# rkansal47/MPGAN

Hardware: AMD Instinct MI355X
Metric: jets/sec (G+D step) MPGAN gluon N=30 bs=256 @1/2/4/8 MI355X (higher is better)
Workload: dtype split-16-bit MFMA, fp32 accumulate, fp32 in/out: f16 hi/lo x3 terms (forward), f16 x2 / x1 terms in per-sender dithered units (edge backward: data / weight gradients), bf16 hi/lo x3 (node network gradients); 1 GPU; MPGAN gluon-like jets (--jets g: lr_disc 3e-05, lr_gen 1e-05), N=30 particles, B=256 per GPU, one train_D+train_G iteration (LSGAN, RMSprop, D dropout 0.5); jets=g, loss=ls, fwd_two_term=False, global_batch=256, particles=30, multiplicity=gluon, parallelism=dp1, hip_graphs=True, graph_collectives=False

## Files before the change

include/mpgan_amd.h:

```cpp
#ifndef MPGAN_AMD_H
#define MPGAN_AMD_H
#include <stdint.h>
#ifdef __cplusplus
extern "C" {
#endif

typedef struct MpgGemm {
    const float* A;
    const float* A2;
    int lda, lda2, K1;
    const float* B;
    int ldb;
    float* C;
    int ldc;
    int M, N, K;
    long long split_stride;
    const float* bias;
    float out_scale;
    int act;
    float alpha;
    const uint64_t* seed;
    uint32_t drop_tag, drop_thr; float drop_scale;
    const float* gateH;
    int ldh, gate_act;
    uint32_t gate_tag, gate_thr; float gate_scale;
    const float* resid;
    int ldr;
    int accumulate;
    int f16;
    int ones_col;
} MpgGemm;

int mpg_gemm(const MpgGemm* g, int ak, int bk, int splitk, void* stream);

int mpg_splitk_reduce(const float* part, int S, int N, int K, int has_bias, float* out, int ldo, float* bias,
                      void* stream);

#define MPG_GROUP_MAX 16
typedef struct MpgReduceJob {
    const float* part; int S, N, K, has_bias; float* out; int ldo; float* bias;
    int accumulate;
} MpgReduceJob;
int mpg_gemm_wgrad_group(const MpgGemm* g, const int* splitk, int n, void* stream);
int mpg_splitk_reduce_group(const MpgReduceJob* jobs, int n, void* stream);

int mpg_gate(const float* in, int ldi, const float* H, int ldh, float* out, int ldo, int M, int N,
             int gate_act, float alpha, const uint64_t* seed, uint32_t tag, uint32_t thr, float scale,
             void* stream);

int mpg_slab_sums(const float* A, int slabsA, uint64_t strideA, const float* B, int slabsB, uint64_t strideB,
                  float* out, int M, int cols, void* stream);

int mpg_dropout_mask(float* out, uint64_t rows, int F, const uint64_t* seed, uint32_t tag, uint32_t thr,
                     void* stream);

int mpg_pack_weights(const float* W, int ldw, int rows, int cols, int transpose, float scale, int f16,
                     void* img, void* stream);

#define MPG_PACK_MAX_JOBS 24
typedef struct MpgPackJob {
    const float* W; int ldw, rows, cols, transpose; float scale; int f16; void* img;
    int row_split, split_cols;
    int* status;
} MpgPackJob;
int mpg_pack_many(const MpgPackJob* jobs, int njobs, void* stream);

typedef struct MpgChainLayer {
    const void* Wimg; const float* bias; int nbias;
    int K, N, act;
    uint32_t drop_tag, drop_thr; float drop_scale;
    const float* gateH; int ldh, gate_act;
    uint32_t gate_tag, gate_thr; float gate_scale;
    const float* resid; int ldr;
    float* out; int ldo;
    float wscale;
} MpgChainLayer;
typedef struct MpgChain {
    const float* A; int lda, K1;
    const float* A2; int lda2;
    int a_slabs; uint64_t a_slab_stride;
    uint32_t in_tag, in_thr; float in_scale;
    float* in_out; int ld_in_out;
    int M, nlayers; float alpha; const uint64_t* seed; int f16;
    float ascale;
    MpgChainLayer L[3];
} MpgChain;
int mpg_chain(const MpgChain* p, void* stream);

typedef struct MpgEdgeFwd {
    const float* a; const float* c;
    int ld_ac;
    const float* mask;
    const void* W2img; const void* W3img;
    const float* b2; const float* b3;
    float* agg;
    int B, N, SC;
    float alpha, agg_scale;
    const uint64_t* seed; uint32_t tag_base, thr; float dscale;
    int skip_masked;
    int f16;
    unsigned int* sign3;
    const unsigned int* nbr;
    void* stageE2;
    const float* es; const float* wq;
    const int* order;
    unsigned int* tickets;
    int two_term;
} MpgEdgeFwd;
#define MPG_EDGE_SCALARS 2
int mpg_edge_fwd(const MpgEdgeFwd* p, void* stream);

#define MPG_FN_NA (-100)
int mpg_edge_fwd_fn(const MpgEdgeFwd* p, const MpgChain* c, const MpgChain* c2, void* stream);

int mpg_knn_sets(const float* x, int ldx, const float* mask, int B, int N, int F, int k, int self_loops,
                 unsigned int* nbr, void* stream);

typedef struct MpgEdgeBwd {
    const float* a; const float* c; int ld_ac; const float* mask;
    const float* dagg; int ld_dagg;
    const unsigned int* sign3;
    const void* W2img; const void* W3Timg; const void* W2Timg;
    const float* b2;
    float* da; float* dc;
    const void* stageE2;
    void* stageZ2;
    int B, N, SC;
    float alpha, agg_scale;
    const uint64_t* seed; uint32_t tag_base, thr; float dscale;
    int f16;
    const unsigned int* nbr;
    int* gexp;
    const float* es; const float* wq;
    float* des;
    float* daq;
    const int* order;
} MpgEdgeBwd;
int mpg_edge_bwd(const MpgEdgeBwd* p, void* stream);

int mpg_edge_bwd_fn(const MpgEdgeBwd* p, const MpgChain* cdx, const MpgChain* cnx, void* stream);

typedef struct MpgEdgeDw {
    const float* a; const float* c; int ld_ac; const float* mask;
    const float* dagg; int ld_dagg;
    const unsigned int* sign3;
    const void* stageE2; const void* stageZ2;
    float* part; int nwg;
    float* dW3; float* dW2; float* db3; float* db2;
    int accumulate;
    int B, N;
    float alpha, agg_scale;
    const uint64_t* seed; uint32_t tag_base, thr; float dscale;
    int f16;
    const unsigned int* nbr;
    const int* gexp;
    const float* es; const float* wq;
    int defer_reduce;
} MpgEdgeDw;
int mpg_edge_dw(const MpgEdgeDw* p, void* stream);
int mpg_splitk_reduce_group_dw(const MpgReduceJob* jobs, int n, const MpgEdgeDw* p, void* stream);

typedef struct MpgAttn {
    const float* q; const float* k; const float* v; int ldq, ldk, ldv;
    const float* ignore;
    float* o; int ldo;
    float* P;
    const float* d_o;
    float* dq; float* dk; float* dv; int lddq, lddk, lddv;
    int B, L, S, H, d;
} MpgAttn;
int mpg_attn_fwd(const MpgAttn* p, void* stream);
int mpg_attn_bwd(const MpgAttn* p, void* stream);

int mpg_rank_mask(const float* x, int ld_jet, int ld_part, const float* labels, int ld_lab, int B, int N,
                  float* mask, float* ignore, void* stream);

int mpg_jet_order(const float* mask, int B, int N, int* order, void* stream);

int mpg_gen_tail_fwd(const float* y, int ldy, const float* mask, float* out, int ldo, int V, int F, int act, void* stream);
int mpg_gen_tail_bwd(const float* dout, int ldd, const float* out, int ldo, float* dy, int ldy, int V, int F, int act,
                     void* stream);

typedef struct MpgDiscHead {
    const float* y; int ldy;
    const float* mask;
    const float* w; const float* bias;
    int B, N, F;
    int mean;
    int sigmoid;
    const uint64_t* seed; uint32_t tag, thr; float dscale;
    float* out;
    float* pooled; float* aux;
    int loss, gen_step, n_real; float inv_count;
    const float* gout;
    float* terms; float* loss_out;
    float* dy; int ld_dy;
    float* dw; float* db; int accumulate;
} MpgDiscHead;
int mpg_disc_head_fwd(const MpgDiscHead* p, void* stream);
int mpg_disc_head_bwd(const MpgDiscHead* p, void* stream);
int mpg_disc_head_loss(const MpgDiscHead* p, void* stream);

typedef struct MpgBridge {
    const float* x; int ldx;
    const float* W1; const float* b1;
    int act1;
    float* feat; int ldf;
    int M, row0, K, F, E;
    const float* W2; const float* b2;
    int act2; float alpha;
    const uint64_t* seed; uint32_t tag, thr; float dscale;
    float* e; int lde;
} MpgBridge;
typedef struct MpgBridgeBwd {
    const float* ge; int ldge;
    const float* e; int lde;
    const float* feat; int ldf;
    const float* gfeat; int ldgf;
    const float* W1; const float* W2;
    int M, row0, K, F, E, act1, act2; float alpha;
    const uint64_t* seed; uint32_t tag, thr; float dscale;
    float* g2; int ldg2;
    float* g1; int ldg1;
    float* dx; int lddx;
} MpgBridgeBwd;
int mpg_bridge_fwd(const MpgBridge* p, void* stream);
int mpg_bridge_bwd(const MpgBridgeBwd* p, void* stream);

typedef struct MpgMab {
    const float* x; int ldx;
    const float* y; int ldy;
    const float* ignore;
    const void* Win; const float* bin;
    const void* Wo; const float* bo;
    const void* Wf; const float* bf;
    int B, L, S, E, H;
    float alpha; int ff_act;
    const uint64_t* seed; uint32_t tag; uint32_t thr_mab; float sc_mab; uint32_t thr_ff; float sc_ff;
    float wscale, ascale;
    float* out; int ldo;
    float* save_o; float* save_z;
    const void* WinT; const void* WoT; const void* WfT;
    const float* dout; int lddout;
    float* dx; int lddx; float* dy; int lddy;
    float* dq; int lddq; float* dk; float* dv; int lddkv;
    float* dza; float* du;
    const float* ln1_w; const float* ln1_b; const float* ln2_w; const float* ln2_b; float ln_eps;
    float* save_za;
    float* dn1; float* gn1; float* dn2; float* gn2;
} MpgMab;
int mpg_mab_fwd(const MpgMab* p, void* stream);
int mpg_mab_bwd(const MpgMab* p, void* stream);
#define MPG_MAB_CHAIN_MAX 4
typedef struct MpgMabChain { MpgMab blk[MPG_MAB_CHAIN_MAX]; int n; } MpgMabChain;
int mpg_mab_chain_fwd(const MpgMabChain* c, void* stream);

int mpg_layernorm_fwd(const float* x, int ldx, const float* w, const float* b, float* y, int ldy, float* stats, int M,
                      int E, float eps, void* stream);
int mpg_layernorm_bwd(const float* g, int ldg, const float* x, int ldx, const float* w, const float* stats, float* dx,
                      int lddx, float* part, int nwaves, float* dw, float* db, int accumulate, int M, int E, void* stream);

int mpg_batchnorm_stats(const float* x, int ldx, int M, int F, float* part, int nchunk, float* mean, float* var, void* stream);
int mpg_batchnorm_apply(const float* x, int ldx, const float* mean, const float* var, const float* w, const float* b, float eps,
                        float* y, int ldy, int M, int F, void* stream);
int mpg_batchnorm_bwd(const float* g, int ldg, const float* x, int ldx, const float* mean, const float* var, const float* w, float eps,
                      float* part, int nchunk, float* sums, float* dx, int lddx, float* dw, float* db, int accumulate, int M, int F,
                      void* stream);

int mpg_rmsprop(float* p, float* g, float* v, uint64_t n, float lr, float alpha, float eps, float gscale, int zero_grad,
                uint64_t* counter, uint64_t counter_add, void* stream);
int mpg_adam(float* p, float* g, float* m, float* v, float* step, uint64_t n, float lr, float beta1,
             float beta2, float eps, float weight_decay, float gscale, int zero_grad, uint64_t* counter, uint64_t counter_add,
             void* stream);
int mpg_adadelta(float* p, float* g, float* v, float* u, uint64_t n, float lr, float rho, float eps,
                 float gscale, int zero_grad, uint64_t* counter, uint64_t counter_add, void* stream);

#define MPG_JET_OBS_MAX_N 160
#define MPG_JET_OBS_EFP 1
#define MPG_JET_OBS_NORMED 2
int mpg_jet_obs(const float* jets, int ld_jet, int ld_part, int n, int N, int flags, float* kin, float* efp, void* stream);

#define MPG_JET_EFPS_D4_PRIMES 21
int mpg_jet_efps_d4(const float* jets, int ld_jet, int ld_part, int n, int N, int flags, float* efp, void* stream);

int mpg_jet_emd(const float* a, int ld_jet_a, const float* b, int ld_jet_b, int ld_part, int na, int nb, int N, float R,
                float* out, int* status, void* stream);
int mpg_jet_emd_host(const float* a, int ld_jet_a, const float* b, int ld_jet_b, int ld_part, int na, int nb, int N, float R,
                     double* out, int* status, int threads);
int mpg_jet_emd_host_iters(const float* a, int ld_jet_a, const float* b, int ld_jet_b, int ld_part, int na, int nb, int N, float R,
                           double* out, int* status, int* iters, int threads);

int mpg_normal(float* out, uint64_t n, const uint64_t* seed, uint32_t tag, float mean, float std, void* stream);
int mpg_normal_rank_mask(float* out, int B, int N, int L, const uint64_t* seed, uint32_t tag, float mean, float std,
                         const float* labels, int ld_lab, float* mask, float* ignore, void* stream);

#define MPG_AUG_R90 1
#define MPG_AUG_FLIP 2
#define MPG_AUG_TRANSLATE 4
#define MPG_AUG_SCALE 8
int mpg_augment(const float* x, float* y, uint64_t jet_stride, int ld, int F, int B, int N, const uint64_t* seed, uint32_t tag,
                const float* p, int flags, float translate_ratio, float scale_sd, float* params, void* stream);
int mpg_augment_bwd(const float* dy, float* dx, uint64_t jet_stride, int ld, int F, int B, int N, const float* params,
                    void* stream);

#define MPG_SHUFFLE_TAG 0x53000000
int mpg_shuffle_index_host(uint64_t key, uint64_t pos0, int64_t count, int64_t n, int32_t* out);

int mpg_batch_feed(const float* particles, const float* labels_in, int64_t n, int N, uint64_t key, uint64_t* cursor,
                   uint32_t* ticket, int B, uint64_t stride, float* data, float* labels, float* dcat, float* x3, float* mask2,
                   float* ign2, float* labels2, void* stream);

#ifdef __cplusplus
}
#endif
#endif
```

mpgan_amd/_lib.py:

```python
from __future__ import annotations

import ctypes as C
import glob
import os
import subprocess

_HERE = os.path.dirname(os.path.abspath(__file__))
CSRC = os.path.join(_HERE, "csrc")
LIBDIR = os.environ.get("MPG_LIBDIR") or os.path.join(_HERE, "lib")
LIBPATH = os.path.join(LIBDIR, "libmpgan_amd.so")
INCLUDE = os.path.join(os.path.dirname(_HERE), "include")

_u64p = C.POINTER(C.c_uint64)
_fp = C.c_void_p


class MpgGemm(C.Structure):
    _fields_ = [
        ("A", _fp), ("A2", _fp), ("lda", C.c_int), ("lda2", C.c_int), ("K1", C.c_int),
        ("B", _fp), ("ldb", C.c_int),
        ("C", _fp), ("ldc", C.c_int),
        ("M", C.c_int), ("N", C.c_int), ("K", C.c_int),
        ("split_stride", C.c_longlong),
        ("bias", _fp), ("out_scale", C.c_float), ("act", C.c_int), ("alpha", C.c_float),
        ("seed", _fp),
        ("drop_tag", C.c_uint32), ("drop_thr", C.c_uint32), ("drop_scale", C.c_float),
        ("gateH", _fp), ("ldh", C.c_int), ("gate_act", C.c_int),
        ("gate_tag", C.c_uint32), ("gate_thr", C.c_uint32), ("gate_scale", C.c_float),
        ("resid", _fp), ("ldr", C.c_int),
        ("accumulate", C.c_int), ("f16", C.c_int), ("ones_col", C.c_int),
    ]


class MpgEdgeFwd(C.Structure):
    _fields_ = [
        ("a", _fp), ("c", _fp), ("ld_ac", C.c_int), ("mask", _fp),
        ("W2img", _fp), ("W3img", _fp), ("b2", _fp), ("b3", _fp),
        ("agg", _fp),
        ("B", C.c_int), ("N", C.c_int), ("SC", C.c_int),
        ("alpha", C.c_float), ("agg_scale", C.c_float),
        ("seed", _fp), ("tag_base", C.c_uint32), ("thr", C.c_uint32), ("dscale", C.c_float),
        ("skip_masked", C.c_int), ("f16", C.c_int),
        ("sign3", _fp), ("nbr", _fp), ("stageE2", _fp),
        ("es", _fp), ("wq", _fp), ("order", _fp), ("tickets", _fp),
        ("two_term", C.c_int),
    ]


class MpgEdgeBwd(C.Structure):
    _fields_ = [
        ("a", _fp), ("c", _fp), ("ld_ac", C.c_int), ("mask", _fp),
        ("dagg", _fp), ("ld_dagg", C.c_int),
        ("sign3", _fp),
        ("W2img", _fp), ("W3Timg", _fp), ("W2Timg", _fp),
        ("b2", _fp),
        ("da", _fp), ("dc", _fp),
        ("stageE2", _fp), ("stageZ2", _fp),
        ("B", C.c_int), ("N", C.c_int), ("SC", C.c_int),
        ("alpha", C.c_float), ("agg_scale", C.c_float),
        ("seed", _fp), ("tag_base", C.c_uint32), ("thr", C.c_uint32), ("dscale", C.c_float),
        ("f16", C.c_int), ("nbr", _fp), ("gexp", _fp),
        ("es", _fp), ("wq", _fp), ("des", _fp), ("daq", _fp), ("order", _fp),
    ]


class MpgEdgeDw(C.Structure):
    _fields_ = [
        ("a", _fp), ("c", _fp), ("ld_ac", C.c_int), ("mask", _fp),
        ("dagg", _fp), ("ld_dagg", C.c_int),
        ("sign3", _fp), ("stageE2", _fp), ("stageZ2", _fp),
        ("part", _fp), ("nwg", C.c_int),
        ("dW3", _fp), ("dW2", _fp), ("db3", _fp), ("db2", _fp), ("accumulate", C.c_int),
        ("B", C.c_int), ("N", C.c_int),
        ("alpha", C.c_float), ("agg_scale", C.c_float),
        ("seed", _fp), ("tag_base", C.c_uint32), ("thr", C.c_uint32), ("dscale", C.c_float),
        ("f16", C.c_int), ("nbr", _fp), ("gexp", _fp),
        ("es", _fp), ("wq", _fp), ("defer_reduce", C.c_int),
    ]


class MpgReduceJob(C.Structure):
    _fields_ = [
        ("part", _fp), ("S", C.c_int), ("N", C.c_int), ("K", C.c_int), ("has_bias", C.c_int),
        ("out", _fp), ("ldo", C.c_int), ("bias", _fp), ("accumulate", C.c_int),
    ]


class MpgPackJob(C.Structure):
    _fields_ = [
        ("W", _fp), ("ldw", C.c_int), ("rows", C.c_int), ("cols", C.c_int), ("transpose", C.c_int),
        ("scale", C.c_float), ("f16", C.c_int), ("img", _fp), ("row_split", C.c_int), ("split_cols", C.c_int),
        ("status", _fp),
    ]


class MpgChainLayer(C.Structure):
    _fields_ = [
        ("Wimg", _fp), ("bias", _fp), ("nbias", C.c_int),
        ("K", C.c_int), ("N", C.c_int), ("act", C.c_int),
        ("drop_tag", C.c_uint32), ("drop_thr", C.c_uint32), ("drop_scale", C.c_float),
        ("gateH", _fp), ("ldh", C.c_int), ("gate_act", C.c_int),
        ("gate_tag", C.c_uint32), ("gate_thr", C.c_uint32), ("gate_scale", C.c_float),
        ("resid", _fp), ("ldr", C.c_int),
        ("out", _fp), ("ldo", C.c_int),
        ("wscale", C.c_float),
    ]


class MpgChain(C.Structure):
    _fields_ = [
        ("A", _fp), ("lda", C.c_int), ("K1", C.c_int),
        ("A2", _fp), ("lda2", C.c_int),
        ("a_slabs", C.c_int), ("a_slab_stride", C.c_uint64),
        ("in_tag", C.c_uint32), ("in_thr", C.c_uint32), ("in_scale", C.c_float),
        ("in_out", _fp), ("ld_in_out", C.c_int),
        ("M", C.c_int), ("nlayers", C.c_int), ("alpha", C.c_float), ("seed", _fp), ("f16", C.c_int),
        ("ascale", C.c_float),
        ("L", MpgChainLayer * 3),
    ]


class MpgAttn(C.Structure):
    _fields_ = [
        ("q", _fp), ("k", _fp), ("v", _fp), ("ldq", C.c_int), ("ldk", C.c_int), ("ldv", C.c_int),
        ("ignore", _fp), ("o", _fp), ("ldo", C.c_int), ("P", _fp), ("d_o", _fp),
        ("dq", _fp), ("dk", _fp), ("dv", _fp), ("lddq", C.c_int), ("lddk", C.c_int), ("lddv", C.c_int),
        ("B", C.c_int), ("L", C.c_int), ("S", C.c_int), ("H", C.c_int), ("d", C.c_int),
    ]


class MpgDiscHead(C.Structure):
    _fields_ = [
        ("y", _fp), ("ldy", C.c_int), ("mask", _fp), ("w", _fp), ("bias", _fp),
        ("B", C.c_int), ("N", C.c_int), ("F", C.c_int), ("mean", C.c_int), ("sigmoid", C.c_int),
        ("seed", _fp), ("tag", C.c_uint32), ("thr", C.c_uint32), ("dscale", C.c_float),
        ("out", _fp), ("pooled", _fp), ("aux", _fp),
        ("loss", C.c_int), ("gen_step", C.c_int), ("n_real", C.c_int), ("inv_count", C.c_float),
        ("gout", _fp), ("terms", _fp), ("loss_out", _fp),
        ("dy", _fp), ("ld_dy", C.c_int), ("dw", _fp), ("db", _fp), ("accumulate", C.c_int),
    ]


class MpgBridge(C.Structure):
    _fields_ = [
        ("x", _fp), ("ldx", C.c_int), ("W1", _fp), ("b1", _fp), ("act1", C.c_int),
        ("feat", _fp), ("ldf", C.c_int),
        ("M", C.c_int), ("row0", C.c_int), ("K", C.c_int), ("F", C.c_int), ("E", C.c_int),
        ("W2", _fp), ("b2", _fp), ("act2", C.c_int), ("alpha", C.c_float),
        ("seed", _fp), ("tag", C.c_uint32), ("thr", C.c_uint32), ("dscale", C.c_float),
        ("e", _fp), ("lde", C.c_int),
    ]


class MpgBridgeBwd(C.Structure):
    _fields_ = [
        ("ge", _fp), ("ldge", C.c_int), ("e", _fp), ("lde", C.c_int), ("feat", _fp), ("ldf", C.c_int),
        ("gfeat", _fp), ("ldgf", C.c_int), ("W1", _fp), ("W2", _fp),
        ("M", C.c_int), ("row0", C.c_int), ("K", C.c_int), ("F", C.c_int), ("E", C.c_int), ("act1", C.c_int), ("act2", C.c_int),
        ("alpha", C.c_float),
        ("seed", _fp), ("tag", C.c_uint32), ("thr", C.c_uint32), ("dscale", C.c_float),
        ("g2", _fp), ("ldg2", C.c_int), ("g1", _fp), ("ldg1", C.c_int), ("dx", _fp), ("lddx", C.c_int),
    ]


class MpgMab(C.Structure):
    _fields_ = [
        ("x", _fp), ("ldx", C.c_int), ("y", _fp), ("ldy", C.c_int), ("ignore", _fp),
        ("Win", _fp), ("bin", _fp), ("Wo", _fp), ("bo", _fp), ("Wf", _fp), ("bf", _fp),
        ("B", C.c_int), ("L", C.c_int), ("S", C.c_int), ("E", C.c_int), ("H", C.c_int),
        ("alpha", C.c_float), ("ff_act", C.c_int),
        ("seed", _fp), ("tag", C.c_uint32), ("thr_mab", C.c_uint32), ("sc_mab", C.c_float),
        ("thr_ff", C.c_uint32), ("sc_ff", C.c_float), ("wscale", C.c_float), ("ascale", C.c_float),
        ("out", _fp), ("ldo", C.c_int), ("save_o", _fp), ("save_z", _fp),
        ("WinT", _fp), ("WoT", _fp), ("WfT", _fp),
        ("dout", _fp), ("lddout", C.c_int), ("dx", _fp), ("lddx", C.c_int), ("dy", _fp), ("lddy", C.c_int),
        ("dq", _fp), ("lddq", C.c_int), ("dk", _fp), ("dv", _fp), ("lddkv", C.c_int),
        ("dza", _fp), ("du", _fp),
        ("ln1_w", _fp), ("ln1_b", _fp), ("ln2_w", _fp), ("ln2_b", _fp), ("ln_eps", C.c_float),
        ("save_za", _fp), ("dn1", _fp), ("gn1", _fp), ("dn2", _fp), ("gn2", _fp),
    ]


MPG_FN_NA = -100

MAB_CHAIN_MAX = 4


class MpgMabChain(C.Structure):
    _fields_ = [("blk", MpgMab * MAB_CHAIN_MAX), ("n", C.c_int)]


SIGNATURES = {
    "mpg_gemm": (C.c_int, [C.POINTER(MpgGemm), C.c_int, C.c_int, C.c_int, C.c_void_p]),
    "mpg_splitk_reduce": (C.c_int, [_fp, C.c_int, C.c_int, C.c_int, C.c_int, _fp, C.c_int, _fp, C.c_void_p]),
    "mpg_gemm_wgrad_group": (C.c_int, [C.POINTER(MpgGemm), C.POINTER(C.c_int), C.c_int, C.c_void_p]),
    "mpg_splitk_reduce_group": (C.c_int, [C.POINTER(MpgReduceJob), C.c_int, C.c_void_p]),
    "mpg_splitk_reduce_group_dw": (C.c_int, [C.POINTER(MpgReduceJob), C.c_int, C.POINTER(MpgEdgeDw), C.c_void_p]),
    "mpg_slab_sums": (C.c_int, [_fp, C.c_int, C.c_uint64, _fp, C.c_int, C.c_uint64, _fp, C.c_int, C.c_int, C.c_void_p]),
    "mpg_gate": (C.c_int, [_fp, C.c_int, _fp, C.c_int, _fp, C.c_int, C.c_int, C.c_int, C.c_int, C.c_float,
                           _fp, C.c_uint32, C.c_uint32, C.c_float, C.c_void_p]),
    "mpg_dropout_mask": (C.c_int, [_fp, C.c_uint64, C.c_int, _fp, C.c_uint32, C.c_uint32, C.c_void_p]),
    "mpg_pack_weights": (C.c_int, [_fp, C.c_int, C.c_int, C.c_int, C.c_int, C.c_float, C.c_int, _fp, C.c_void_p]),
    "mpg_pack_many": (C.c_int, [C.POINTER(MpgPackJob), C.c_int, C.c_void_p]),
    "mpg_chain": (C.c_int, [C.POINTER(MpgChain), C.c_void_p]),
    "mpg_edge_fwd": (C.c_int, [C.POINTER(MpgEdgeFwd), C.c_void_p]),
    "mpg_edge_fwd_fn": (C.c_int, [C.POINTER(MpgEdgeFwd), C.POINTER(MpgChain), C.POINTER(MpgChain), C.c_void_p]),
    "mpg_edge_bwd": (C.c_int, [C.POINTER(MpgEdgeBwd), C.c_void_p]),
    "mpg_edge_bwd_fn": (C.c_int, [C.POINTER(MpgEdgeBwd), C.POINTER(MpgChain), C.POINTER(MpgChain), C.c_void_p]),
    "mpg_edge_dw": (C.c_int, [C.POINTER(MpgEdgeDw), C.c_void_p]),
    "mpg_attn_fwd": (C.c_int, [C.POINTER(MpgAttn), C.c_void_p]),
    "mpg_attn_bwd": (C.c_int, [C.POINTER(MpgAttn), C.c_void_p]),
    "mpg_mab_fwd": (C.c_int, [C.POINTER(MpgMab), C.c_void_p]),
    "mpg_mab_bwd": (C.c_int, [C.POINTER(MpgMab), C.c_void_p]),
    "mpg_mab_chain_fwd": (C.c_int, [C.POINTER(MpgMabChain), C.c_void_p]),
    "mpg_knn_sets": (C.c_int, [_fp, C.c_int, _fp, C.c_int, C.c_int, C.c_int, C.c_int, C.c_int, _fp, C.c_void_p]),
    "mpg_rank_mask": (C.c_int, [_fp, C.c_int, C.c_int, _fp, C.c_int, C.c_int, C.c_int, _fp, _fp, C.c_void_p]),
    "mpg_jet_order": (C.c_int, [_fp, C.c_int, C.c_int, _fp, C.c_void_p]),
    "mpg_gen_tail_fwd": (C.c_int, [_fp, C.c_int, _fp, _fp, C.c_int, C.c_int, C.c_int, C.c_int, C.c_void_p]),
    "mpg_gen_tail_bwd": (C.c_int, [_fp, C.c_int, _fp, C.c_int, _fp, C.c_int, C.c_int, C.c_int, C.c_int, C.c_void_p]),
    "mpg_disc_head_fwd": (C.c_int, [C.POINTER(MpgDiscHead), C.c_void_p]),
    "mpg_disc_head_bwd": (C.c_int, [C.POINTER(MpgDiscHead), C.c_void_p]),
    "mpg_disc_head_loss": (C.c_int, [C.POINTER(MpgDiscHead), C.c_void_p]),
    "mpg_layernorm_fwd": (C.c_int, [_fp, C.c_int, _fp, _fp, _fp, C.c_int, _fp, C.c_int, C.c_int, C.c_float, C.c_void_p]),
    "mpg_layernorm_bwd": (C.c_int, [_fp, C.c_int, _fp, C.c_int, _fp, _fp, _fp, C.c_int, _fp, C.c_int, _fp, _fp, C.c_int,
                                    C.c_int, C.c_int, C.c_void_p]),
    "mpg_batchnorm_stats": (C.c_int, [_fp, C.c_int, C.c_int, C.c_int, _fp, C.c_int, _fp, _fp, C.c_void_p]),
    "mpg_batchnorm_apply": (C.c_int, [_fp, C.c_int, _fp, _fp, _fp, _fp, C.c_float, _fp, C.c_int, C.c_int, C.c_int, C.c_void_p]),
    "mpg_batchnorm_bwd": (C.c_int, [_fp, C.c_int, _fp, C.c_int, _fp, _fp, _fp, C.c_float, _fp, C.c_int, _fp, _fp, C.c_int, _fp, _fp,
                                    C.c_int, C.c_int, C.c_int, C.c_void_p]),
    "mpg_rmsprop": (C.c_int, [_fp, _fp, _fp, C.c_uint64, C.c_float, C.c_float, C.c_float, C.c_float, C.c_int, _fp, C.c_uint64, C.c_void_p]),
    "mpg_adam": (C.c_int, [_fp, _fp, _fp, _fp, _fp, C.c_uint64, C.c_float, C.c_float, C.c_float, C.c_float, C.c_float,
                           C.c_float, C.c_int, _fp, C.c_uint64, C.c_void_p]),
    "mpg_adadelta": (C.c_int, [_fp, _fp, _fp, _fp, C.c_uint64, C.c_float, C.c_float, C.c_float, C.c_float, C.c_int, _fp, C.c_uint64,
                               C.c_void_p]),
    "mpg_bridge_fwd": (C.c_int, [C.POINTER(MpgBridge), C.c_void_p]),
    "mpg_bridge_bwd": (C.c_int, [C.POINTER(MpgBridgeBwd), C.c_void_p]),
    "mpg_normal": (C.c_int, [_fp, C.c_uint64, _fp, C.c_uint32, C.c_float, C.c_float, C.c_void_p]),
    "mpg_normal_rank_mask": (C.c_int, [_fp, C.c_int, C.c_int, C.c_int, _fp, C.c_uint32, C.c_float, C.c_float, _fp, C.c_int, _fp, _fp,
                                       C.c_void_p]),
    "mpg_jet_obs": (C.c_int, [_fp, C.c_int, C.c_int, C.c_int, C.c_int, C.c_int, _fp, _fp, C.c_void_p]),
    "mpg_jet_efps_d4": (C.c_int, [_fp, C.c_int, C.c_int, C.c_int, C.c_int, C.c_int, _fp, C.c_void_p]),
    "mpg_jet_emd": (C.c_int, [_fp, C.c_int, _fp, C.c_int, C.c_int, C.c_int, C.c_int, C.c_int, C.c_float, _fp, _fp, C.c_void_p]),
    "mpg_jet_emd_host": (C.c_int, [_fp, C.c_int, _fp, C.c_int, C.c_int, C.c_int, C.c_int, C.c_int, C.c_float, _fp, _fp, C.c_int]),
    "mpg_jet_emd_host_iters": (C.c_int, [_fp, C.c_int, _fp, C.c_int, C.c_int, C.c_int, C.c_int, C.c_int, C.c_float, _fp, _fp, _fp,
                                         C.c_int]),
    "mpg_augment": (C.c_int, [_fp, _fp, C.c_uint64, C.c_int, C.c_int, C.c_int, C.c_int, _fp, C.c_uint32, _fp, C.c_int, C.c_float,
                              C.c_float, _fp, C.c_void_p]),
    "mpg_augment_bwd": (C.c_int, [_fp, _fp, C.c_uint64, C.c_int, C.c_int, C.c_int, C.c_int, _fp, C.c_void_p]),
    "mpg_shuffle_index_host": (C.c_int, [C.c_uint64, C.c_uint64, C.c_int64, C.c_int64, _fp]),
    "mpg_batch_feed": (C.c_int, [_fp, _fp, C.c_int64, C.c_int, C.c_uint64, _fp, _fp, C.c_int, C.c_uint64, _fp, _fp, _fp, _fp, _fp,
                                 _fp, _fp, C.c_void_p]),
}


EXTRA_FLAGS = os.environ.get("MPG_HIPCC_FLAGS", "-fno-slp-vectorize").split()


def sources():
    return sorted(glob.glob(os.path.join(CSRC, "*.hip")))


DIGEST_FILE = os.path.join(LIBDIR, "libmpgan_amd.source_digest")


def _stale():
    if not os.path.isfile(LIBPATH):
        return True
    if os.path.isfile(DIGEST_FILE):
        try:
            with open(DIGEST_FILE) as f:
                return f.read().strip() != source_digest()
        except OSError:
            pass
    t = os.path.getmtime(LIBPATH)
    deps = sources() + glob.glob(os.path.join(CSRC, "*.h")) + glob.glob(os.path.join(INCLUDE, "*.h"))
    return any(os.path.getmtime(d) > t for d in deps)


def _includes(path, seen):
    import re
    if path in seen:
        return
    seen.add(path)
    with open(path, "r", errors="replace") as f:
        text = f.read()
    for inc in re.findall(r'^\s*#\s*include\s+"([^"]+)"', text, flags=re.M):
        for root in (os.path.dirname(path), INCLUDE):
            cand = os.path.normpath(os.path.join(root, inc))
            if os.path.isfile(cand):
                _includes(cand, seen)
                break


_compiler_id_cache = {}


def _compiler_id(hipcc: str) -> str:
    if hipcc not in _compiler_id_cache:
        real = os.path.realpath(hipcc)
        try:
            ver = subprocess.run([hipcc, "--version"], check=True, capture_output=True, text=True, env=_compiler_env(),
                                 timeout=60).stdout
        except Exception:
            st = os.stat(real) if os.path.exists(real) else None
            ver = "unversioned %s %s" % ((st.st_size, int(st.st_mtime)) if st else ("?", "?"))
        _compiler_id_cache[hipcc] = real + "\n" + ver
    return _compiler_id_cache[hipcc]


def _digest(src, flags, hipcc=None) -> str:
    import hashlib
    deps = set()
    _includes(os.path.abspath(src), deps)
    h = hashlib.sha1(" ".join(flags).encode())
    if hipcc is not None:
        h.update(b"\0" + _compiler_id(hipcc).encode() + b"\0")
    for d in sorted(deps):
        with open(d, "rb") as f:
            h.update(os.path.relpath(d, CSRC).encode() + b"\0" + f.read() + b"\0")
    return h.hexdigest()[:16]


def source_digest() -> str:
    import hashlib
    h = hashlib.sha1()
    for d in sorted(sources() + glob.glob(os.path.join(CSRC, "*.h")) + glob.glob(os.path.join(INCLUDE, "*.h"))):
        with open(d, "rb") as f:
            h.update(os.path.basename(d).encode() + b"\0" + f.read() + b"\0")
    return h.hexdigest()[:16]


def _compiler_env():
    env = dict(os.environ)
    for k in list(env):
        if k == "LD_PRELOAD" or k.startswith(("ROCP", "ROCPROF", "HSA_TOOLS", "ROCTRACER")):
            env.pop(k)
    return env


def _under_profiler() -> bool:
    pre = os.environ.get("LD_PRELOAD", "").lower()
    return any(t in pre for t in ("rocprof", "roctracer", "rocp_")) or any(k.startswith(("ROCPROF", "ROCP_")) for k in os.environ)


def _note_digest():
    if not os.path.isfile(DIGEST_FILE):
        try:
            tmp = DIGEST_FILE + ".%d.tmp" % os.getpid()
            with open(tmp, "w") as f:
                f.write(source_digest() + "\n")
            os.replace(tmp, DIGEST_FILE)
        except OSError:
            pass


def build(force: bool = False, verbose: bool = False) -> str:
    if not force and not _stale():
        _note_digest()
        return LIBPATH
    import fcntl
    import tempfile
    os.makedirs(LIBDIR, exist_ok=True)
    with open(os.path.join(LIBDIR, ".build.lock"), "w") as lock:
        fcntl.flock(lock, fcntl.LOCK_EX)
        if not force and not _stale():
            return LIBPATH
        hipcc = os.environ.get("HIPCC", "/opt/rocm/bin/hipcc")
        env = _compiler_env()
        tmpdir = tempfile.mkdtemp(prefix=".build.", dir=LIBDIR)
        objdir = os.path.join(LIBDIR, "obj")
        os.makedirs(objdir, exist_ok=True)
        try:
            jobs, objs = [], []
            flags = ["--offload-arch=gfx950", "-O3", "-fPIC", "-std=c++17"] + EXTRA_FLAGS
            for src in sources():
                base = os.path.basename(src)[:-4]
                obj = os.path.join(objdir, "%s.%s.o" % (base, _digest(src, flags, hipcc)))
                objs.append(obj)
                if force or not os.path.isfile(obj):
                    tmpobj = os.path.join(tmpdir, base + ".o")
                    jobs.append((tmpobj, [hipcc] + flags + ["-I", INCLUDE, "-c", src, "-o", tmpobj], obj, base))
            from concurrent.futures import ThreadPoolExecutor

            def run(job):
                if verbose:
                    print(" ".join(job[1]))
                subprocess.run(job[1], check=True, env=env)
                for old in glob.glob(os.path.join(objdir, job[3] + ".*.o")):
                    os.remove(old)
                os.replace(job[0], job[2])
            if jobs:
                with ThreadPoolExecutor(max_workers=max(1, min(os.cpu_count() or 4, 8, len(jobs)))) as ex:
                    list(ex.map(run, jobs))
            tmplib = os.path.join(tmpdir, "libmpgan_amd.so")
            subprocess.run([hipcc, "--offload-arch=gfx950", "-shared", "-fPIC", "-o", tmplib] + objs, check=True, env=env)
            os.replace(tmplib, LIBPATH)
            with open(os.path.join(tmpdir, "digest"), "w") as f:
                f.write(source_digest() + "\n")
            os.replace(os.path.join(tmpdir, "digest"), DIGEST_FILE)
        finally:
            import shutil
            shutil.rmtree(tmpdir, ignore_errors=True)
    return LIBPATH


_lib = None


def lib():
    global _lib
    if _lib is None:
        if _stale() and not (os.environ.get("MPG_LIB_STALE_OK") == "1" and os.environ.get("MPG_LIBDIR") and os.path.isfile(LIBPATH)):
            can_build = os.path.isfile(os.environ.get("HIPCC", "/opt/rocm/bin/hipcc")) and os.path.isdir(CSRC)
            guarded = int(os.environ.get("WORLD_SIZE", "1")) > 1 or _under_profiler()
            if can_build and not guarded:
                build()
            elif not os.path.isfile(LIBPATH):
                raise RuntimeError("libmpgan_amd.so is missing%s: run `python __graft_entry__.py` (build) first"
                                   % (" and this process must not compile (multi-rank launch or profiler preload)"
                                      if can_build else " and hipcc is not available"))
            elif can_build:
                raise RuntimeError("libmpgan_amd.so is older than its sources and this process must not compile "
                                   "(multi-rank launch or profiler preload): run `python __graft_entry__.py` first")
        _lib = C.CDLL(LIBPATH)
        for name, (res, args) in SIGNATURES.items():
            fn = getattr(_lib, name)
            fn.restype = res
            fn.argtypes = args
    return _lib


def check(code: int, what: str):
    if code != 0:
        raise RuntimeError(f"{what} failed with code {code}")
```

mpgan_amd/csrc/head.hip:

```cpp
#include "common.h"
#include "../../include/mpgan_amd.h"

namespace {

__global__ __launch_bounds__(256) void rank_mask_kernel(const float* __restrict__ x, int ld_jet, int ld_part,
                                                        const float* __restrict__ labels, int ld_lab, int N,
                                                        float* __restrict__ mask, float* __restrict__ ignore) {
    extern __shared__ float xs[];
    const int b = blockIdx.x;
    for (int i = threadIdx.x; i < N; i += blockDim.x) xs[i] = x[(size_t)b * ld_jet + (size_t)i * ld_part];
    __syncthreads();
    const int n_minus_1 = (int)(labels[(size_t)b * ld_lab] * (float)N) - 1;
    for (int i = threadIdx.x; i < N; i += blockDim.x) {
        const float xi = xs[i];
        int rank = 0;
        for (int j = 0; j < N; ++j) {
            const float xj = xs[j];
            rank += (xj < xi) || (xj == xi && j < i);
        }
        mask[(size_t)b * N + i] = rank <= n_minus_1 ? 1.f : 0.f;
        if (ignore != nullptr) ignore[(size_t)b * N + i] = rank <= n_minus_1 ? 0.f : 1.f;
    }
}

__global__ __launch_bounds__(1024) void jet_order_kernel(const float* __restrict__ mask, int B, int N, int* __restrict__ order) {
    extern __shared__ int jo[];
    int* keys = jo;
    int* hist = jo + B;
    int* wcnt = jo + B + N + 2;
    const int nw = (B + 63) / 64, lane = threadIdx.x & 63;
    for (int t = threadIdx.x; t < N + 2; t += blockDim.x) hist[t] = 0;
    for (int t = threadIdx.x; t < nw * (N + 1); t += blockDim.x) wcnt[t] = 0;
    __syncthreads();
    for (int b = threadIdx.x; b < B; b += blockDim.x) {
        const float* mb = mask + (size_t)b * N;
        int c = 0;
#pragma unroll 8
        for (int i = 0; i < N; ++i) c += mb[i] != 0.f;
        const int k = N - c;
        keys[b] = k;
        atomicAdd(&hist[k + 1], 1);
        atomicAdd(&wcnt[(b >> 6) * (N + 1) + k], 1);
    }
    __syncthreads();
    if (threadIdx.x == 0)
        for (int k = 1; k < N + 2; ++k) hist[k] += hist[k - 1];
    for (int k = threadIdx.x; k <= N; k += blockDim.x) {
        int run = 0;
        for (int w = 0; w < nw; ++w) { const int c = wcnt[w * (N + 1) + k]; wcnt[w * (N + 1) + k] = run; run += c; }
    }
    __syncthreads();
    for (int b0 = (threadIdx.x >> 6) * 64; b0 < B; b0 += blockDim.x) {
        const int b = b0 + lane;
        const int k = b < B ? keys[b] : -1;
        int below = 0;
        for (int l = 0; l < 64; ++l) {
            const int kl = __shfl(k, l, 64);
            below += (l < lane && kl == k);
        }
        if (b < B) order[hist[k] + wcnt[(b >> 6) * (N + 1) + k] + below] = b;
    }
}

__global__ __launch_bounds__(256) void gen_tail_fwd_kernel(const float* __restrict__ y, int ldy, const float* __restrict__ mask,
                                                           float* __restrict__ out, int ldo, int V, int F, int act) {
    const int v = blockIdx.x * blockDim.x + threadIdx.x;
    if (v >= V) return;
    for (int f = 0; f < F; ++f) {
        const float t = y[(size_t)v * ldy + f];
        out[(size_t)v * ldo + f] = act == 1 ? tanhf(t) : (act == 2 ? 1.f / (1.f + expf(-t)) : t);
    }
    if (mask != nullptr) out[(size_t)v * ldo + F] = mask[v] - 0.5f;
}

__global__ __launch_bounds__(256) void gen_tail_bwd_kernel(const float* __restrict__ dout, int ldd, const float* __restrict__ out, int ldo,
                                                           float* __restrict__ dy, int ldy, int V, int F, int act) {
    const int v = blockIdx.x * blockDim.x + threadIdx.x;
    if (v >= V) return;
    for (int f = 0; f < F; ++f) {
        const float o = out[(size_t)v * ldo + f], g = dout[(size_t)v * ldd + f];
        dy[(size_t)v * ldy + f] = act == 1 ? g * (1.f - o * o) : (act == 2 ? g * o * (1.f - o) : g);
    }
}

MPG_DEV float wave_sum(float x) {
#pragma unroll
    for (int o = 32; o > 0; o >>= 1) x += __shfl_xor(x, o, 64);
    return x;
}

MPG_DEV void disc_head_bwd_jet(const MpgDiscHead& p, const int b, const int lane, const float out, const float aux0);

template <bool FUSED>
__global__ __launch_bounds__(256) void disc_head_fwd_kernel(const MpgDiscHead p) {
    const int lane = threadIdx.x & 63, b = blockIdx.x * 4 + (threadIdx.x >> 6);
    if (b >= p.B) return;
    const float* yb = p.y + (size_t)b * p.N * p.ldy;
    float z = 0.f, msum = 0.f;
    for (int f0 = 0; f0 < p.F; f0 += 32) {
        const int f = f0 + (lane & 31);
        float a0 = 0.f, a1 = 0.f, a2 = 0.f, a3 = 0.f;
        auto term = [&](int i) {
            return i < p.N ? (p.mask ? p.mask[(size_t)b * p.N + i] : 1.f) * yb[(size_t)i * p.ldy + f] : 0.f;
        };
        if (f < p.F)
            for (int i = lane >> 5; i < p.N; i += 8) { a0 += term(i); a1 += term(i + 2); a2 += term(i + 4); a3 += term(i + 6); }
        float acc = (a0 + a1) + (a2 + a3);
        acc += __shfl_xor(acc, 32, 64);
        if (p.pooled != nullptr && lane < 32 && f < p.F) p.pooled[(size_t)b * p.F + f] = acc;
        z += (lane < 32 && f < p.F) ? acc * p.w[f] : 0.f;
    }
    if (p.mean) {
        for (int i = lane; i < p.N; i += 64) msum += p.mask ? p.mask[(size_t)b * p.N + i] : 1.f;
        msum = wave_sum(msum);
    }
    z = wave_sum(z);
    const float pool_scale = p.mean ? 1.f / (p.mask ? msum + 1e-12f : (float)p.N) : 1.f;
    z = z * pool_scale + (p.bias ? p.bias[0] : 0.f);
    float keep = 1.f;
    if (p.thr) {
        const uint64_t sd = *p.seed;
        keep = drop_keep_f((uint32_t)sd, (uint32_t)(sd >> 32), p.tag, (uint32_t)b, 0, p.thr) ? p.dscale : 0.f;
    }
    z *= keep;
    const float out = p.sigmoid ? 1.f / (1.f + expf(-z)) : z;
    if (lane == 0) {
        p.out[b] = out;
        if (p.aux != nullptr) { p.aux[2 * b] = keep * pool_scale; p.aux[2 * b + 1] = 0.f; }
    }
    if (FUSED) disc_head_bwd_jet(p, b, lane, out, keep * pool_scale);
}

MPG_DEV float loss_grad(int loss, float out, float t, float& term) {
    switch (loss) {
    case 0: term = (out - t) * (out - t); return 2.f * (out - t);
    case 1: {
        const float l1 = fmaxf(logf(out), -100.f), l0 = fmaxf(logf(1.f - out), -100.f);
        term = -(t * l1 + (1.f - t) * l0);
        return (out - t) / fmaxf((1.f - out) * out, 1e-12f);
    }
    case 2: term = t > 0.5f ? -out : out; return t > 0.5f ? -1.f : 1.f;
    default: {
        const float s = t > 0.5f ? -1.f : 1.f, m = 1.f + s * out;
        term = fmaxf(m, 0.f);
        return m > 0.f ? s : 0.f;
    }
    }
}

MPG_DEV void disc_head_bwd_jet(const MpgDiscHead& p, const int b, const int lane, const float out, const float aux0) {
    float g;
    if (p.loss >= 0) {
        const float t = b < p.n_real ? 1.f : 0.f;
        float term;
        g = loss_grad((p.gen_step && p.loss == 3) ? 2 : p.loss, out, t, term) * p.inv_count;
        if (lane == 0) p.terms[b] = term * p.inv_count;
    } else {
        g = p.gout[b];
    }
    const float gz = g * (p.sigmoid ? out * (1.f - out) : 1.f);
    const float gp = gz * aux0;
    if (lane == 0) p.aux[2 * b + 1] = gz * (aux0 != 0.f ? (p.thr ? p.dscale : 1.f) : 0.f);
    if (p.dy == nullptr) return;
    float* db_ = p.dy + (size_t)b * p.N * p.ld_dy;
    for (int f0 = 0; f0 < p.F; f0 += 32) {
        const int f = f0 + (lane & 31);
        if (f >= p.F) continue;
        const float wf = p.w[f] * gp;
        for (int i = lane >> 5; i < p.N; i += 2) db_[(size_t)i * p.ld_dy + f] = (p.mask ? p.mask[(size_t)b * p.N + i] : 1.f) * wf;
    }
}

__global__ __launch_bounds__(256) void disc_head_bwd_kernel(const MpgDiscHead p) {
    const int lane = threadIdx.x & 63, b = blockIdx.x * 4 + (threadIdx.x >> 6);
    if (b >= p.B) return;
    disc_head_bwd_jet(p, b, lane, p.out[b], p.aux[2 * b]);
}

__global__ __launch_bounds__(256) void disc_head_reduce_kernel(const MpgDiscHead p) {
    __shared__ float red[256];
    const int tid = threadIdx.x;
    if (blockIdx.x == 0) {
        if (p.loss >= 0 && p.loss_out != nullptr) {
            float s = 0.f;
            for (int b = tid; b < p.B; b += 256) s += p.terms[b];
            red[tid] = s;
            __syncthreads();
            for (int o = 128; o > 0; o >>= 1) { if (tid < o) red[tid] += red[tid + o]; __syncthreads(); }
            if (tid == 0) *p.loss_out = red[0];
        }
        return;
    }
    if (p.dw == nullptr) return;
    const int f = (blockIdx.x - 1) * 4 + (tid >> 6), lane = tid & 63;
    if (f > p.F) return;
    const float ds = p.thr ? p.dscale : 1.f;
    auto term = [&](int b) {
        if (b >= p.B) return 0.f;
        const float gzp = p.aux[2 * b + 1];
        if (f >= p.F) return gzp;
        const float a0 = p.aux[2 * b];
        return gzp * (a0 != 0.f ? a0 / ds : 0.f) * p.pooled[(size_t)b * p.F + f];
    };
    float s0 = 0.f, s1 = 0.f, s2 = 0.f, s3 = 0.f;
    for (int b = lane; b < p.B; b += 256) {
        s0 += term(b); s1 += term(b + 64); s2 += term(b + 128); s3 += term(b + 192);
    }
    float s = (s0 + s1) + (s2 + s3);
    s += __shfl_xor(s, 1, 64); s += __shfl_xor(s, 2, 64); s += __shfl_xor(s, 4, 64); s += __shfl_xor(s, 8, 64); s += __shfl_xor(s, 16, 64);
    s += __shfl_xor(s, 32, 64);
    if (lane == 0) {
        if (f < p.F) p.dw[f] = s + (p.accumulate ? p.dw[f] : 0.f);
        else if (p.db != nullptr) p.db[0] = s + (p.accumulate ? p.db[0] : 0.f);
    }
}

__global__ __launch_bounds__(256) void knn_sets_kernel(const float* __restrict__ x, int ldx, const float* __restrict__ mask, int N, int F,
                                                       int k, int first, unsigned int* __restrict__ nbr) {
    extern __shared__ float dist[];
    const int b = blockIdx.x, NW = (N + 31) >> 5;
    const float* xb = x + (size_t)b * N * ldx;
    for (int e = threadIdx.x; e < N * N; e += blockDim.x) {
        const int i = e / N, j = e % N;
        const float sj = mask != nullptr ? (1.f - 1e4f) * mask[(size_t)b * N + j] + 1e4f : 1.f;
        float acc = 0.f;
        for (int f = 0; f < F; ++f) {
            const float d = sj * xb[(size_t)j * ldx + f] - xb[(size_t)i * ldx + f] + 1e-12f;
            acc += d * d;
        }
        dist[e] = sqrtf(acc);
    }
    __syncthreads();
    for (int e = threadIdx.x; e < N * NW; e += blockDim.x) {
        const int i = e / NW, wq = e % NW;
        unsigned int bits = 0u;
        for (int jj = 0; jj < 32; ++jj) {
            const int j = wq * 32 + jj;
            if (j >= N) break;
            const float dij = dist[i * N + j];
            int rank = 0;
            for (int l = 0; l < N; ++l) {
                const float dil = dist[i * N + l];
                rank += (dil < dij) || (dil == dij && l < j);
            }
            if (rank >= first && rank < first + k) bits |= 1u << jj;
        }
        nbr[((size_t)b * N + i) * NW + wq] = bits;
    }
}

__global__ __launch_bounds__(256) void layernorm_fwd_kernel(const float* __restrict__ x, int ldx, const float* __restrict__ w,
                                                            const float* __restrict__ b, float* __restrict__ y, int ldy,
                                                            float* __restrict__ stats, int M, int E, float eps) {
    const int lane = threadIdx.x & 63, row = blockIdx.x * 4 + (threadIdx.x >> 6);
    if (row >= M) return;
    const float* xr = x + (size_t)row * ldx;
    float s = 0.f;
    for (int f = lane; f < E; f += 64) s += xr[f];
    const float mean = wave_sum(s) / (float)E;
    float v = 0.f;
    for (int f = lane; f < E; f += 64) { const float d = xr[f] - mean; v += d * d; }
    const float rstd = rsqrtf(wave_sum(v) / (float)E + eps);
    for (int f = lane; f < E; f += 64) y[(size_t)row * ldy + f] = (xr[f] - mean) * rstd * w[f] + b[f];
    if (lane == 0) { stats[2 * row] = mean; stats[2 * row + 1] = rstd; }
}

__global__ __launch_bounds__(256) void layernorm_bwd_kernel(const float* __restrict__ g, int ldg, const float* __restrict__ x, int ldx,
                                                            const float* __restrict__ w, const float* __restrict__ stats,
                                                            float* __restrict__ dx, int lddx, float* __restrict__ part,
                                                            int M, int E) {
    const int lane = threadIdx.x & 63, wv = blockIdx.x * 4 + (threadIdx.x >> 6), nwv = gridDim.x * 4;
    float aw[16], ab[16];
#pragma unroll
    for (int k = 0; k < 16; ++k) { aw[k] = 0.f; ab[k] = 0.f; }
    for (int row = wv; row < M; row += nwv) {
        const float mean = stats[2 * row], rstd = stats[2 * row + 1];
        const float* gr = g + (size_t)row * ldg;
        const float* xr = x + (size_t)row * ldx;
        float s1 = 0.f, s2 = 0.f;
#pragma unroll
        for (int k = 0; k < 16; ++k) {
            const int f = lane + 64 * k;
            if (f < E) {
                const float xh = (xr[f] - mean) * rstd, gw = gr[f] * w[f];
                s1 += gw; s2 += gw * xh;
                aw[k] += gr[f] * xh; ab[k] += gr[f];
            }
        }
        s1 = wave_sum(s1) / (float)E; s2 = wave_sum(s2) / (float)E;
#pragma unroll
        for (int k = 0; k < 16; ++k) {
            const int f = lane + 64 * k;
            if (f < E) {
                const float xh = (xr[f] - mean) * rstd;
                dx[(size_t)row * lddx + f] = rstd * (gr[f] * w[f] - s1 - xh * s2);
            }
        }
    }
#pragma unroll
    for (int k = 0; k < 16; ++k) {
        const int f = lane + 64 * k;
        if (f < E) { part[((size_t)wv * 2 + 0) * E + f] = aw[k]; part[((size_t)wv * 2 + 1) * E + f] = ab[k]; }
    }
}

__global__ __launch_bounds__(256) void layernorm_reduce_kernel(const float* __restrict__ part, int nwv, int E, float* __restrict__ dw,
                                                               float* __restrict__ db, int accumulate) {
    const int f = blockIdx.x * blockDim.x + threadIdx.x;
    if (f >= 2 * E) return;
    const int which = f / E, ff = f % E;
    float s = 0.f;
    for (int v = 0; v < nwv; ++v) s += part[((size_t)v * 2 + which) * E + ff];
    float* dst = which == 0 ? dw : db;
    dst[ff] = s + (accumulate ? dst[ff] : 0.f);
}

}

extern "C" int mpg_knn_sets(const float* x, int ldx, const float* mask, int B, int N, int F, int k, int self_loops,
                            unsigned int* nbr, void* stream) {
    if (B <= 0 || N <= 0 || F <= 0 || k <= 0 || N > 192) return -1;
    const int lds = N * N * (int)sizeof(float);
    MPG_ENSURE_LDS(knn_sets_kernel, lds);
    hipLaunchKernelGGL(knn_sets_kernel, dim3(B), dim3(256), lds, (hipStream_t)stream, x, ldx, mask, N, F, k, self_loops ? 0 : 1, nbr);
    return (int)hipGetLastError();
}

extern "C" int mpg_layernorm_fwd(const float* x, int ldx, const float* w, const float* b, float* y, int ldy, float* stats,
                                 int M, int E, float eps, void* stream) {
    if (M <= 0 || E <= 0) return -1;
    hipLaunchKernelGGL(layernorm_fwd_kernel, dim3((M + 3) / 4), dim3(256), 0, (hipStream_t)stream, x, ldx, w, b, y, ldy, stats, M, E, eps);
    return (int)hipGetLastError();
}

extern "C" int mpg_layernorm_bwd(const float* g, int ldg, const float* x, int ldx, const float* w, const float* stats, float* dx,
                                 int lddx, float* part, int nwaves, float* dw, float* db, int accumulate, int M, int E,
                                 void* stream) {
    if (M <= 0 || E <= 0 || E > 1024 || nwaves <= 0 || nwaves % 4 != 0) return -1;
    hipStream_t st = (hipStream_t)stream;
    hipLaunchKernelGGL(layernorm_bwd_kernel, dim3(nwaves / 4), dim3(256), 0, st, g, ldg, x, ldx, w, stats, dx, lddx, part, M, E);
    if (dw != nullptr)
        hipLaunchKernelGGL(layernorm_reduce_kernel, dim3((2 * E + 255) / 256), dim3(256), 0, st, part, nwaves, E, dw, db, accumulate);
    return (int)hipGetLastError();
}

extern "C" int mpg_rank_mask(const float* x, int ld_jet, int ld_part, const float* labels, int ld_lab, int B, int N,
                             float* mask, float* ignore, void* stream) {
    if (B <= 0 || N <= 0 || N > 8192) return -1;
    hipLaunchKernelGGL(rank_mask_kernel, dim3(B), dim3(N <= 64 ? 64 : 256), N * sizeof(float), (hipStream_t)stream, x, ld_jet, ld_part,
                       labels, ld_lab, N, mask, ignore);
    return (int)hipGetLastError();
}

extern "C" int mpg_jet_order(const float* mask, int B, int N, int* order, void* stream) {
    if (B <= 0 || N <= 0 || mask == nullptr || order == nullptr) return -1;
    const size_t lds = ((size_t)B + N + 2 + (size_t)((B + 63) / 64) * (N + 1)) * sizeof(int);
    if (lds > 64 * 1024) return -2;
    hipLaunchKernelGGL(jet_order_kernel, dim3(1), dim3(B <= 256 ? 256 : 1024), lds, (hipStream_t)stream, mask, B, N, order);
    return (int)hipGetLastError();
}

extern "C" int mpg_gen_tail_fwd(const float* y, int ldy, const float* mask, float* out, int ldo, int V, int F, int act,
                                void* stream) {
    if (V <= 0 || F <= 0) return -1;
    hipLaunchKernelGGL(gen_tail_fwd_kernel, dim3((V + 255) / 256), dim3(256), 0, (hipStream_t)stream, y, ldy, mask, out, ldo, V, F, act);
    return (int)hipGetLastError();
}

extern "C" int mpg_gen_tail_bwd(const float* dout, int ldd, const float* out, int ldo, float* dy, int ldy, int V, int F,
                                int act, void* stream) {
    if (V <= 0 || F <= 0) return -1;
    hipLaunchKernelGGL(gen_tail_bwd_kernel, dim3((V + 255) / 256), dim3(256), 0, (hipStream_t)stream, dout, ldd, out, ldo, dy, ldy, V, F, act);
    return (int)hipGetLastError();
}

extern "C" int mpg_disc_head_fwd(const MpgDiscHead* p, void* stream) {
    if (p->B <= 0 || p->N <= 0 || p->F <= 0 || p->out == nullptr || p->aux == nullptr) return -1;
    hipLaunchKernelGGL(disc_head_fwd_kernel<false>, dim3((p->B + 3) / 4), dim3(256), 0, (hipStream_t)stream, *p);
    return (int)hipGetLastError();
}

extern "C" int mpg_disc_head_loss(const MpgDiscHead* p, void* stream) {
    if (p->B <= 0 || p->N <= 0 || p->F <= 0 || p->out == nullptr || p->aux == nullptr) return -1;
    if (p->loss < 0 || p->terms == nullptr) return -2;
    if (p->dw != nullptr && p->pooled == nullptr) return -2;
    hipStream_t st = (hipStream_t)stream;
    hipLaunchKernelGGL(disc_head_fwd_kernel<true>, dim3((p->B + 3) / 4), dim3(256), 0, st, *p);
    if (p->loss_out != nullptr || p->dw != nullptr)
        hipLaunchKernelGGL(disc_head_reduce_kernel, dim3(1 + (p->dw != nullptr ? (p->F + 1 + 3) / 4 : 0)), dim3(256), 0, st, *p);
    return (int)hipGetLastError();
}

extern "C" int mpg_disc_head_bwd(const MpgDiscHead* p, void* stream) {
    if (p->B <= 0 || p->N <= 0 || p->F <= 0 || p->out == nullptr || p->aux == nullptr) return -1;
    if (p->loss >= 0 ? p->terms == nullptr : p->gout == nullptr) return -2;
    if (p->dw != nullptr && p->pooled == nullptr) return -2;
    hipStream_t st = (hipStream_t)stream;
    hipLaunchKernelGGL(disc_head_bwd_kernel, dim3((p->B + 3) / 4), dim3(256), 0, st, *p);
    if ((p->loss >= 0 && p->loss_out != nullptr) || p->dw != nullptr)
        hipLaunchKernelGGL(disc_head_reduce_kernel, dim3(1 + (p->dw != nullptr ? (p->F + 1 + 3) / 4 : 0)), dim3(256), 0, st, *p);
    return (int)hipGetLastError();
}
```

mpgan_amd/csrc/optim.hip:

```cpp
#include "common.h"
#include "../../include/mpgan_amd.h"

namespace {
__global__ void rmsprop_kernel(float* __restrict__ p, float* __restrict__ g, float* __restrict__ v, size_t n,
                               float lr, float alpha, float eps, float gscale, int zero_grad, uint64_t* __restrict__ counter, uint64_t counter_add) {
    if (counter != nullptr && blockIdx.x == 0 && threadIdx.x == 0) *counter += counter_add;
    size_t i = (size_t)blockIdx.x * blockDim.x + threadIdx.x;
    const size_t stride = (size_t)gridDim.x * blockDim.x;
    for (; i < n; i += stride) {
        const float gi = g[i] * gscale;
        const float vi = alpha * v[i] + (1.f - alpha) * gi * gi;
        v[i] = vi;
        p[i] -= lr * gi / (sqrtf(vi) + eps);
        if (zero_grad) g[i] = 0.f;
    }
}

__global__ void adam_kernel(float* __restrict__ p, float* __restrict__ g, float* __restrict__ m, float* __restrict__ v,
                            const float* __restrict__ step, size_t n, float lr, float b1, float b2, float eps, float wd,
                            float gscale, int zero_grad, uint64_t* __restrict__ counter, uint64_t counter_add) {
    if (counter != nullptr && blockIdx.x == 0 && threadIdx.x == 0) *counter += counter_add;
    const float t = *step + 1.f;
    const float bc1 = 1.f - powf(b1, t), bc2s = sqrtf(1.f - powf(b2, t));
    const float step_size = lr / bc1;
    size_t i = (size_t)blockIdx.x * blockDim.x + threadIdx.x;
    const size_t stride = (size_t)gridDim.x * blockDim.x;
    for (; i < n; i += stride) {
        const float pi = p[i];
        const float gi = g[i] * gscale + wd * pi;
        const float mi = b1 * m[i] + (1.f - b1) * gi;
        const float vi = b2 * v[i] + (1.f - b2) * gi * gi;
        m[i] = mi;
        v[i] = vi;
        p[i] = pi - step_size * mi / (sqrtf(vi) / bc2s + eps);
        if (zero_grad) g[i] = 0.f;
    }
}
__global__ void step_inc_kernel(float* step) { *step += 1.f; }

__global__ void adadelta_kernel(float* __restrict__ p, float* __restrict__ g, float* __restrict__ v, float* __restrict__ u,
                                size_t n, float lr, float rho, float eps, float gscale, int zero_grad, uint64_t* __restrict__ counter, uint64_t counter_add) {
    if (counter != nullptr && blockIdx.x == 0 && threadIdx.x == 0) *counter += counter_add;
    size_t i = (size_t)blockIdx.x * blockDim.x + threadIdx.x;
    const size_t stride = (size_t)gridDim.x * blockDim.x;
    for (; i < n; i += stride) {
        const float gi = g[i] * gscale;
        const float vi = rho * v[i] + (1.f - rho) * gi * gi;
        const float d = sqrtf(u[i] + eps) / sqrtf(vi + eps) * gi;
        v[i] = vi;
        u[i] = rho * u[i] + (1.f - rho) * d * d;
        p[i] -= lr * d;
        if (zero_grad) g[i] = 0.f;
    }
}

__global__ void normal_kernel(float* __restrict__ out, size_t n, const uint64_t* __restrict__ seed, uint32_t tag, float mean, float std) {
    const uint64_t sd = *seed;
    const uint32_t lo = (uint32_t)sd, hi = (uint32_t)(sd >> 32);
    size_t i = (size_t)blockIdx.x * blockDim.x + threadIdx.x;
    const size_t stride = (size_t)gridDim.x * blockDim.x, npair = (n + 1) / 2;
    for (; i < npair; i += stride) {
        uint32_t a = drop_word(lo, hi, tag, (uint32_t)i, (uint32_t)(i >> 32));
        uint32_t b = drop_word(hi ^ 0x9E3779B9u, lo, tag + 0x7F4A7C15u, (uint32_t)i ^ a, (uint32_t)(i >> 32) + 1u);
        const float u1 = ((float)(a >> 8) + 0.5f) * (1.f / 16777216.f);
        const float u2 = ((float)(b >> 8) + 0.5f) * (1.f / 16777216.f);
        const float r = sqrtf(-2.f * logf(u1)) * std;
        float sn, cs;
        sincosf(6.283185307179586f * u2, &sn, &cs);
        out[2 * i] = mean + r * cs;
        if (2 * i + 1 < n) out[2 * i + 1] = mean + r * sn;
    }
}

__global__ __launch_bounds__(256) void normal_rank_mask_kernel(float* __restrict__ out, int N, int L, const uint64_t* __restrict__ seed,
                                                               uint32_t tag, float mean, float std, const float* __restrict__ labels,
                                                               int ld_lab, float* __restrict__ mask, float* __restrict__ ignore) {
    extern __shared__ float first[];
    const uint64_t sd = *seed;
    const uint32_t lo = (uint32_t)sd, hi = (uint32_t)(sd >> 32);
    const int b = blockIdx.x;
    const size_t per_jet = (size_t)N * L, pair0 = (size_t)b * per_jet / 2, npair = per_jet / 2;
    for (size_t q = threadIdx.x; q < npair; q += blockDim.x) {
        const size_t i = pair0 + q;
        uint32_t a = drop_word(lo, hi, tag, (uint32_t)i, (uint32_t)(i >> 32));
        uint32_t c = drop_word(hi ^ 0x9E3779B9u, lo, tag + 0x7F4A7C15u, (uint32_t)i ^ a, (uint32_t)(i >> 32) + 1u);
        const float u1 = ((float)(a >> 8) + 0.5f) * (1.f / 16777216.f);
        const float u2 = ((float)(c >> 8) + 0.5f) * (1.f / 16777216.f);
        const float r = sqrtf(-2.f * logf(u1)) * std;
        float sn, cs;
        sincosf(6.283185307179586f * u2, &sn, &cs);
        const float v0 = mean + r * cs, v1 = mean + r * sn;
        out[2 * i] = v0;
        out[2 * i + 1] = v1;
        const size_t e0 = 2 * q;
        if (e0 % L == 0) first[e0 / L] = v0;
        if ((e0 + 1) % L == 0) first[(e0 + 1) / L] = v1;
    }
    __syncthreads();
    const int n_minus_1 = (int)(labels[(size_t)b * ld_lab] * (float)N) - 1;
    for (int i = threadIdx.x; i < N; i += blockDim.x) {
        const float xi = first[i];
        int rank = 0;
        for (int j = 0; j < N; ++j) {
            const float xj = first[j];
            rank += (xj < xi) || (xj == xi && j < i);
        }
        mask[(size_t)b * N + i] = rank <= n_minus_1 ? 1.f : 0.f;
        if (ignore != nullptr) ignore[(size_t)b * N + i] = rank <= n_minus_1 ? 0.f : 1.f;
    }
}

inline int nblocks(uint64_t n) { return (int)((n + 255) / 256 < 2048 ? (n + 255) / 256 : 2048); }
}

extern "C" int mpg_rmsprop(float* p, float* g, float* v, uint64_t n, float lr, float alpha, float eps,
                           float gscale, int zero_grad, uint64_t* counter, uint64_t counter_add, void* stream) {
    if (n == 0) return counter != nullptr ? -1 : 0;
    hipLaunchKernelGGL(rmsprop_kernel, dim3(nblocks(n)), dim3(256), 0, (hipStream_t)stream, p, g, v, (size_t)n, lr, alpha,
                       eps, gscale, zero_grad, counter, counter_add);
    return (int)hipGetLastError();
}

extern "C" int mpg_adam(float* p, float* g, float* m, float* v, float* step, uint64_t n, float lr, float beta1,
                        float beta2, float eps, float weight_decay, float gscale, int zero_grad, uint64_t* counter, uint64_t counter_add,
                        void* stream) {
    if (n == 0) return counter != nullptr ? -1 : 0;
    if (step == nullptr) return -1;
    hipLaunchKernelGGL(adam_kernel, dim3(nblocks(n)), dim3(256), 0, (hipStream_t)stream, p, g, m, v, step, (size_t)n, lr,
                       beta1, beta2, eps, weight_decay, gscale, zero_grad, counter, counter_add);
    hipLaunchKernelGGL(step_inc_kernel, dim3(1), dim3(1), 0, (hipStream_t)stream, step);
    return (int)hipGetLastError();
}

extern "C" int mpg_adadelta(float* p, float* g, float* v, float* u, uint64_t n, float lr, float rho, float eps,
                            float gscale, int zero_grad, uint64_t* counter, uint64_t counter_add, void* stream) {
    if (n == 0) return counter != nullptr ? -1 : 0;
    hipLaunchKernelGGL(adadelta_kernel, dim3(nblocks(n)), dim3(256), 0, (hipStream_t)stream, p, g, v, u, (size_t)n, lr, rho,
                       eps, gscale, zero_grad, counter, counter_add);
    return (int)hipGetLastError();
}

extern "C" int mpg_normal(float* out, uint64_t n, const uint64_t* seed, uint32_t tag, float mean, float std, void* stream) {
    if (n == 0) return 0;
    if (seed == nullptr || !(std >= 0.f)) return -1;
    hipLaunchKernelGGL(normal_kernel, dim3(nblocks((n + 1) / 2)), dim3(256), 0, (hipStream_t)stream, out, (size_t)n, seed, tag, mean, std);
    return (int)hipGetLastError();
}

extern "C" int mpg_normal_rank_mask(float* out, int B, int N, int L, const uint64_t* seed, uint32_t tag, float mean, float std,
                                    const float* labels, int ld_lab, float* mask, float* ignore, void* stream) {
    if (B <= 0 || N <= 0 || L <= 0 || N > 8192 || ((size_t)N * L) % 2) return -1;
    if (seed == nullptr || labels == nullptr || mask == nullptr || !(std >= 0.f)) return -1;
    hipLaunchKernelGGL(normal_rank_mask_kernel, dim3(B), dim3(256), N * sizeof(float), (hipStream_t)stream, out, N, L, seed, tag, mean,
                       std, labels, ld_lab, mask, ignore);
    return (int)hipGetLastError();
}
```

mpgan_amd/ops.py:

```python
from __future__ import annotations

import ctypes as C
import itertools
import os
import sys
import threading
from collections import namedtuple
from typing import Optional

import torch
from torch.autograd.function import once_differentiable

from . import _lib
from ._lib import MpgGemm, MpgEdgeFwd, MpgEdgeBwd, MpgEdgeDw, MpgPackJob, MpgChain, MpgReduceJob, check

H1, H2, H3 = 96, 160, 192
SC_W2, SC_W3 = 16.0, 64.0
SC_WN, SC_ACT = 64.0, 8.0
TAG_E0, TAG_E1, TAG_E2, TAG_N0, TAG_N1, TAG_N2, TAG_GENERIC = 1, 2, 3, 4, 5, 6, 7

OPTIONS = {
    "skip_masked": True,
    "lpt_order": True,
    "fn_epilogue": os.environ.get("MPG_FN_EPILOGUE", "1") != "0",
    "bwd_epilogue": os.environ.get("MPG_BWD_EPILOGUE", "1") != "0",
    "fn_chunks": os.environ.get("MPG_FN_CHUNKS", "1") != "0",
    "dw_reduce_grouped": os.environ.get("MPG_DW_REDUCE_GROUPED", "1") != "0",
    "fwd_two_term": int(os.environ.get("MPG_FWD_TWO_TERM", "0")),
}
NUM_CUS = 256
FWD_F16 = True


class DeviceState:

    def __init__(self, index: int):
        self.index = index
        self._seed = None
        self.seed_is_default = True
        self.auto_seed_key = None
        self.tags = itertools.count(1)
        self.last_tag = 0
        self.tag_log = None
        self.sign_tap = None
        self.grad_into_param = False
        self.deferred_wgrad = None
        self.wgrad_stream = None
        self.wgrad_keep = []
        self.double_backward = False
        self._status = None

    @property
    def status(self) -> torch.Tensor:
        if self._status is None:
            dev = torch.device("cuda", self.index) if self.index >= 0 else torch.device("cpu")
            self._status = torch.zeros((1,), dtype=torch.int32, device=dev)
        return self._status

    @property
    def seed(self) -> torch.Tensor:
        if self._seed is None:
            dev = torch.device("cuda", self.index) if self.index >= 0 else torch.device("cpu")
            self._seed = torch.full((1,), 0x243F6A8885A308D3, dtype=torch.int64, device=dev)
        return self._seed


_states = {}
_states_lock = threading.Lock()


def _dev_index(device) -> int:
    if isinstance(device, int):
        return device
    d = torch.device(device)
    if d.type == "cpu":
        return -1
    if d.index is not None:
        return d.index
    return torch.cuda.current_device() if torch.cuda.is_available() else 0


def dev_state(device) -> DeviceState:
    idx = _dev_index(device)
    st = _states.get(idx)
    if st is None:
        with _states_lock:
            st = _states.get(idx)
            if st is None:
                st = _states[idx] = DeviceState(idx)
    return st


def seed_tensor(device) -> torch.Tensor:
    return dev_state(device).seed


def range_status(device="cuda", clear: bool = False) -> int:
    st = dev_state(device).status
    v = int(st.item())
    if clear:
        st.zero_()
    return v


def set_seed(value: int, device="cuda", _auto: bool = False):
    v = int(value) & 0xFFFFFFFFFFFFFFFF
    seed_tensor(device).fill_(v - (1 << 64) if v >= (1 << 63) else v)
    st = dev_state(device)
    st.seed_is_default = _auto
    if not _auto:
        st.auto_seed_key = None


def derived_seed(torch_seed: int, rank: int) -> int:
    return (torch_seed * 0x9E3779B97F4A7C15 + (rank + 1) * 0xD1B54A32D192ED03 + 0x243F6A8885A308D3) & 0x7FFFFFFFFFFFFFFF


RANK_TERM = 0xD1B54A32D192ED03


def rerank_seed(saved: int, saved_rank: int, rank: int) -> int:
    return (int(saved) + (int(rank) - int(saved_rank)) * RANK_TERM) & 0xFFFFFFFFFFFFFFFF


def get_seed(device="cuda") -> int:
    return int(seed_tensor(device).item()) & 0xFFFFFFFFFFFFFFFF


SEED_STEP = 0x1E3779B97F4A7C15


def bump_seed(device="cuda"):
    seed_tensor(device).add_(SEED_STEP)


NOISE_TAG = 0x4E000000


def normal_noise(shape, std: float, site: int = 0, device="cuda", mean: float = 0.0) -> torch.Tensor:
    out = torch.empty(shape, device=device, dtype=torch.float32)
    check(_lib.lib().mpg_normal(_p(out), out.numel(), _p(seed_tensor(out.device)), NOISE_TAG + int(site), mean, std, _stream()),
          "mpg_normal")
    return out


def next_tag(device="cuda", kind: str = "", thr: int = 0) -> int:
    st = dev_state(device)
    st.last_tag = (next(st.tags) % (1 << 24)) * 8
    if st.tag_log is not None:
        st.tag_log.append((kind, st.last_tag, int(thr)))
    return st.last_tag


def last_tag(device="cuda") -> int:
    return dev_state(device).last_tag


def drop_params(p: float):
    thr = int(round(256.0 * p))
    if thr <= 0:
        return 0, 1.0
    if thr >= 256:
        raise ValueError("dropout p too close to 1")
    return thr, 256.0 / (256.0 - thr)


TICKET_SLOTS = 32


def _tickets(device, n: int) -> torch.Tensor:
    buf = reserve_tickets(device, n)
    st = dev_state(device)
    st._ticket_i = (st._ticket_i + 1) % TICKET_SLOTS
    return buf[st._ticket_i]


def reserve_tickets(device, n: int) -> torch.Tensor:
    st = dev_state(device)
    buf = getattr(st, "_tickets", None)
    per = max(4096, n)
    if buf is None or buf.shape[1] < per:
        if buf is not None:
            st._tickets_retired = getattr(st, "_tickets_retired", []) + [buf]
        buf = torch.zeros((TICKET_SLOTS, per), dtype=torch.int32, device=device)
        if not torch.cuda.is_current_stream_capturing():
            torch.cuda.synchronize(device)
        st._tickets, st._ticket_i = buf, 0
    return buf


def _stream():
    return C.c_void_p(torch.cuda.current_stream().cuda_stream)


def _p(t: Optional[torch.Tensor], offset_elems: int = 0):
    if t is None:
        return None
    return C.c_void_p(t.data_ptr() + 4 * offset_elems)


def _chk(t: torch.Tensor, name: str):
    if not (t.is_cuda and t.dtype == torch.float32):
        raise RuntimeError(f"{name}: expected a float32 tensor on the GPU (got {t.dtype} on {t.device}); "
                           "mpgan_amd has no CPU path")


def gemm(A, lda, B, ldb, Cout, ldc, M, N, K, *, ak=True, bk=True, a_off=0, b_off=0, c_off=0,
         A2=None, lda2=0, K1=0, bias=None, out_scale=1.0, act=False, alpha=0.2,
         drop=None, gate=None, resid=None, ldr=0, accumulate=False, splitk=1, split_stride=0, f16=False,
         ones_col=False):
    g = MpgGemm()
    g.A, g.A2, g.lda, g.lda2, g.K1 = _p(A, a_off), _p(A2), lda, lda2, K1
    g.B, g.ldb = _p(B, b_off), ldb
    g.C, g.ldc = _p(Cout, c_off), ldc
    g.M, g.N, g.K = M, N, K
    g.split_stride = split_stride
    g.bias, g.out_scale, g.act, g.alpha = _p(bias), out_scale, int(act), alpha
    g.seed = None
    if drop is not None and drop[2]:
        g.seed = _p(drop[0]); g.drop_tag, g.drop_thr, g.drop_scale = drop[1], drop[2], drop[3]
    if gate is not None:
        H, ldh, gact, seed_t, tag, thr, scale = gate
        g.gateH, g.ldh, g.gate_act = _p(H), ldh, int(gact)
        if thr:
            g.seed = _p(seed_t); g.gate_tag, g.gate_thr, g.gate_scale = tag, thr, scale
    g.resid, g.ldr = _p(resid), ldr
    g.accumulate = int(accumulate)
    g.f16 = int(f16)
    g.ones_col = int(ones_col)
    check(_lib.lib().mpg_gemm(C.byref(g), int(ak), int(bk), splitk, _stream()), "mpg_gemm")


def linear_fwd(x, W, bias=None, *, act=False, alpha=0.2, drop=None, x2=None, w_col0=0, w_cols=None, resid=None, f16=None):
    M, K1 = x.shape
    K2 = 0 if x2 is None else x2.shape[1]
    K = K1 + K2 if w_cols is None else w_cols
    N = W.shape[0]
    y = torch.empty((M, N), device=x.device, dtype=torch.float32)
    gemm(x, x.stride(0), W, W.stride(0), y, N, M, N, K, ak=True, bk=True, b_off=w_col0,
         A2=x2, lda2=0 if x2 is None else x2.stride(0), K1=K1, bias=bias, act=act, alpha=alpha, drop=drop,
         resid=resid, ldr=0 if resid is None else resid.stride(0), f16=FWD_F16 if f16 is None else f16)
    return y


def linear_bwd_data(dy, W, *, w_col0=0, w_cols=None, gate=None, out=None, accumulate=False, alpha=0.2):
    M, N = dy.shape
    K = (W.shape[1] - w_col0) if w_cols is None else w_cols
    if out is None:
        out = torch.empty((M, K), device=dy.device, dtype=torch.float32)
    gemm(dy, dy.stride(0), W, W.stride(0), out, out.stride(0), M, K, N, ak=True, bk=False, b_off=w_col0,
         gate=gate, accumulate=accumulate, alpha=alpha)
    return out


def linear_bwd_weight(dy, x, *, out=None, out_col0=0, out_scale=1.0, bias_out=None):
    M, N = dy.shape
    K = x.shape[1]
    if out is None:
        out = torch.empty((N, K), device=dy.device, dtype=torch.float32)
    hb = int(bias_out is not None)
    tiles = ((N + 63) // 64) * ((K + hb + 63) // 64)
    splitk = max(1, min((M + 255) // 256, (1024 + tiles - 1) // tiles))
    part = torch.empty((splitk, N, K + hb), device=dy.device, dtype=torch.float32)
    gemm(dy, dy.stride(0), x, x.stride(0), part, K + hb, N, K + hb, M, ak=False, bk=False, out_scale=out_scale,
         splitk=splitk, split_stride=N * (K + hb), ones_col=bool(hb))
    check(_lib.lib().mpg_splitk_reduce(_p(part), splitk, N, K, hb, _p(out, out_col0), out.stride(0), _p(bias_out),
                                       _stream()), "mpg_splitk_reduce")
    return out


WGRAD_TARGET_WGS = int(__import__("os").environ.get("MPG_WGRAD_TARGET", "512"))


GROUP_MAX = 16


class WgradBatch:

    def __init__(self):
        self.jobs = []

    def add(self, dy, x, *, out, out_col0=0, out_scale=1.0, bias_out=None, accumulate=False):
        M, N = dy.shape
        K = x.shape[1]
        hb = int(bias_out is not None)
        kcols = K if (hb and K % 64 == 0) else K + hb
        tiles = ((N + 63) // 64) * ((kcols + 63) // 64)
        splitk = max(1, min((M + 255) // 256, (WGRAD_TARGET_WGS + tiles - 1) // tiles))
        part = torch.empty((splitk, N, K + hb), device=dy.device, dtype=torch.float32)
        self.jobs.append((dy, x, out, out_col0, out_scale, bias_out, splitk, part, accumulate))

    def flush(self, dw=None):
        if dw is not None and not self.jobs:
            check(_lib.lib().mpg_splitk_reduce_group_dw(None, 0, C.byref(dw), _stream()), "mpg_splitk_reduce_group_dw")
        for i0 in range(0, len(self.jobs), GROUP_MAX):
            jobs = self.jobs[i0:i0 + GROUP_MAX]
            n = len(jobs)
            gs, sk, rj = (MpgGemm * n)(), (C.c_int * n)(), (MpgReduceJob * n)()
            for i, (dy, x, out, col0, scale, bias_out, splitk, part, acc) in enumerate(jobs):
                M, N = dy.shape
                K = x.shape[1]
                hb = int(bias_out is not None)
                g = gs[i]
                g.A, g.lda, g.B, g.ldb = _p(dy), dy.stride(0), _p(x), x.stride(0)
                g.C, g.ldc = _p(part), K + hb
                g.M, g.N, g.K = N, K + hb, M
                g.split_stride, g.out_scale, g.alpha, g.ones_col = N * (K + hb), scale, 0.2, hb
                sk[i] = splitk
                r = rj[i]
                r.part, r.S, r.N, r.K, r.has_bias = _p(part), splitk, N, K, hb
                r.out, r.ldo, r.bias, r.accumulate = _p(out, col0), out.stride(0), _p(bias_out), int(acc)
            check(_lib.lib().mpg_gemm_wgrad_group(gs, sk, n, _stream()), "mpg_gemm_wgrad_group")
            if dw is not None and i0 == 0:
                check(_lib.lib().mpg_splitk_reduce_group_dw(rj, n, C.byref(dw), _stream()), "mpg_splitk_reduce_group_dw")
            else:
                check(_lib.lib().mpg_splitk_reduce_group(rj, n, _stream()), "mpg_splitk_reduce_group")
        self.jobs = []


def gate(g, H, *, gate_act, alpha, seed_t=None, tag=0, thr=0, scale=1.0):
    M, N = g.shape
    out = torch.empty((M, N), device=g.device, dtype=torch.float32)
    check(_lib.lib().mpg_gate(_p(g), g.stride(0), _p(H), 0 if H is None else H.stride(0), _p(out), N, M, N,
                              int(gate_act), alpha, _p(seed_t), tag, thr, scale, _stream()), "mpg_gate")
    return out


def normal_noise_masked(shape, std: float, labels: torch.Tensor, site: int = 0, device="cuda", mean: float = 0.0,
                        mask_out: Optional[torch.Tensor] = None, ignore_out: Optional[torch.Tensor] = None):
    B, N, L = shape
    out = torch.empty(shape, device=device, dtype=torch.float32)
    lab = labels[:, -1]
    if lab.dtype != torch.float32:
        lab = lab.float()
    mask = mask_out if mask_out is not None else torch.empty((B, N), device=device, dtype=torch.float32)
    ign = ignore_out if ignore_out is not None else torch.empty((B, N), device=device, dtype=torch.float32)
    assert mask.is_contiguous() and ign.is_contiguous() and mask.numel() == B * N and ign.numel() == B * N
    check(_lib.lib().mpg_normal_rank_mask(_p(out), B, N, L, _p(seed_tensor(out.device)), NOISE_TAG + int(site), mean, std,
                                          _p(lab), lab.stride(0), _p(mask), _p(ign), _stream()), "mpg_normal_rank_mask")
    return out, mask.view(B, N), ign.view(B, N)


SHUFFLE_TAG = 0x53000000


def shuffle_indices(key: int, pos0: int, count: int, n: int) -> torch.Tensor:
    out = torch.empty(int(count), dtype=torch.int32)
    check(_lib.lib().mpg_shuffle_index_host(int(key) & 0xFFFFFFFFFFFFFFFF, int(pos0) & 0xFFFFFFFFFFFFFFFF, int(count), int(n),
                                            C.c_void_p(out.data_ptr())), "mpg_shuffle_index_host")
    return out.long()


def batch_feed(particles: torch.Tensor, labels_in: torch.Tensor, key: int, cursor: torch.Tensor, ticket: torch.Tensor, B: int,
               stride: int, data=None, labels=None, dcat=None, x3=None, mask2=None, ign2=None, labels2=None):
    _chk(particles, "particles")
    n, N, F = particles.shape
    if F != 4 or not particles.is_contiguous():
        raise ValueError(f"batch_feed: contiguous particles [n, N, 4] expected, got {tuple(particles.shape)}")
    if cursor.dtype != torch.int64 or ticket.dtype != torch.int32 or cursor.device != particles.device or ticket.device != particles.device:
        raise ValueError("batch_feed: cursor (int64) and ticket (int32) live on the data set's device")
    need = {"data": (data, B * N * 4), "labels": (labels, B), "dcat": (dcat, B * N * 4), "x3": (x3, B * N * 3),
            "mask2": (mask2, B * N), "ign2": (ign2, B * N), "labels2": (labels2, 2 * B), "labels_in": (labels_in, n)}
    for name, (t, k) in need.items():
        if t is not None:
            _chk(t, name)
            if not t.is_contiguous() or t.numel() < k:
                raise ValueError(f"batch_feed: {name} must be contiguous with at least {k} elements, got {tuple(t.shape)}")
    check(_lib.lib().mpg_batch_feed(_p(particles), _p(labels_in), n, N, int(key) & 0xFFFFFFFFFFFFFFFF, C.c_void_p(cursor.data_ptr()),
                                    C.c_void_p(ticket.data_ptr()), int(B), int(stride), _p(data), _p(labels), _p(dcat), _p(x3),
                                    _p(mask2), _p(ign2), _p(labels2), _stream()), "mpg_batch_feed")


AUG_TAG = 0x41000000
AUG_R90, AUG_FLIP, AUG_TRANSLATE, AUG_SCALE = 1, 2, 4, 8


def augment_flags(aug_r90=False, aug_f=False, aug_t=False, aug_s=False) -> int:
    return AUG_R90 * bool(aug_r90) + AUG_FLIP * bool(aug_f) + AUG_TRANSLATE * bool(aug_t) + AUG_SCALE * bool(aug_s)


def _jet_layout(x: torch.Tensor, name: str):
    _chk(x, name)
    B, N, F = x.shape
    if x.stride(2) != 1 or x.stride(1) < F or x.stride(0) < N * x.stride(1):
        raise ValueError(f"{name}: rows of unit feature stride, jets of whole rows expected (strides {x.stride()})")
    return B, N, F


def augment_params(B: int, p_tensor: torch.Tensor, flags: int, translate_ratio: float, scale_sd: float, site: int,
                   out: Optional[torch.Tensor] = None) -> torch.Tensor:
    _chk(p_tensor, "p_tensor")
    params = out if out is not None else torch.empty((B, 6), device=p_tensor.device, dtype=torch.float32)
    assert params.shape == (B, 6) and params.is_contiguous()
    check(_lib.lib().mpg_augment(None, None, 0, 2, 2, B, 0, _p(seed_tensor(p_tensor.device)), AUG_TAG + int(site), _p(p_tensor),
                                 int(flags), translate_ratio, scale_sd, _p(params), _stream()), "mpg_augment")
    return params


def augment(x: torch.Tensor, p_tensor: torch.Tensor, flags: int, translate_ratio: float, scale_sd: float, site: int,
            out: Optional[torch.Tensor] = None, params: Optional[torch.Tensor] = None):
    B, N, F = _jet_layout(x, "x")
    _chk(p_tensor, "p_tensor")
    if out is None:
        x = x.contiguous()
        out = torch.empty_like(x)
    elif out is not x:
        _jet_layout(out, "out")
        if out.shape != x.shape or out.stride() != x.stride():
            raise ValueError("augment: out must have x's shape and strides")
    if params is None:
        params = torch.empty((B, 6), device=x.device, dtype=torch.float32)
    assert params.shape == (B, 6) and params.is_contiguous()
    check(_lib.lib().mpg_augment(_p(x), _p(out), x.stride(0), x.stride(1), F, B, N, _p(seed_tensor(x.device)), AUG_TAG + int(site),
                                 _p(p_tensor), int(flags), translate_ratio, scale_sd, _p(params), _stream()), "mpg_augment")
    return out, params


def augment_apply_reference(x: torch.Tensor, params: torch.Tensor) -> torch.Tensor:
    a00, a01, a10, a11, t0, t1 = (params[:, k].reshape(-1, 1) for k in range(6))
    x0, x1 = x[..., 0], x[..., 1]
    return torch.cat((torch.stack((a00 * x0 + a01 * x1 + t0, a10 * x0 + a11 * x1 + t1), dim=2), x[..., 2:]), dim=2)


class AugmentFn(torch.autograd.Function):

    @staticmethod
    def forward(ctx, x, p_tensor, flags, translate_ratio, scale_sd, site, params):
        y, ctx.params = augment(x, p_tensor, flags, translate_ratio, scale_sd, site, params=params)
        return y

    @staticmethod
    @once_differentiable
    def backward(ctx, dy):
        B, N, F = dy.shape
        dy = dy.contiguous()
        dx = torch.empty_like(dy)
        check(_lib.lib().mpg_augment_bwd(_p(dy), _p(dx), N * F, F, F, B, N, _p(ctx.params), _stream()), "mpg_augment_bwd")
        return dx, None, None, None, None, None, None


def dropout_mask(rows: int, F: int, tag: int, thr: int, device="cuda"):
    out = torch.empty((rows, F), device=device, dtype=torch.float32)
    check(_lib.lib().mpg_dropout_mask(_p(out), rows, F, _p(seed_tensor(device)), tag, thr, _stream()),
          "mpg_dropout_mask")
    return out


def pack_weights(W, rows, cols, *, col0=0, transpose=False, scale=1.0, f16=False):
    r, c = (cols, rows) if transpose else (rows, cols)
    MT, QT = (r + 31) // 32, (c + 31) // 32
    img = torch.empty((2 * MT * QT * 2 * 512,), device=W.device, dtype=torch.bfloat16)
    check(_lib.lib().mpg_pack_weights(_p(W, col0), W.stride(0), r, c, int(transpose), scale, int(f16),
                                      C.c_void_p(img.data_ptr()), _stream()), "mpg_pack_weights")
    return img


def _img_elems(rows, cols):
    return 2 * ((rows + 31) // 32) * ((cols + 31) // 32) * 2 * 512


PACK_MAX = 24


def refresh_many(packs):
    todo = [j for pk in packs for j in pk.jobs()]
    for i0 in range(0, len(todo), PACK_MAX):
        chunk = todo[i0:i0 + PACK_MAX]
        jobs = (MpgPackJob * len(chunk))()
        status = C.c_void_p(dev_state(chunk[0][0].device).status.data_ptr())
        for j, (W, rows, cols, tr, scale, f16, rs, sc, img) in zip(jobs, chunk):
            j.W, j.ldw, j.rows, j.cols, j.transpose = _p(W), W.stride(0), rows, cols, tr
            j.scale, j.f16, j.img, j.row_split, j.split_cols = scale, int(f16), C.c_void_p(img.data_ptr()), rs, sc
            j.status = status
        check(_lib.lib().mpg_pack_many(jobs, len(chunk), _stream()), "mpg_pack_many")
    for pk in packs:
        pk._key = pk._current_key()


class _PackedSet:

    def __init__(self, params, spec):
        self.params, self._spec = params, spec
        self.img = {k: torch.empty((_img_elems(v[1], v[2]),), device=params[0].device, dtype=torch.bfloat16) for k, v in spec.items()}
        self._key = None

    def _current_key(self):
        return tuple((q.data_ptr(), q._version) for q in self.params)

    def jobs(self):
        return [v + (self.img[k],) for k, v in self._spec.items()]

    def refresh(self):
        refresh_many([self])

    def ensure(self):
        if self._key != self._current_key():
            self.refresh()
        return self

    def ptr(self, name):
        return C.c_void_p(self.img[name].data_ptr())


class PackedMPLayer(_PackedSet):

    def __init__(self, params, F, out, dscale, f16, plist=None):
        W1, W2, W3, V1, V2, V3 = params
        self.plist = plist
        self.F, self.out, self.dscale, self.f16 = F, out, float(dscale), bool(f16)
        KN = V1.shape[1]
        super().__init__(params, {
            "W2": (W2, H2, H1, 0, dscale * SC_W2, f16, 0, 0), "W3": (W3, H3, H2, 0, dscale * SC_W3, f16, 0, 0),
            "W3T": (W3, H2, H3, 1, dscale * SC_W3, True, 0, 0), "W2T": (W2, H1, H2, 1, dscale * SC_W2, True, 0, 0),
            "V1": (V1, V1.shape[0], KN, 0, SC_WN, f16, 0, 0), "V2": (V2, V2.shape[0], V2.shape[1], 0, SC_WN, f16, 0, 0),
            "V3": (V3, out, V3.shape[1], 0, SC_WN, f16, 0, 0),
            "V3T": (V3, V3.shape[1], out, 1, 1.0, False, 0, 0), "V2T": (V2, V2.shape[1], V2.shape[0], 1, 1.0, False, 0, 0),
            "V1T": (V1, KN, V1.shape[0], 1, 1.0, False, 0, 0),
            "W1S": (W1, 2 * H1, F, 0, SC_WN, f16, H1, F),
            "W1ST": (W1, F, 2 * H1, 1, 1.0, False, H1, F),
        })


def chain(M, layers, **kw):
    c = chain_struct(M, layers, **kw)
    check(_lib.lib().mpg_chain(C.byref(c), _stream()), "mpg_chain")


def chain_struct(M, layers, *, A, lda, K1, A2=None, lda2=0, a_slabs=1, a_slab_stride=0, in_gate=None, in_out=None,
                 alpha=0.2, seed_t=None, f16=False, ascale=1.0):
    c = MpgChain()
    c.A, c.lda, c.K1 = _p(A), lda, K1
    c.A2, c.lda2 = _p(A2), lda2
    c.a_slabs, c.a_slab_stride = a_slabs, a_slab_stride
    if in_gate is not None and in_gate[1]:
        c.in_tag, c.in_thr, c.in_scale = in_gate
    if in_out is not None:
        c.in_out, c.ld_in_out = _p(in_out), in_out.stride(0)
    c.M, c.nlayers, c.alpha, c.seed, c.f16 = M, len(layers), alpha, _p(seed_t), int(f16)
    c.ascale = ascale
    for i, d in enumerate(layers):
        L = c.L[i]
        L.Wimg, L.K, L.N = d["img"], d["K"], d["N"]
        L.wscale = d.get("wscale", 1.0)
        L.bias, L.nbias, L.act = _p(d.get("bias")), d.get("nbias", 0), int(d.get("act", False))
        if d.get("drop") is not None and d["drop"][1]:
            L.drop_tag, L.drop_thr, L.drop_scale = d["drop"]
        if d.get("gate") is not None:
            H, gact, tag, thr, scale = d["gate"]
            L.gateH, L.ldh, L.gate_act = _p(H), H.stride(0), int(gact)
            if thr:
                L.gate_tag, L.gate_thr, L.gate_scale = tag, thr, scale
        if d.get("resid") is not None:
            L.resid, L.ldr = _p(d["resid"]), d["resid"].stride(0)
        if d.get("out") is not None:
            L.out, L.ldo = _p(d["out"]), d["out"].stride(0)
    return c


EDGE_SCALARS = 2
MAX_CHUNK_SENDERS_ES = 116
PARK_BYTES_PER_BLOCK = 10240
MAX_CHUNK_SENDERS = 160


def jet_order(mask2d: torch.Tensor) -> torch.Tensor:
    st = dev_state(mask2d.device)
    key = (mask2d.data_ptr(), tuple(mask2d.shape), mask2d._version)
    hit = getattr(st, "order_cache", None)
    if hit is not None and hit[0] == key:
        return hit[1]
    B, N = mask2d.shape
    order = torch.empty((B,), device=mask2d.device, dtype=torch.int32)
    check(_lib.lib().mpg_jet_order(_p(mask2d), B, N, C.c_void_p(order.data_ptr()), _stream()), "mpg_jet_order")
    st.order_cache = (key, order)
    return order


def _sender_chunks(B, N, max_chunk=None):
    RB = (N + 31) // 32
    wg = B * RB
    max_chunk = max_chunk or MAX_CHUNK_SENDERS
    forced = os.environ.get("MPG_FORCE_SC")
    if forced:
        return max(int(forced), -(-N // max_chunk))
    best, best_cost = 1, None
    for sc in range(1, max(1, N // 8) + 1):
        per = -(-N // sc)
        if per > max_chunk:
            continue
        cost = -(-wg * sc // 256) * (5 + per)
        if best_cost is None or cost < best_cost:
            best, best_cost = sc, cost
    if best_cost is None:
        best = -(-N // max_chunk)
    return best


def dw_workgroups(nblk, N):
    R = max(d for d in range(1, 7) if N % d == 0)
    nruns = nblk // R
    return min(nruns, max(256, -(-nruns // (64 // R))))


MPLayerSaved = namedtuple("MPLayerSaved", "x2 m1 ac agg h1 h2 W1 b2 b3 W2 W3 V1 V2 V3 sign3 nbr stE2 es wq xf2 order")
MPLayerCfg = namedtuple("MPLayerCfg", "B N F agg_scale alpha thr dscale tag SC f16 nq")
MPLayerSettings = namedtuple("MPLayerSettings", "sum_agg alpha p_drop training packed nbr num_knn nq handoff no_grad",
                             defaults=(None, None, 0, 0, None, False))


def mplayer_saved(node):
    return MPLayerSaved(*node.saved_tensors)


def _fn_grad_chain(ctx, gy2):
    sv, cfg, pk = mplayer_saved(ctx), ctx.cfg, ctx.packed
    V1, V2, V3, alpha, thr, dscale, tag = sv.V1, sv.V2, sv.V3, cfg.alpha, cfg.thr, cfg.dscale, cfg.tag
    V, dev = cfg.B * cfg.N, gy2.device
    n1, n2, out_f = V1.shape[0], V2.shape[0], V3.shape[0]
    dz3 = torch.empty_like(gy2) if thr else gy2
    dz2 = torch.empty((V, n2), device=dev, dtype=torch.float32)
    dz1 = torch.empty((V, n1), device=dev, dtype=torch.float32)
    dh0 = torch.empty((V, V1.shape[1]), device=dev, dtype=torch.float32)
    c = chain_struct(V, [dict(img=pk.ptr("V3T"), K=out_f, N=n2, gate=(sv.h2, True, tag + TAG_N1, thr, dscale), out=dz2),
                         dict(img=pk.ptr("V2T"), K=n2, N=n1, gate=(sv.h1, True, tag + TAG_N0, thr, dscale), out=dz1),
                         dict(img=pk.ptr("V1T"), K=n1, N=V1.shape[1], out=dh0)],
                     A=gy2, lda=gy2.stride(0), K1=out_f, in_gate=(tag + TAG_N2, thr, dscale), in_out=dz3 if thr else None,
                     alpha=alpha, seed_t=seed_tensor(dev), f16=False)
    return dz3, dz2, dz1, dh0, c


def _below_chain(prev, dx, thr, alpha, V):
    if prev is None or getattr(prev, "cfg", None) is None or getattr(prev, "packed", None) is None:
        return None
    try:
        sv, cfg = mplayer_saved(prev), prev.cfg
    except RuntimeError:
        return None
    if sv.h1 is None or sv.h2 is None or cfg.B * cfg.N != V or sv.V3.shape[0] != dx.shape[1] or (cfg.thr, cfg.alpha) != (thr, alpha):
        return None
    if not any(prev.needs_input_grad):
        return None
    return _fn_grad_chain(prev, dx)


class LayerHandoff:
    __slots__ = ("below", "above", "next", "ac_out", "node")

    def __init__(self, below=None, above=None):
        self.below, self.above, self.next, self.ac_out, self.node = below, above, None, None, None


class FusedMPLayerFn(torch.autograd.Function):

    @staticmethod
    def forward(ctx, x, mask, W1, b1, W2, b2, W3, b3, V1, c1, V2, c2, V3, c3, es, xfn, settings):
        sum_agg, alpha, p_drop, training, packed, nbr, num_knn, nq, handoff, no_grad = settings
        _chk(x, "x")
        B, N, F = x.shape
        V = B * N
        dev = x.device
        thr, dscale = drop_params(p_drop) if training else (0, 1.0)
        seed_t = seed_tensor(dev)
        tag = next_tag(dev, "mplayer", thr)
        x2 = x.reshape(V, F)
        if x2.stride(1) != 1:
            x2 = x2.contiguous()
        m1 = None if mask is None else mask.reshape(V).contiguous()
        f16 = FWD_F16
        out_f = V3.shape[0]
        if packed is None or packed.dscale != dscale or packed.f16 != f16:
            packed = PackedMPLayer((W1, W2, W3, V1, V2, V3), F, out_f, dscale, f16)
        pk = packed.ensure()

        def dr(site):
            return (tag + site, thr, dscale)

        ac = None
        below = handoff.below if handoff is not None else None
        if below is not None and below.ac_out is not None:
            ac_pre, pk_pre, x_ptr, key_pre = below.ac_out
            if pk_pre is pk and key_pre == pk._key and x_ptr == x2.data_ptr() and tuple(ac_pre.shape) == (V, 2 * H1):
                ac = ac_pre
        if ac is None:
            ac = torch.empty((V, 2 * H1), device=dev, dtype=torch.float32)
            chain(V, [dict(img=pk.ptr("W1S"), K=F, N=2 * H1, bias=b1, nbias=H1, out=ac, wscale=SC_WN)], A=x2, lda=x2.stride(0), K1=F,
                  alpha=alpha, f16=f16, ascale=SC_ACT)
        SC = _sender_chunks(B, N, MAX_CHUNK_SENDERS_ES if es is not None else None)
        aggp = torch.empty((SC, V, H3), device=dev, dtype=torch.float32)
        e = MpgEdgeFwd()
        e.a, e.c, e.ld_ac, e.mask = _p(ac), _p(ac, H1), 2 * H1, _p(m1)
        e.W2img, e.W3img = pk.ptr("W2"), pk.ptr("W3")
        e.b2, e.b3, e.agg = _p(b2), _p(b3), _p(aggp)
        e.B, e.N, e.SC = B, N, SC
        agg_scale = 1.0 if sum_agg else 1.0 / (num_knn if nbr is not None else N)
        e.alpha, e.agg_scale = alpha, agg_scale
        e.nbr = None if nbr is None else C.c_void_p(nbr.data_ptr())
        e.seed, e.tag_base, e.thr, e.dscale = _p(seed_t), tag, thr, dscale
        e.skip_masked = int(OPTIONS["skip_masked"])
        e.f16 = int(f16)
        e.two_term = int(OPTIONS["fwd_two_term"]) if es is None else 0
        wq = None
        if es is not None:
            assert 0 < nq <= EDGE_SCALARS and tuple(es.shape) == (B, N, EDGE_SCALARS, N) and W1.shape[1] == 2 * F + nq
            es = es.detach().float().contiguous()
            wq = torch.zeros((EDGE_SCALARS, H1), device=dev, dtype=torch.float32)
            wq[:nq] = W1.detach()[:, 2 * F:2 * F + nq].t()
            e.es, e.wq = _p(es), _p(wq)
        RB = (N + 31) // 32
        order = None
        if m1 is not None and OPTIONS["lpt_order"] and B * RB * SC > NUM_CUS and B + N + 2 + (B + 63) // 64 * (N + 1) <= 16384:
            order = jet_order(m1.view(B, N))
            e.order = C.c_void_p(order.data_ptr())
        need_grad = any(ctx.needs_input_grad) and not no_grad
        if need_grad and B * RB * N * PARK_BYTES_PER_BLOCK > 0x7fffffff:
            raise RuntimeError(f"FusedMPLayerFn: {B} jets x {N} particles park {B * RB * N * PARK_BYTES_PER_BLOCK / 2**30:.1f} GiB of "
                               f"edge activations for the backward, beyond the kernels' 2 GiB per launch; split the batch "
                               f"(at most {0x7fffffff // (RB * N * PARK_BYTES_PER_BLOCK)} jets per call at this size)")
        sign3 = torch.empty((B * RB * N * 192,), device=dev, dtype=torch.int32) if need_grad else None
        e.sign3 = None if sign3 is None else C.c_void_p(sign3.data_ptr())
        stE2 = torch.empty((B * RB * N, H2, 32), device=dev, dtype=torch.float16) if need_grad else None
        e.stageE2 = None if stE2 is None else C.c_void_p(stE2.data_ptr())
        xf2 = x2
        if xfn is not None:
            xf2 = xfn.detach().reshape(V, -1)
            if xf2.stride(1) != 1:
                xf2 = xf2.contiguous()
        assert V1.shape[1] == H3 + xf2.shape[1]
        n1, n2 = V1.shape[0], V2.shape[0]
        h1 = torch.empty((V, n1), device=dev, dtype=torch.float32) if need_grad else None
        h2 = torch.empty((V, n2), device=dev, dtype=torch.float32) if need_grad else None
        y = torch.empty((V, out_f), device=dev, dtype=torch.float32)
        fn_layers = [dict(img=pk.ptr("V1"), K=V1.shape[1], N=n1, bias=c1, act=True, drop=dr(TAG_N0), out=h1, wscale=SC_WN),
                     dict(img=pk.ptr("V2"), K=n1, N=n2, bias=c2, act=True, drop=dr(TAG_N1), out=h2, wscale=SC_WN),
                     dict(img=pk.ptr("V3"), K=n2, N=out_f, bias=c3, act=False, drop=dr(TAG_N2), out=y, wscale=SC_WN)]
        fn_kw = dict(A2=xf2, lda2=xf2.stride(0), alpha=alpha, seed_t=seed_t, f16=f16, ascale=SC_ACT)
        rc = _lib.MPG_FN_NA
        if OPTIONS["fn_epilogue"] and es is None and (SC == 1 or OPTIONS["fn_chunks"]):
            if SC > 1:
                e.tickets = _p(_tickets(dev, B * RB))
            if not need_grad and SC == 1:
                e.agg = None
            cs = chain_struct(V, fn_layers, A=aggp, lda=H3, K1=H3, **fn_kw)
            cs2 = ac_next = None
            if handoff is not None and handoff.next is not None and out_f % 4 == 0 and out_f <= 32:
                pk_n, b1_n = handoff.next
                if pk_n.F == out_f and pk_n.f16 == f16:
                    pk_n.ensure()
                    ac_next = torch.empty((V, 2 * H1), device=dev, dtype=torch.float32)
                    cs2 = chain_struct(V, [dict(img=pk_n.ptr("W1S"), K=out_f, N=2 * H1, bias=b1_n, nbias=H1, out=ac_next, wscale=SC_WN)],
                                       A=y, lda=out_f, K1=out_f, alpha=alpha, f16=f16, ascale=SC_ACT)
            rc = _lib.lib().mpg_edge_fwd_fn(C.byref(e), C.byref(cs), None if cs2 is None else C.byref(cs2), _stream())
            if rc != _lib.MPG_FN_NA:
                check(rc, "mpg_edge_fwd_fn")
                agg = aggp[0] if need_grad else None
                if cs2 is not None:
                    handoff.ac_out = (ac_next, pk_n, y.data_ptr(), pk_n._key)
        if rc == _lib.MPG_FN_NA:
            e.agg = _p(aggp)
            check(_lib.lib().mpg_edge_fwd(C.byref(e), _stream()), "mpg_edge_fwd")
            agg = aggp[0]
            for q in range(1, SC):
                agg = agg + aggp[q]
            chain(V, fn_layers, A=agg, lda=H3, K1=H3, **fn_kw)
        ctx.packed = pk
        ctx.prev_node = below.node if (below is not None and need_grad and x.grad_fn is below.node) else None
        ctx.pre = None
        if handoff is not None and need_grad:
            handoff.node = ctx

        if need_grad and dev_state(dev).sign_tap is not None:
            dev_state(dev).sign_tap.append(dict(B=B, N=N, ac=ac, stE2=stE2, sign3=sign3, h1=h1, h2=h2))
        ctx.save_for_backward(*MPLayerSaved(x2, m1, ac, agg, h1, h2, W1, b2, b3, W2, W3, V1, V2, V3, sign3, nbr, stE2, es, wq, xf2, order))
        ctx.cfg = MPLayerCfg(B, N, F, agg_scale, alpha, thr, dscale, tag, SC, f16, nq)
        return y.reshape(B, N, V3.shape[0])

    @staticmethod
    @once_differentiable
    def backward(ctx, gy):
        x2, m1, ac, agg, h1, h2, W1, b2, b3, W2, W3, V1, V2, V3, sign3, nbr, stE2, es, wq, xf2, order = mplayer_saved(ctx)
        pk = ctx.packed
        B, N, F, agg_scale, alpha, thr, dscale, tag, SC, f16, nq = ctx.cfg
        nbr_p = None if nbr is None else C.c_void_p(nbr.data_ptr())
        V = B * N
        dev = x2.device
        seed_t = seed_tensor(dev)
        gy2 = gy.reshape(V, -1).contiguous()

        def gt(H, site, act):
            return (H, H.stride(0), act, seed_t, tag + site, thr, dscale)

        need_x, _, *need_p, _, need_xfn, _ = ctx.needs_input_grad
        need_w = any(need_p)

        n1, n2, out_f = V1.shape[0], V2.shape[0], V3.shape[0]
        pre, fnb = ctx.pre, None
        ctx.pre = None
        if pre is not None and pre["gy_ptr"] == gy2.data_ptr() and tuple(gy2.shape) == (V, out_f):
            dz3, dz2, dz1, dh0 = pre["dz3"], pre["dz2"], pre["dz1"], pre["dh0"]
        else:
            dz3, dz2, dz1, dh0, fnb = _fn_grad_chain(ctx, gy2)
        dV1 = dV2 = dV3 = dc1 = dc2 = dc3 = None
        wb = WgradBatch()
        direct = (need_w and dev_state(dev).grad_into_param and pk.plist is not None
                  and all(q.grad is not None and q.grad.is_contiguous() for q in pk.plist))
        if need_w:
            if direct:
                gW1, gb1, gW2, gb2, gW3, gb3, dV1, dc1, dV2, dc2, dV3, dc3 = (q.grad for q in pk.plist)
            else:
                dc3, dc2, dc1 = (torch.empty(t.shape[1], device=dev, dtype=torch.float32) for t in (dz3, dz2, dz1))
                dV3, dV2, dV1 = torch.empty_like(V3), torch.empty_like(V2), torch.empty_like(V1)
            wb.add(dz3, h2, out=dV3, bias_out=dc3, accumulate=direct)
            wb.add(dz2, h1, out=dV2, bias_out=dc2, accumulate=direct)
            wb.add(dz1, agg, out=dV1, out_col0=0, bias_out=dc1, accumulate=direct)
            wb.add(dz1, xf2, out=dV1, out_col0=H3, accumulate=direct)

        RB = (N + 31) // 32
        nblk = B * RB * N
        dap = torch.empty((SC, V, H1), device=dev, dtype=torch.float32)
        dcp = torch.empty((RB, V, H1), device=dev, dtype=torch.float32)
        stZ2 = None
        if need_w:
            stZ2 = torch.empty((nblk, H2, 32), device=dev, dtype=torch.float16)
            gexp = torch.empty((B * RB,), device=dev, dtype=torch.int32)
        e = MpgEdgeBwd()
        e.a, e.c, e.ld_ac, e.mask = _p(ac), _p(ac, H1), 2 * H1, _p(m1)
        e.dagg, e.ld_dagg = _p(dh0), dh0.stride(0)
        e.sign3 = C.c_void_p(sign3.data_ptr())
        e.W2img = pk.ptr("W2")
        e.W3Timg, e.W2Timg = pk.ptr("W3T"), pk.ptr("W2T")
        e.b2 = _p(b2)
        e.da, e.dc = _p(dap), _p(dcp)
        e.stageE2 = C.c_void_p(stE2.data_ptr())
        e.stageZ2 = None if stZ2 is None else C.c_void_p(stZ2.data_ptr())
        e.gexp = None if stZ2 is None else C.c_void_p(gexp.data_ptr())
        e.B, e.N, e.SC = B, N, SC
        e.alpha, e.agg_scale, e.nbr = alpha, agg_scale, nbr_p
        e.seed, e.tag_base, e.thr, e.dscale = _p(seed_t), tag, thr, dscale
        e.f16 = int(f16)
        if order is not None:
            e.order = C.c_void_p(order.data_ptr())
        des = daq = None
        if es is not None:
            des = torch.zeros_like(es)
            daq = torch.empty((SC, V, EDGE_SCALARS, H1), device=dev, dtype=torch.float32)
            e.es, e.wq, e.des, e.daq = _p(es), _p(wq), _p(des), _p(daq)
        if fnb is not None:
            check(_lib.lib().mpg_chain(C.byref(fnb), _stream()), "mpg_chain")
        dx = cdx = None
        rc = _lib.MPG_FN_NA
        if need_x:
            dx = torch.empty((V, F), device=dev, dtype=torch.float32)
            if SC == 1 and RB == 1:
                cdx = chain_struct(V, [dict(img=pk.ptr("W1ST"), K=2 * H1, N=F, resid=dh0[:, H3:H3 + F], out=dx)],
                                   A=dap, lda=H1, K1=H1, A2=dcp, lda2=H1, alpha=alpha, f16=False)
            if cdx is not None and OPTIONS["bwd_epilogue"] and es is None:
                below = _below_chain(ctx.prev_node, dx, thr, alpha, V)
                rc = _lib.lib().mpg_edge_bwd_fn(C.byref(e), C.byref(cdx), None if below is None else C.byref(below[4]), _stream())
                if rc == _lib.MPG_FN_NA and below is not None:
                    below = None
                    rc = _lib.lib().mpg_edge_bwd_fn(C.byref(e), C.byref(cdx), None, _stream())
                if rc != _lib.MPG_FN_NA:
                    check(rc, "mpg_edge_bwd_fn")
                    if below is not None:
                        ctx.prev_node.pre = dict(gy_ptr=dx.data_ptr(), keep=dx, dz3=below[0], dz2=below[1], dz1=below[2], dh0=below[3])
        if rc == _lib.MPG_FN_NA:
            check(_lib.lib().mpg_edge_bwd(C.byref(e), _stream()), "mpg_edge_bwd")
        if SC == 1 and RB == 1:
            da, dc, dadc = dap[0], dcp[0], None
        else:
            dadc = torch.empty((V, 2 * H1), device=dev, dtype=torch.float32)
            check(_lib.lib().mpg_slab_sums(_p(dap), SC, V * H1, _p(dcp), RB, V * H1, _p(dadc), V, H1, _stream()), "mpg_slab_sums")
            da, dc = dadc[:, :H1], dadc[:, H1:]
        dW1 = db1 = dW2 = db2 = dW3 = db3 = None
        st_dev = dev_state(dev)
        side = st_dev.wgrad_stream if (need_w and direct and es is None) else None
        main = torch.cuda.current_stream(dev) if side is not None else None
        if need_w:
            nwg = dw_workgroups(nblk, N)
            part = torch.empty((nwg, H3 * H2 + H2 * H1 + H3 + H2), device=dev, dtype=torch.float32)
            if direct:
                dW3, dW2, db3, db2 = gW3, gW2, gb3, gb2
            else:
                dW3, dW2 = torch.empty_like(W3), torch.empty_like(W2)
                db3, db2 = torch.empty_like(b3), torch.empty_like(b2)
            d = MpgEdgeDw()
            d.a, d.c, d.ld_ac, d.mask = _p(ac), _p(ac, H1), 2 * H1, _p(m1)
            d.dagg, d.ld_dagg = _p(dh0), dh0.stride(0)
            d.sign3 = C.c_void_p(sign3.data_ptr())
            d.stageE2, d.stageZ2 = C.c_void_p(stE2.data_ptr()), C.c_void_p(stZ2.data_ptr())
            d.gexp = C.c_void_p(gexp.data_ptr())
            d.part, d.nwg = _p(part), nwg
            d.dW3, d.dW2, d.db3, d.db2, d.accumulate = _p(dW3), _p(dW2), _p(db3), _p(db2), int(direct)
            d.B, d.N = B, N
            d.alpha, d.agg_scale, d.nbr = alpha, agg_scale, nbr_p
            d.seed, d.tag_base, d.thr, d.dscale = _p(seed_t), tag, thr, dscale
            d.f16 = int(f16)
            d.defer_reduce = int(OPTIONS["dw_reduce_grouped"])
            if es is not None:
                d.es, d.wq = _p(es), _p(wq)
            if direct:
                dW1, db1 = gW1, gb1
            else:
                dW1 = torch.empty_like(W1)
                db1 = torch.empty(H1, device=dev, dtype=torch.float32)
            wb.add(da, x2, out=dW1, out_col0=0, bias_out=db1, accumulate=direct)
            wb.add(dc, x2, out=dW1, out_col0=F, accumulate=direct)
            if side is not None:
                st_dev.wgrad_keep.append((ac, m1, dh0, sign3, stE2, stZ2, gexp, part, da, dc, dap, dcp, dadc, x2, xf2, agg, h1, h2,
                                          dz1, dz2, dz3, gy2, nbr, [j[7] for j in wb.jobs]))
                side.wait_stream(main)
                with torch.cuda.stream(side):
                    check(_lib.lib().mpg_edge_dw(C.byref(d), _stream()), "mpg_edge_dw")
                    wb.flush(dw=d if d.defer_reduce else None)
            else:
                check(_lib.lib().mpg_edge_dw(C.byref(d), _stream()), "mpg_edge_dw")
                wb.flush(dw=d if d.defer_reduce else None)
            del stZ2
            if es is not None:
                dWq = daq.sum((0, 1))[:nq].t()
                if direct:
                    dW1[:, 2 * F:2 * F + nq] += dWq
                else:
                    dW1[:, 2 * F:2 * F + nq] = dWq
            if direct:
                dW1 = db1 = dW2 = db2 = dW3 = db3 = dV1 = dc1 = dV2 = dc2 = dV3 = dc3 = None
        if need_x:
            if rc == _lib.MPG_FN_NA:
                if dadc is not None:
                    chain(V, [dict(img=pk.ptr("W1ST"), K=2 * H1, N=F, resid=dh0[:, H3:H3 + F], out=dx)],
                          A=dadc, lda=2 * H1, K1=2 * H1, alpha=alpha, f16=False)
                else:
                    chain(V, [dict(img=pk.ptr("W1ST"), K=2 * H1, N=F, resid=dh0[:, H3:H3 + F], out=dx)],
                          A=dap, lda=H1, K1=H1, A2=dc, lda2=dc.stride(0), alpha=alpha, f16=False)
            dx = dx.reshape(B, N, F)
        dxfn = None
        if need_xfn and dh0.shape[1] > H3 + F:
            dxfn = torch.cat((torch.zeros((V, F), device=dev, dtype=torch.float32), dh0[:, H3 + F:]), dim=1).reshape(B, N, -1)
        return dx, None, dW1, db1, dW2, db2, dW3, db3, dV1, dc1, dV2, dc2, dV3, dc3, des, dxfn, None


def _grad_target(t):
    if t is None:
        return None
    if t.is_leaf:
        return t.grad if (t.grad is not None and t.grad.is_contiguous()) else None
    base = t._base
    if base is None or not base.is_leaf or base.grad is None or not t.is_contiguous() or not base.grad.is_contiguous():
        return None
    return base.grad.as_strided(t.size(), t.stride(), t.storage_offset() - base.storage_offset() + base.grad.storage_offset())


def _deferred_targets(st, params):
    if not st.grad_into_param or st.deferred_wgrad is None:
        return None
    targets = [_grad_target(q) for q in params]
    return None if any(t is None for t in targets) else (targets, st.deferred_wgrad)


class FusedLinearFn(torch.autograd.Function):

    @staticmethod
    def forward(ctx, x, W, b, act, alpha, p_drop, training, resid=None):
        _chk(x, "x")
        shp = x.shape
        x2 = x.reshape(-1, shp[-1])
        if x2.stride(1) != 1 or x2.stride(0) < shp[-1]:
            x2 = x2.contiguous()
        thr, dscale = drop_params(p_drop) if training else (0, 1.0)
        seed_t = seed_tensor(x.device)
        tag = next_tag(x.device, "linear", thr)
        if resid is not None and act:
            raise NotImplementedError("FusedLinearFn: a fused residual needs a layer without activation")
        r2 = None if resid is None else resid.reshape(-1, W.shape[0]).contiguous()
        y = linear_fwd(x2, W, b, act=act, alpha=alpha, drop=(seed_t, tag + TAG_GENERIC, thr, dscale) if thr else None,
                       resid=r2)
        ctx.has_resid = resid is not None
        ctx.save_for_backward(x2, W, y)
        ctx.wparam, ctx.bias = W, b
        ctx.cfg = (shp, act, alpha, thr, dscale, tag, b is not None)
        return y.reshape(*shp[:-1], W.shape[0])

    @staticmethod
    @once_differentiable
    def backward(ctx, gy):
        x2, W, y = ctx.saved_tensors
        shp, act, alpha, thr, dscale, tag, has_b = ctx.cfg
        g2 = gy.reshape(-1, W.shape[0]).contiguous()
        if act or thr:
            g2 = gate(g2, y, gate_act=act, alpha=alpha, seed_t=seed_tensor(g2.device), tag=tag + TAG_GENERIC,
                      thr=thr, scale=dscale)
        dW = db = None
        want_b = has_b and ctx.needs_input_grad[2]
        queue = None
        if ctx.needs_input_grad[1]:
            queue = _deferred_targets(dev_state(g2.device), [ctx.wparam, ctx.bias] if want_b else [ctx.wparam])
        if queue is not None:
            targets, batch = queue
            batch.add(g2, x2, out=targets[0], bias_out=targets[1] if want_b else None, accumulate=True)
        elif ctx.needs_input_grad[1]:
            if want_b:
                db = torch.empty(W.shape[0], device=g2.device, dtype=torch.float32)
            dW = linear_bwd_weight(g2, x2, bias_out=db)
        elif want_b:
            db = g2.sum(0)
        dx = linear_bwd_data(g2, W).reshape(shp) if ctx.needs_input_grad[0] else None
        return dx, dW, db, None, None, None, None, (gy if ctx.has_resid else None)


class MatMulFn(torch.autograd.Function):

    @staticmethod
    def forward(ctx, A, B, form):
        _chk(A, "A"); _chk(B, "B")
        A, B = A.contiguous(), B.contiguous()
        ctx.form = form
        ctx.save_for_backward(A, B)
        if form == "nt":
            return linear_fwd(A, B, None, f16=False)
        if form == "nn":
            return linear_bwd_data(A, B)
        if form == "tn":
            return linear_bwd_weight(A, B)
        raise ValueError(f"MatMulFn: form must be nt / nn / tn, got {form!r}")

    @staticmethod
    def backward(ctx, G):
        A, B = ctx.saved_tensors
        nA, nB = ctx.needs_input_grad[0], ctx.needs_input_grad[1]
        mm = MatMulFn.apply
        if ctx.form == "nt":
            return (mm(G, B, "nn") if nA else None), (mm(G, A, "tn") if nB else None), None
        if ctx.form == "nn":
            return (mm(G, B, "nt") if nA else None), (mm(A, G, "tn") if nB else None), None
        return (mm(B, G, "nt") if nA else None), (mm(A, G, "nn") if nB else None), None


class double_backward_route:

    def __init__(self, device="cuda"):
        self.state = dev_state(device)

    def __enter__(self):
        self.prev, self.state.double_backward = self.state.double_backward, True
        return self

    def __exit__(self, *exc):
        self.state.double_backward = self.prev
        return False


def double_backward_on(device) -> bool:
    return dev_state(device).double_backward


class FusedDropoutFn(torch.autograd.Function):

    @staticmethod
    def forward(ctx, x, p_drop, training):
        thr, scale = drop_params(p_drop) if training else (0, 1.0)
        if not thr:
            ctx.cfg = None
            return x
        _chk(x, "x")
        x2 = x.reshape(-1, x.shape[-1]).contiguous()
        tag = next_tag(x.device, "dropout", thr) + TAG_GENERIC
        ctx.cfg = (tag, thr, scale, x.shape)
        return gate(x2, None, gate_act=False, alpha=0.0, seed_t=seed_tensor(x.device), tag=tag, thr=thr,
                    scale=scale).reshape(x.shape)

    @staticmethod
    @once_differentiable
    def backward(ctx, g):
        if ctx.cfg is None:
            return g, None, None
        tag, thr, scale, shp = ctx.cfg
        g2 = g.reshape(-1, shp[-1]).contiguous()
        return gate(g2, None, gate_act=False, alpha=0.0, seed_t=seed_tensor(g.device), tag=tag, thr=thr,
                    scale=scale).reshape(shp), None, None


def _attn_struct(q, k, v, ignore, o, P, B, L, S, H, d):
    a = _lib.MpgAttn()
    a.q, a.k, a.v = _p(q), _p(k), _p(v)
    a.ldq, a.ldk, a.ldv = q.stride(0), k.stride(0), v.stride(0)
    a.ignore = _p(ignore)
    a.o, a.ldo, a.P = _p(o), o.stride(0), _p(P)
    a.B, a.L, a.S, a.H, a.d = B, L, S, H, d
    return a


class FusedPackedAttnFn(torch.autograd.Function):

    @staticmethod
    def forward(ctx, qx, kv, ignore, B, L, S, H):
        _chk(qx, "qkv")
        self_attn = kv is None
        E = qx.shape[1] // 3 if self_attn else qx.shape[1]
        d = E // H
        q = qx[:, :E]
        k, v = (qx[:, E:2 * E], qx[:, 2 * E:]) if self_attn else (kv[:, :E], kv[:, E:])
        o = torch.empty((B * L, E), device=qx.device, dtype=torch.float32)
        P = torch.empty((B, H, L, S), device=qx.device, dtype=torch.float32)
        a = _attn_struct(q, k, v, ignore, o, P, B, L, S, H, d)
        check(_lib.lib().mpg_attn_fwd(C.byref(a), _stream()), "mpg_attn_fwd")
        ctx.save_for_backward(qx, kv, P)
        ctx.ignore = ignore
        ctx.dims = (B, L, S, H, d, E, self_attn)
        return o

    @staticmethod
    @once_differentiable
    def backward(ctx, go):
        qx, kv, P = ctx.saved_tensors
        B, L, S, H, d, E, self_attn = ctx.dims
        go = go.contiguous()
        dqx = torch.empty_like(qx)
        dkv = None if self_attn else torch.empty_like(kv)
        q = qx[:, :E]
        k, v = (qx[:, E:2 * E], qx[:, 2 * E:]) if self_attn else (kv[:, :E], kv[:, E:])
        dq = dqx[:, :E]
        dk, dv = (dqx[:, E:2 * E], dqx[:, 2 * E:]) if self_attn else (dkv[:, :E], dkv[:, E:])
        a = _attn_struct(q, k, v, ctx.ignore, go, P, B, L, S, H, d)
        a.d_o = _p(go)
        a.dq, a.dk, a.dv = C.c_void_p(dq.data_ptr()), C.c_void_p(dk.data_ptr()), C.c_void_p(dv.data_ptr())
        a.lddq, a.lddk, a.lddv = dq.stride(0), dk.stride(0), dv.stride(0)
        check(_lib.lib().mpg_attn_bwd(C.byref(a), _stream()), "mpg_attn_bwd")
        return dqx, dkv, None, None, None, None, None


class FusedAttnFn(torch.autograd.Function):

    @staticmethod
    def forward(ctx, q, k, v, ignore, B, L, S, H):
        _chk(q, "q")
        E = q.shape[1]
        d = E // H
        o = torch.empty((B * L, E), device=q.device, dtype=torch.float32)
        P = torch.empty((B, H, L, S), device=q.device, dtype=torch.float32)
        a = _attn_struct(q, k, v, ignore, o, P, B, L, S, H, d)
        check(_lib.lib().mpg_attn_fwd(C.byref(a), _stream()), "mpg_attn_fwd")
        ctx.save_for_backward(q, k, v, P)
        ctx.ignore = ignore
        ctx.dims = (B, L, S, H, d)
        return o

    @staticmethod
    @once_differentiable
    def backward(ctx, go):
        q, k, v, P = ctx.saved_tensors
        B, L, S, H, d = ctx.dims
        go = go.contiguous()
        dq = torch.empty((B * L, H * d), device=q.device, dtype=torch.float32)
        dk = torch.empty((B * S, H * d), device=q.device, dtype=torch.float32)
        dv = torch.empty((B * S, H * d), device=q.device, dtype=torch.float32)
        a = _attn_struct(q, k, v, ctx.ignore, go, P, B, L, S, H, d)
        a.d_o = _p(go)
        a.dq, a.dk, a.dv = _p(dq), _p(dk), _p(dv)
        a.lddq, a.lddk, a.lddv = H * d, H * d, H * d
        check(_lib.lib().mpg_attn_bwd(C.byref(a), _stream()), "mpg_attn_bwd")
        return dq, dk, dv, None, None, None, None, None


class PackedMAB(_PackedSet):

    def __init__(self, Win, Wo, Wf):
        E = Wo.shape[0]
        super().__init__((Win, Wo, Wf), {
            "Win": (Win, 3 * E, E, 0, SC_WN, True, 0, 0), "Wo": (Wo, E, E, 0, SC_WN, True, 0, 0), "Wf": (Wf, E, E, 0, SC_WN, True, 0, 0),
            "WinT": (Win, E, 3 * E, 1, 1.0, False, 0, 0), "WoT": (Wo, E, E, 1, 1.0, False, 0, 0), "WfT": (Wf, E, E, 1, 1.0, False, 0, 0),
        })


def mab_fusable(E: int, H: int, L: int, S: int) -> bool:
    return E in (32, 64) and H * 16 == E and 1 <= L <= MAB_MAX_TOKENS and 1 <= S <= MAB_MAX_TOKENS


MAB_MAX_TOKENS = 160
MAB_CHAIN_TOKENS = 32

MABParams = namedtuple("MABParams", "Win bin Wo bo Wf bf")
MABCfg = namedtuple("MABCfg", "B L S E H alpha ff_act tag p_mab p_ff")
MABSaved = namedtuple("MABSaved", "x2 y2 ignore o z za n1w n1b n2w n2b", defaults=(None,) * 5)


def _groups(seq, n):
    return [tuple(seq[i:i + n]) for i in range(0, len(seq), n)]


def mab_saved(node):
    return MABSaved(*node.saved_tensors)


def _mab_cfg(dev, B, L, S, E, H, alpha, ff_act, p_mab, p_ff, training):
    p_mab, p_ff = (p_mab, p_ff) if training else (0.0, 0.0)
    tag = next_tag(dev, "mab", max(drop_params(p_mab)[0], drop_params(p_ff)[0]))
    return MABCfg(B, L, S, E, H, alpha, ff_act, tag, p_mab, p_ff)


def _mab_struct(cfg, x2, y2, ignore, pk, prm, ln=None):
    m = _lib.MpgMab()
    m.x, m.ldx = _p(x2), x2.stride(0)
    m.y, m.ldy = (_p(x2), x2.stride(0)) if y2 is None else (_p(y2), y2.stride(0))
    m.ignore = _p(ignore)
    m.Win, m.bin, m.Wo, m.bo, m.Wf, m.bf = pk.ptr("Win"), _p(prm.bin), pk.ptr("Wo"), _p(prm.bo), pk.ptr("Wf"), _p(prm.bf)
    m.WinT, m.WoT, m.WfT = pk.ptr("WinT"), pk.ptr("WoT"), pk.ptr("WfT")
    m.B, m.L, m.S, m.E, m.H = cfg.B, cfg.L, cfg.S, cfg.E, cfg.H
    m.alpha, m.ff_act = cfg.alpha, int(cfg.ff_act)
    m.seed, m.tag = _p(seed_tensor(x2.device)), cfg.tag
    (m.thr_mab, m.sc_mab), (m.thr_ff, m.sc_ff) = drop_params(cfg.p_mab), drop_params(cfg.p_ff)
    m.wscale, m.ascale = SC_WN, SC_ACT
    if ln is not None:
        w1, b1, w2, b2, eps = ln
        m.ln1_w, m.ln1_b, m.ln2_w, m.ln2_b, m.ln_eps = _p(w1), _p(b1), _p(w2), _p(b2), float(eps)
    return m


def mab_forward(cfg, x2, y2, ignore, pk, prm, *, save=False, ln=None):
    _chk(x2, "x")
    out = torch.empty((cfg.B * cfg.L, cfg.E), device=x2.device, dtype=torch.float32)
    o = torch.empty_like(out) if save else None
    z = torch.empty_like(out) if save else None
    za = torch.empty_like(out) if (save and ln is not None) else None
    m = _mab_struct(cfg, x2, y2, ignore, pk, prm, ln)
    m.out, m.ldo, m.save_o, m.save_z, m.save_za = _p(out), out.stride(0), _p(o), _p(z), _p(za)
    check(_lib.lib().mpg_mab_fwd(C.byref(m), _stream()), "mpg_mab_fwd")
    return out, MABSaved(x2, y2, ignore, o, z, za, *(ln[:4] if ln is not None else ()))


def _mab_rows(x, y):
    B, L, E = x.shape
    shared = B == 1 and L == 1 and y is not None and y.shape[0] > 1
    if shared:
        B = y.shape[0]
    S = L if y is None else y.shape[1]
    x2 = x.reshape(1, E).contiguous().expand(B, E) if shared else x.reshape(B * L, E).contiguous()
    y2 = None if y is None else y.reshape(B * S, E).contiguous()
    return x2, y2, B, L, S, shared


def _mab_run(x, y, ignore, pk, prm, ln, H, alpha, ff_act, p_mab, p_ff, training, save):
    x2, y2, B, L, S, shared = _mab_rows(x, y)
    cfg = _mab_cfg(x.device, B, L, S, x.shape[2], H, alpha, ff_act, p_mab, p_ff, training)
    out, saved = mab_forward(cfg, x2, y2, ignore, pk, prm, save=save, ln=ln)
    return out.reshape(B, L, cfg.E), saved, cfg, shared


def mab_block(x, y, ignore, pk, prm, ln, H, alpha, ff_act, p_mab, p_ff, training):
    if not torch.is_grad_enabled():
        return _mab_run(x, y, ignore, pk, prm, ln, H, alpha, ff_act, p_mab, p_ff, training, False)[0]
    if ln is not None and x.shape[0] == 1 and y is not None and y.shape[0] > 1:
        x = x.expand(y.shape[0], -1, -1)
    return FusedMABFn.apply(x, y, ignore, *prm, *(ln if ln is not None else (None,) * 5), H, alpha, ff_act, p_mab, p_ff, training, pk)


def _ln_param_grads(dn, gn, w, b, need_w, need_b):
    st = dev_state(dn.device)
    E = dn.shape[1]
    out = [None, None]
    for k, (rows, prm, need) in enumerate(((gn, w, need_w), (dn, b, need_b))):
        if not need:
            continue
        queue = _deferred_targets(st, [prm])
        if queue is not None:
            queue[1].add(rows, rows[:, :1], out=torch.empty((E, 1), device=dn.device, dtype=torch.float32),
                         bias_out=queue[0][0].reshape(-1), accumulate=True)
        else:
            out[k] = rows.sum(0)
    return out


def _mab_backward_block(cfg, sv, prm, pk, gout, need_x, need_y, need_w, eps=None, need_ln=False):
    B, L, S, E = cfg.B, cfg.L, cfg.S, cfg.E
    x2, y2, o, z = sv.x2, sv.y2, sv.o, sv.z
    dev = x2.device
    cross = y2 is not None
    dout = gout.reshape(B * L, E).contiguous()
    m = _mab_struct(cfg, x2, y2, sv.ignore, pk, prm, None if sv.n1w is None else (sv.n1w, sv.n1b, sv.n2w, sv.n2b, eps))
    m.save_o, m.save_z, m.save_za = _p(o), _p(z), _p(sv.za)
    m.dout, m.lddout = _p(dout), dout.stride(0)
    dx = torch.empty((B * L, E), device=dev, dtype=torch.float32) if need_x else None
    dy = torch.empty((B * S, E), device=dev, dtype=torch.float32) if (cross and need_y) else None
    m.dx, m.lddx, m.dy, m.lddy = _p(dx), E, _p(dy), E
    dqkv = dq = dkv = dza = du = None
    if need_w:
        if cross:
            dq = torch.empty((B * L, E), device=dev, dtype=torch.float32)
            dkv = torch.empty((B * S, 2 * E), device=dev, dtype=torch.float32)
            m.dq, m.lddq, m.dk, m.dv, m.lddkv = _p(dq), E, _p(dkv), _p(dkv, E), 2 * E
        else:
            dqkv = torch.empty((B * L, 3 * E), device=dev, dtype=torch.float32)
            m.dq, m.lddq, m.dk, m.dv, m.lddkv = _p(dqkv), 3 * E, _p(dqkv, E), _p(dqkv, 2 * E), 3 * E
        dza, du = torch.empty_like(dout), torch.empty_like(dout)
        m.dza, m.du = _p(dza), _p(du)
    elif L > 32 or S > 32:
        dza = torch.empty_like(dout)
        m.dza = _p(dza)
    lnrows = None
    if need_ln:
        lnrows = tuple(torch.empty((B * L, E), device=dev, dtype=torch.float32) for _ in range(4))
        m.dn1, m.gn1, m.dn2, m.gn2 = (_p(t) for t in lnrows)
    check(_lib.lib().mpg_mab_bwd(C.byref(m), _stream()), "mpg_mab_bwd")
    grads = [None] * 6
    if need_w:
        queue = _deferred_targets(dev_state(dev), prm)
        if queue is not None:
            g, wb = MABParams(*queue[0]), queue[1]
            if cross:
                wb.add(dq, x2, out=g.Win[:E], bias_out=g.bin[:E], accumulate=True)
                wb.add(dkv, y2, out=g.Win[E:], bias_out=g.bin[E:], accumulate=True)
            else:
                wb.add(dqkv, x2, out=g.Win, bias_out=g.bin, accumulate=True)
            wb.add(dza, o, out=g.Wo, bias_out=g.bo, accumulate=True)
            wb.add(du, z, out=g.Wf, bias_out=g.bf, accumulate=True)
        else:
            def wgrad(dyv, xv):
                db = torch.empty(dyv.shape[1], device=dev, dtype=torch.float32)
                return linear_bwd_weight(dyv, xv, bias_out=db), db
            if cross:
                (wq, bq), (wkv, bkv) = wgrad(dq, x2), wgrad(dkv, y2)
                grads[0], grads[1] = torch.cat([wq, wkv], 0), torch.cat([bq, bkv], 0)
            else:
                grads[0], grads[1] = wgrad(dqkv, x2)
            grads[2], grads[3] = wgrad(dza, o)
            grads[4], grads[5] = wgrad(du, z)
    return dx, dy, grads, lnrows


def sab_chain_forward(x, ignore, H, alpha, ff_act, p_mab, p_ff, training, pks, blocks, save=False):
    B, L, E = x.shape
    dev = x.device
    c = _lib.MpgMabChain()
    c.n = len(pks)
    inp, saved, cfgs = x.reshape(B * L, E).contiguous(), [], []
    for b, (pk, prm) in enumerate(zip(pks, blocks)):
        cfg = _mab_cfg(dev, B, L, L, E, H, alpha, ff_act, p_mab, p_ff, training)
        out = torch.empty((B * L, E), device=dev, dtype=torch.float32)
        o, z = (torch.empty_like(out), torch.empty_like(out)) if save else (None, None)
        m = _mab_struct(cfg, inp, None, ignore, pk, prm)
        m.out, m.ldo, m.save_o, m.save_z = _p(out), E, _p(o), _p(z)
        c.blk[b] = m
        saved.append(MABSaved(inp, None, ignore, o, z))
        cfgs.append(cfg)
        inp = out
    check(_lib.lib().mpg_mab_chain_fwd(C.byref(c), _stream()), "mpg_mab_chain_fwd")
    return inp.reshape(B, L, E), saved, cfgs


class FusedSABChainFn(torch.autograd.Function):

    @staticmethod
    def forward(ctx, x, ignore, H, alpha, ff_act, p_mab, p_ff, training, pks, *params):
        ctx.blocks = [MABParams(*g) for g in _groups(params, len(MABParams._fields))]
        out, saved, ctx.cfgs = sab_chain_forward(x, ignore, H, alpha, ff_act, p_mab, p_ff, training, pks, ctx.blocks, save=True)
        ctx.save_for_backward(ignore, *(t for sv in saved for t in (sv.x2, sv.o, sv.z)))
        ctx.pks = pks
        return out

    @staticmethod
    @once_differentiable
    def backward(ctx, gout):
        ignore, *rows = ctx.saved_tensors
        saved = [MABSaved(x2=x2, y2=None, ignore=ignore, o=o, z=z) for x2, o, z in _groups(rows, 3)]
        need_params = _groups(ctx.needs_input_grad[9:], len(MABParams._fields))
        g, all_grads = gout, []
        for b in reversed(range(len(saved))):
            need_x = b > 0 or ctx.needs_input_grad[0]
            g, _, grads, _ = _mab_backward_block(ctx.cfgs[b], saved[b], ctx.blocks[b], ctx.pks[b], g, need_x, False, any(need_params[b]))
            all_grads[:0] = grads
        return (None if g is None else g.reshape(gout.shape), None, None, None, None, None, None, None, None, *all_grads)


class FusedMABFn(torch.autograd.Function):

    @staticmethod
    def forward(ctx, x, y, ignore, Win, bin_, Wo, bo, Wf, bf, n1w, n1b, n2w, n2b, eps, H, alpha, ff_act, p_mab, p_ff, training, pk):
        ctx.params = MABParams(Win, bin_, Wo, bo, Wf, bf)
        ln = None if n1w is None else (n1w, n1b, n2w, n2b, eps)
        out, saved, ctx.cfg, ctx.shared = _mab_run(x, y, ignore, pk, ctx.params, ln, H, alpha, ff_act, p_mab, p_ff, training, True)
        ctx.save_for_backward(*saved)
        ctx.pk, ctx.eps = pk, eps
        ctx.seed = x if (ctx.shared and x.is_leaf) else None
        return out

    @staticmethod
    @once_differentiable
    def backward(ctx, gout):
        sv, cfg, need = MABSaved(*ctx.saved_tensors), ctx.cfg, ctx.needs_input_grad
        dx, dy, grads, rows = _mab_backward_block(cfg, sv, ctx.params, ctx.pk, gout, need[0], need[1], any(need[3:9]),
                                                  eps=ctx.eps, need_ln=any(need[9:13]))
        gln = [None] * 4
        if rows is not None:
            gln = (_ln_param_grads(rows[0], rows[1], sv.n1w, sv.n1b, need[9], need[10])
                   + _ln_param_grads(rows[2], rows[3], sv.n2w, sv.n2b, need[11], need[12]))
        if ctx.shared and dx is not None:
            queue = _deferred_targets(dev_state(dx.device), [ctx.seed]) if ctx.seed is not None else None
            if queue is not None:
                queue[1].add(dx, dx[:, :1], out=torch.empty((cfg.E, 1), device=dx.device, dtype=torch.float32),
                             bias_out=queue[0][0].reshape(-1), accumulate=True)
                dx = None
            else:
                dx = dx.sum(0).reshape(1, 1, cfg.E)
        elif dx is not None:
            dx = dx.reshape(cfg.B, cfg.L, cfg.E)
        return (dx, None if dy is None else dy.reshape(cfg.B, cfg.S, cfg.E), None, *grads, *gln, None, None, None, None, None, None, None, None)


def rank_mask(first_feature: torch.Tensor, labels: torch.Tensor, num_particles: int, out: Optional[torch.Tensor] = None,
              with_ignore: bool = False, ignore_out: Optional[torch.Tensor] = None):
    _chk(first_feature, "first_feature")
    B, N = first_feature.shape
    lab = labels[:, -1]
    if lab.dtype != torch.float32:
        lab = lab.float()
    if out is None:
        out = torch.empty((B, N), device=first_feature.device, dtype=torch.float32)
    ign = ignore_out if ignore_out is not None else (torch.empty((B, N), device=first_feature.device, dtype=torch.float32) if with_ignore else None)
    assert out.is_contiguous() and (ign is None or ign.is_contiguous())
    check(_lib.lib().mpg_rank_mask(_p(first_feature), first_feature.stride(0), first_feature.stride(1), _p(lab), lab.stride(0),
                                   B, N, _p(out), _p(ign), _stream()), "mpg_rank_mask")
    return (out, ign) if (with_ignore or ignore_out is not None) else out


def knn_sets(x: torch.Tensor, mask: Optional[torch.Tensor], num_knn: int, self_loops: bool = True):
    _chk(x, "x")
    B, N, F = x.shape
    x2 = x.reshape(B * N, F)
    if x2.stride(1) != 1:
        x2 = x2.contiguous()
    m1 = None if mask is None else mask.reshape(B * N).contiguous()
    nbr = torch.empty((B * N, (N + 31) // 32), device=x.device, dtype=torch.int32)
    check(_lib.lib().mpg_knn_sets(_p(x2), x2.stride(0), _p(m1), B, N, F, num_knn, int(self_loops),
                                  C.c_void_p(nbr.data_ptr()), _stream()), "mpg_knn_sets")
    return nbr


ACT_CODES = {"": 0, "tanh": 1, "sigmoid": 2}


def gen_tail_into(y, mask, act: int, out):
    B, N, F = y.shape
    y2 = y.reshape(B * N, F)
    if y2.stride(1) != 1:
        y2 = y2.contiguous()
    assert out.shape == (B, N, F + (mask is not None)) and out.stride(2) == 1 and out.stride(0) == N * out.stride(1)
    m1 = None if mask is None else mask.reshape(B * N)
    check(_lib.lib().mpg_gen_tail_fwd(_p(y2), y2.stride(0), _p(m1), _p(out), out.stride(1), B * N, F, act, _stream()),
          "mpg_gen_tail_fwd")
    return out


class GenTailFn(torch.autograd.Function):

    @staticmethod
    def forward(ctx, y, mask, act):
        _chk(y, "y")
        B, N, F = y.shape
        out = torch.empty((B, N, F + (mask is not None)), device=y.device, dtype=torch.float32)
        gen_tail_into(y, mask, act, out)
        ctx.save_for_backward(out)
        ctx.cfg = (B, N, F, act)
        return out

    @staticmethod
    @once_differentiable
    def backward(ctx, dout):
        (out,) = ctx.saved_tensors
        B, N, F, act = ctx.cfg
        if dout.stride(2) != 1 or dout.stride(0) != N * dout.stride(1):
            dout = dout.contiguous()
        dy = torch.empty((B * N, F), device=out.device, dtype=torch.float32)
        check(_lib.lib().mpg_gen_tail_bwd(_p(dout), dout.stride(1), _p(out), out.stride(1), _p(dy), F, B * N, F, act, _stream()),
              "mpg_gen_tail_bwd")
        return dy.reshape(B, N, F), None, None


def bridge_fusable(K: int, F: int, E: int) -> bool:
    return K == 64 and E == 64 and (1 <= F <= 4 or F == 8)


class GenDiscBridgeFn(torch.autograd.Function):

    @staticmethod
    def forward(ctx, pre, W1, b1, feat_buf, W2, b2, act1, act2, alpha, p_drop, training):
        _chk(pre, "pre")
        Bg, N, K = pre.shape
        F, E = W1.shape[0], W2.shape[0]
        pre2 = pre.reshape(Bg * N, K)
        if pre2.stride(1) != 1 or pre2.stride(0) % 4:
            pre2 = pre2.contiguous()
        if feat_buf is None:
            feat = torch.empty((Bg, N, F), device=pre.device, dtype=torch.float32)
        else:
            feat = feat_buf
            assert feat.is_contiguous() and feat.shape[1:] == (N, F) and feat.shape[0] >= Bg
        B = feat.shape[0]
        e = torch.empty((B, N, E), device=pre.device, dtype=torch.float32)
        thr, dscale = drop_params(p_drop) if training else (0, 1.0)
        tag = next_tag(pre.device, "bridge", thr) + TAG_GENERIC
        q = _lib.MpgBridge()
        q.x, q.ldx, q.W1, q.b1, q.act1 = _p(pre2), pre2.stride(0), _p(W1), _p(b1), int(act1)
        q.feat, q.ldf = _p(feat), F
        q.M, q.row0, q.K, q.F, q.E = B * N, (B - Bg) * N, K, F, E
        q.W2, q.b2, q.act2, q.alpha = _p(W2), _p(b2), int(act2), alpha
        q.seed, q.tag, q.thr, q.dscale = _p(seed_tensor(pre.device)), tag, thr, dscale
        q.e, q.lde = _p(e), E
        check(_lib.lib().mpg_bridge_fwd(q, _stream()), "mpg_bridge_fwd")
        ctx.save_for_backward(pre2, W1, W2, feat, e)
        ctx.set_materialize_grads(False)
        ctx.params = (W1, b1, W2, b2)
        ctx.cfg = (Bg, B, N, K, F, E, int(act1), int(act2), alpha, thr, dscale, tag)
        return (feat if feat_buf is None else None), e

    @staticmethod
    @once_differentiable
    def backward(ctx, gfeat, ge):
        pre2, W1s, W2s, feat, e = ctx.saved_tensors
        W1, b1, W2, b2 = ctx.params
        Bg, B, N, K, F, E, act1, act2, alpha, thr, dscale, tag = ctx.cfg
        need = ctx.needs_input_grad
        if ge is None:
            ge = torch.zeros((B, N, E), device=pre2.device, dtype=torch.float32)
        want1 = need[1] or (b1 is not None and need[2])
        want2 = need[4] or (b2 is not None and need[5])
        M, row0 = B * N, (B - Bg) * N
        dev = pre2.device
        ge2 = ge.reshape(M, E)
        if ge2.stride(1) != 1 or ge2.stride(0) % 4:
            ge2 = ge2.contiguous()
        g2 = torch.empty((M, E), device=dev, dtype=torch.float32) if want2 else None
        g1 = torch.empty((Bg * N, F), device=dev, dtype=torch.float32) if want1 else None
        dx = torch.empty((Bg * N, K), device=dev, dtype=torch.float32) if need[0] else None
        gf = None
        if gfeat is not None and (want1 or need[0]):
            gf = gfeat.reshape(-1, F)[row0:] if gfeat.shape[0] == B else gfeat.reshape(-1, F)
            gf = gf.contiguous()
        q = _lib.MpgBridgeBwd()
        q.ge, q.ldge, q.e, q.lde, q.feat, q.ldf = _p(ge2), ge2.stride(0), _p(e), E, _p(feat), F
        q.gfeat, q.ldgf, q.W1, q.W2 = _p(gf), F, _p(W1s), _p(W2s)
        q.M, q.row0, q.K, q.F, q.E, q.act1, q.act2, q.alpha = M, row0, K, F, E, act1, act2, alpha
        q.seed, q.tag, q.thr, q.dscale = _p(seed_tensor(dev)), tag, thr, dscale
        q.g2, q.ldg2, q.g1, q.ldg1, q.dx, q.lddx = _p(g2), E, _p(g1), F, _p(dx), K
        if want1 or want2 or need[0]:
            check(_lib.lib().mpg_bridge_bwd(q, _stream()), "mpg_bridge_bwd")
        st = dev_state(dev)
        outs = {}
        for key, g, xin, W, b, nW, nb in (("1", g1, pre2, W1, b1, need[1], b1 is not None and need[2]),
                                          ("2", g2, feat.reshape(M, F), W2, b2, need[4], b2 is not None and need[5])):
            dW = db = None
            if g is not None:
                queue = _deferred_targets(st, [W, b] if nb else [W]) if nW else None
                if queue is not None:
                    targets, batch = queue
                    batch.add(g, xin, out=targets[0], bias_out=targets[1] if nb else None, accumulate=True)
                elif nW:
                    if nb:
                        db = torch.empty(W.shape[0], device=dev, dtype=torch.float32)
                    dW = linear_bwd_weight(g, xin, bias_out=db)
                elif nb:
                    db = g.sum(0)
            outs[key] = (dW, db)
        return (None if dx is None else dx.reshape(Bg, N, K), outs["1"][0], outs["1"][1], None, outs["2"][0], outs["2"][1],
                None, None, None, None, None)


LOSS_CODES = {"ls": 0, "og": 1, "w": 2, "hinge": 3}


def _head_struct(y, mask, w, b, mean, sigmoid, p_drop, training, tag, out, pooled, aux):
    B, N, F = y.shape
    h = _lib.MpgDiscHead()
    h.y, h.ldy, h.mask = _p(y), y.stride(1), _p(mask)
    h.w, h.bias = _p(w), _p(b)
    h.B, h.N, h.F, h.mean, h.sigmoid = B, N, F, int(mean), int(sigmoid)
    thr, dscale = drop_params(p_drop) if training else (0, 1.0)
    h.seed, h.tag, h.thr, h.dscale = _p(seed_tensor(y.device)), tag, thr, dscale
    h.out, h.pooled, h.aux = _p(out), _p(pooled), _p(aux)
    h.loss = -1
    return h


def _head_inputs(y, mask):
    _chk(y, "y")
    B, N, F = y.shape
    if y.stride(2) != 1 or y.stride(0) != N * y.stride(1):
        y = y.contiguous()
    m = None if mask is None else mask.reshape(B, N)
    if m is not None and not m.is_contiguous():
        m = m.contiguous()
    return y, m


class DiscHeadFn(torch.autograd.Function):

    @staticmethod
    def forward(ctx, y, mask, w, b, mean, sigmoid, p_drop, training):
        y, m = _head_inputs(y, mask)
        B, N, F = y.shape
        dev = y.device
        out = torch.empty((B,), device=dev, dtype=torch.float32)
        pooled = torch.empty((B, F), device=dev, dtype=torch.float32)
        aux = torch.empty((2 * B,), device=dev, dtype=torch.float32)
        tag = next_tag(dev, "head", drop_params(p_drop)[0] if training else 0) + TAG_GENERIC
        wv = w.reshape(-1)
        h = _head_struct(y, m, wv, b, mean, sigmoid, p_drop, training, tag, out, pooled, aux)
        check(_lib.lib().mpg_disc_head_fwd(C.byref(h), _stream()), "mpg_disc_head_fwd")
        ctx.save_for_backward(y, m, w, b, out, pooled, aux)
        ctx.cfg = (mean, sigmoid, p_drop, training, tag)
        return out

    @staticmethod
    @once_differentiable
    def backward(ctx, gout):
        y, m, w, b, out, pooled, aux = ctx.saved_tensors
        mean, sigmoid, p_drop, training, tag = ctx.cfg
        B, N, F = y.shape
        dev = y.device
        h = _head_struct(y, m, w.reshape(-1), b, mean, sigmoid, p_drop, training, tag, out, pooled, aux)
        gout = gout.contiguous()
        h.gout = _p(gout)
        dy = torch.empty((B, N, F), device=dev, dtype=torch.float32) if ctx.needs_input_grad[0] else None
        h.dy, h.ld_dy = _p(dy), F
        dw = db = None
        if ctx.needs_input_grad[2]:
            st = dev_state(dev)
            gw = _grad_target(w) if st.grad_into_param else None
            gb = _grad_target(b) if (st.grad_into_param and b is not None) else None
            if gw is not None and (b is None or gb is not None):
                h.dw, h.db, h.accumulate = _p(gw), _p(gb), 1
            else:
                dw = torch.empty_like(w)
                db = None if b is None else torch.empty_like(b)
                h.dw, h.db, h.accumulate = _p(dw), _p(db), 0
        check(_lib.lib().mpg_disc_head_bwd(C.byref(h), _stream()), "mpg_disc_head_bwd")
        return dy, None, dw, db, None, None, None, None


def disc_head_loss(y, mask, w, b, *, mean, sigmoid, p_drop, training, loss, n_real, gen_step, count, loss_out,
                   want_dy=True, wgrad=None):
    y, m = _head_inputs(y, mask)
    B, N, F = y.shape
    dev = y.device
    out = torch.empty((B,), device=dev, dtype=torch.float32)
    pooled = torch.empty((B, F), device=dev, dtype=torch.float32)
    aux = torch.empty((2 * B,), device=dev, dtype=torch.float32)
    terms = torch.empty((B,), device=dev, dtype=torch.float32)
    tag = next_tag(dev, "head", drop_params(p_drop)[0] if training else 0) + TAG_GENERIC
    h = _head_struct(y, m, w.reshape(-1), b, mean, sigmoid, p_drop, training, tag, out, pooled, aux)
    h.loss, h.gen_step, h.n_real, h.inv_count = LOSS_CODES[loss], int(gen_step), n_real, 1.0 / count
    h.terms, h.loss_out = _p(terms), _p(loss_out)
    dy = torch.empty((B, N, F), device=dev, dtype=torch.float32) if want_dy else None
    h.dy, h.ld_dy = _p(dy), F
    if wgrad is not None:
        h.dw, h.db, h.accumulate = _p(wgrad[0]), _p(wgrad[1]), 1
    check(_lib.lib().mpg_disc_head_loss(C.byref(h), _stream()), "mpg_disc_head_loss")
    return out, dy


class BatchNormFn(torch.autograd.Function):

    @staticmethod
    def forward(ctx, x, w, b, eps):
        _chk(x, "x")
        x2 = x.contiguous()
        M, F = x2.shape
        nchunk = max(1, min(256, M // 64))
        part = torch.empty((nchunk, F), device=x.device, dtype=torch.float32)
        mean, var = (torch.empty(F, device=x.device, dtype=torch.float32) for _ in range(2))
        check(_lib.lib().mpg_batchnorm_stats(_p(x2), x2.stride(0), M, F, _p(part), nchunk, _p(mean), _p(var), _stream()),
              "mpg_batchnorm_stats")
        y = torch.empty_like(x2)
        check(_lib.lib().mpg_batchnorm_apply(_p(x2), x2.stride(0), _p(mean), _p(var), _p(w), _p(b), eps, _p(y), y.stride(0), M, F,
                                             _stream()), "mpg_batchnorm_apply")
        ctx.save_for_backward(x2, w, mean, var)
        ctx.eps, ctx.params = eps, (w, b)
        ctx.mark_non_differentiable(mean, var)
        return y, mean, var

    @staticmethod
    @once_differentiable
    def backward(ctx, g, _gm, _gv):
        x2, w, mean, var = ctx.saved_tensors
        M, F = x2.shape
        g2 = g.contiguous()
        nchunk = max(1, min(256, M // 64))
        part = torch.empty((2 * nchunk, F), device=g.device, dtype=torch.float32)
        sums = torch.empty(2 * F, device=g.device, dtype=torch.float32)
        dx = torch.empty_like(x2) if ctx.needs_input_grad[0] else None
        wp, bp = ctx.params
        st = dev_state(g.device)
        wanted = ctx.needs_input_grad[1] or ctx.needs_input_grad[2]
        gw = _grad_target(wp) if (st.grad_into_param and wanted) else None
        gb = _grad_target(bp) if (st.grad_into_param and wanted) else None
        direct = gw is not None and gb is not None
        dw = gw if direct else torch.empty(F, device=g.device, dtype=torch.float32)
        db = gb if direct else torch.empty(F, device=g.device, dtype=torch.float32)
        check(_lib.lib().mpg_batchnorm_bwd(_p(g2), g2.stride(0), _p(x2), x2.stride(0), _p(mean), _p(var), _p(w), ctx.eps, _p(part), nchunk,
                                           _p(sums), _p(dx), F, _p(dw), _p(db), int(direct), M, F, _stream()), "mpg_batchnorm_bwd")
        return dx, (None if direct else dw), (None if direct else db), None


def batchnorm_eval(x, w, b, mean, var, eps):
    x2 = x.contiguous()
    M, F = x2.shape
    y = torch.empty_like(x2)
    check(_lib.lib().mpg_batchnorm_apply(_p(x2), x2.stride(0), _p(mean), _p(var), _p(w), _p(b), eps, _p(y), y.stride(0), M, F, _stream()),
          "mpg_batchnorm_apply")
    return y


class LayerNormFn(torch.autograd.Function):

    @staticmethod
    def forward(ctx, x, w, b, eps):
        _chk(x, "x")
        shp = x.shape
        E = shp[-1]
        x2 = x.reshape(-1, E)
        if x2.stride(1) != 1:
            x2 = x2.contiguous()
        M = x2.shape[0]
        y = torch.empty((M, E), device=x.device, dtype=torch.float32)
        stats = torch.empty((M, 2), device=x.device, dtype=torch.float32)
        check(_lib.lib().mpg_layernorm_fwd(_p(x2), x2.stride(0), _p(w), _p(b), _p(y), E, _p(stats), M, E, eps, _stream()),
              "mpg_layernorm_fwd")
        ctx.save_for_backward(x2, w, stats)
        ctx.params = (w, b)
        ctx.shp = shp
        return y.reshape(shp)

    @staticmethod
    @once_differentiable
    def backward(ctx, g):
        x2, w, stats = ctx.saved_tensors
        M, E = x2.shape
        g2 = g.reshape(M, E)
        if g2.stride(1) != 1:
            g2 = g2.contiguous()
        dx = torch.empty((M, E), device=g.device, dtype=torch.float32)
        nwaves = 4 * min(256, (M + 3) // 4)
        part = torch.empty((nwaves, 2, E), device=g.device, dtype=torch.float32)
        st = dev_state(g.device)
        wp, bp = ctx.params
        dw = db = None
        if not (ctx.needs_input_grad[1] or ctx.needs_input_grad[2]):
            tw = tb = None
            acc = 0
        else:
            gw = _grad_target(wp) if st.grad_into_param else None
            gb = _grad_target(bp) if st.grad_into_param else None
            if gw is not None and gb is not None:
                tw, tb, acc = gw, gb, 1
            else:
                dw, db = torch.empty_like(w), torch.empty_like(w)
                tw, tb, acc = dw, db, 0
        check(_lib.lib().mpg_layernorm_bwd(_p(g2), g2.stride(0), _p(x2), x2.stride(0), _p(w), _p(stats), _p(dx), E, _p(part),
                                           nwaves, _p(tw), _p(tb), acc, M, E, _stream()), "mpg_layernorm_bwd")
        return dx.reshape(ctx.shp), dw, db, None
```

mpgan_amd/train.py:

```python
from __future__ import annotations

import ctypes as C
import os
from dataclasses import dataclass
from types import SimpleNamespace
from typing import Optional

import torch
from torch import nn

from . import _lib, ops, dist as mdist
from .mpgan import MPGenerator, MPDiscriminator, augment as maugment

LR = {
    "g": (3e-5, 1e-5), "t": (6e-5, 2e-5), "q": (1.5e-5, 0.5e-5),
}


def default_mpgan(num_particles: int = 30, disc_dropout: float = 0.5, gen_dropout: float = 0.0, device="cuda",
                  loss: str = "ls", spectral_norm_gen: bool = False, spectral_norm_disc: bool = False,
                  batch_norm_gen: bool = False, batch_norm_disc: bool = False):
    def lin(p, bn=False, sn=False):
        return {"leaky_relu_alpha": 0.2, "dropout_p": p, "batch_norm": bn, "spectral_norm": sn}
    mp_args = {"pos_diffs": False, "all_ef": False, "coords": "polarrel", "delta_coords": False, "delta_r": False,
               "int_diffs": False, "clabels": 0, "mask_fne_np": False, "fully_connected": True, "num_knn": 10,
               "self_loops": True, "sum": True}
    common = {"num_particles": num_particles, "hidden_node_size": 32, "fe_layers": [96, 160, 192],
              "fn_layers": [256, 256], "fn1_layers": None}
    mask_args = {"mask_feat": False, "mask_feat_bin": False, "mask_weights": False, "mask_manual": False,
                 "mask_exp": False, "mask_real_only": False, "mask_learn": False, "mask_learn_bin": True,
                 "mask_learn_sep": False, "fmg": [64], "mask_disc_sep": False, "mask_fnd_np": False,
                 "mask_c": True, "mask_fne_np": False}
    G = MPGenerator(mp_iters=2, fe1_layers=None, final_activation="tanh", output_node_size=3, input_node_size=32,
                    lfc=False, lfc_latent_size=128, **common, mp_args=dict(mp_args),
                    mp_args_first_layer={"clabels": 0}, linear_args=lin(gen_dropout, batch_norm_gen, spectral_norm_gen),
                    mask_args=dict(mask_args))
    D = MPDiscriminator(mp_iters=2, fe1_layers=None, final_activation="" if loss in ("w", "hinge") else "sigmoid",
                        input_node_size=3, dea=True,
                        dea_sum=True, fnd=[], mask_fnd_np=False, **common, mp_args=dict(mp_args),
                        mp_args_first_layer={"clabels": 0, "all_ef": False},
                        linear_args=lin(disc_dropout, batch_norm_disc, spectral_norm_disc), mask_args=dict(mask_args))
    return G.to(device), D.to(device)


def default_gapt(num_particles: int = 30, disc_dropout: float = 0.5, gen_dropout: float = 0.0, device="cuda",
                 use_isab: bool = False):
    from .gapt import GAPT_G, GAPT_D

    def lin(p):
        return {"leaky_relu_alpha": 0.2, "dropout_p": p, "batch_norm": False, "spectral_norm": False}
    common = {"num_particles": num_particles, "num_heads": 4, "embed_dim": 64, "sab_fc_layers": [],
              "use_mask": True, "use_isab": use_isab, "num_isab_nodes": 10}
    G = GAPT_G(sab_layers=4, output_feat_size=3, final_fc_layers=[], dropout_p=gen_dropout, layer_norm=False,
               **common, linear_args=lin(gen_dropout))
    D = GAPT_D(sab_layers=2, input_feat_size=3, final_fc_layers=[], dropout_p=disc_dropout, layer_norm=False,
               **common, linear_args=lin(disc_dropout))
    return G.to(device), D.to(device)


LR_GAPT = (1.5e-4, 0.5e-4)


OPTIMIZERS = ("rmsprop", "adam", "adadelta")


class FlatParams:

    def __init__(self, module: nn.Module, optimizer: str = "rmsprop", betas=(0.9, 0.999), weight_decay: float = 5e-4):
        if optimizer not in OPTIMIZERS:
            raise ValueError(f"optimizer must be one of {OPTIMIZERS}, got {optimizer!r}")
        all_ps = list(module.parameters())
        self._trained_idx = [i for i, p in enumerate(all_ps) if p.requires_grad]
        self._n_all = len(all_ps)
        ps = [all_ps[i] for i in self._trained_idx]
        if not ps:
            raise ValueError("FlatParams: the module has no trainable parameter")
        self.params = ps
        self.module = module
        self.optimizer, self.betas, self.weight_decay = optimizer, tuple(betas), float(weight_decay)
        n = sum(p.numel() for p in ps)
        dev = ps[0].device
        self.flat = torch.empty(n, device=dev, dtype=torch.float32)
        self.grad = torch.zeros(n, device=dev, dtype=torch.float32)
        self.sq = torch.zeros(n, device=dev, dtype=torch.float32)
        self.aux = torch.zeros(n, device=dev, dtype=torch.float32) if optimizer != "rmsprop" else None
        self.step_count = torch.zeros((), device=dev, dtype=torch.float32)
        self._host_steps = 0
        self._spans = []
        off = 0
        for p in ps:
            k = p.numel()
            self.flat[off:off + k].copy_(p.data.reshape(-1))
            p.data = self.flat[off:off + k].view_as(p)
            p.grad = self.grad[off:off + k].view_as(p)
            self._spans.append((off, k, tuple(p.shape)))
            off += k
        self.n = n
        self.lr = None
        self.seed_device = None
        self.seed_rank = 0

    def zero_grad(self):
        self.grad.zero_()

    def step(self, lr: float, gscale: float = 1.0, zero_grad: bool = False, advance_seed: torch.Tensor = None):
        self.lr = lr
        vp = lambda t: C.c_void_p(t.data_ptr())
        st = C.c_void_p(torch.cuda.current_stream().cuda_stream)
        L = _lib.lib()
        z = int(zero_grad)
        cnt, add = (None, 0) if advance_seed is None else (vp(advance_seed), ops.SEED_STEP)
        if self.optimizer == "rmsprop":
            _lib.check(L.mpg_rmsprop(vp(self.flat), vp(self.grad), vp(self.sq), self.n, lr, 0.99, 1e-8, gscale, z, cnt, add, st),
                       "mpg_rmsprop")
        elif self.optimizer == "adam":
            _lib.check(L.mpg_adam(vp(self.flat), vp(self.grad), vp(self.aux), vp(self.sq), vp(self.step_count), self.n,
                                  lr, self.betas[0], self.betas[1], 1e-8, self.weight_decay, gscale, z, cnt, add, st), "mpg_adam")
        else:
            _lib.check(L.mpg_adadelta(vp(self.flat), vp(self.grad), vp(self.sq), vp(self.aux), self.n, lr, 0.9, 1e-6,
                                      gscale, z, cnt, add, st), "mpg_adadelta")
        if not (self.flat.is_cuda and torch.cuda.is_current_stream_capturing()):
            self._host_steps += 1

    def note_step(self):
        self._host_steps += 1

    @property
    def steps(self) -> float:
        return float(self.step_count) if self.optimizer == "adam" else float(self._host_steps)

    def rmsprop(self, lr: float, alpha: float = 0.99, eps: float = 1e-8, gscale: float = 1.0):
        assert self.optimizer == "rmsprop" and alpha == 0.99 and eps == 1e-8
        self.step(lr, gscale)

    _STATE_KEYS = {"rmsprop": ("square_avg", None), "adam": ("exp_avg_sq", "exp_avg"), "adadelta": ("square_avg", "acc_delta")}
    SEED_KEY = "mpgan_amd_seed"
    SEED_RANK_KEY = "mpgan_amd_seed_rank"

    def _torch_optimizer(self, lr):
        stand_ins = [torch.zeros(shape) for _, _, shape in self._spans]
        if self.optimizer == "rmsprop":
            return torch.optim.RMSprop(stand_ins, lr=lr)
        if self.optimizer == "adam":
            return torch.optim.Adam(stand_ins, lr=lr, weight_decay=self.weight_decay, betas=self.betas)
        return torch.optim.Adadelta(stand_ins, lr=lr)

    def state_dict(self, lr: float = None, filtered: bool = True) -> dict:
        lr = self.lr if lr is None else lr
        sd = self._torch_optimizer(1e-2 if lr is None else lr).state_dict()
        k_sq, k_aux = self._STATE_KEYS[self.optimizer]
        steps = torch.tensor(self.steps, dtype=torch.float32)
        if not filtered:
            sd["param_groups"][0]["params"] = list(range(self._n_all))
        if float(steps) > 0:
            for i, (off, k, shape) in enumerate(self._spans):
                ent = {"step": steps.clone(), k_sq: self.sq[off:off + k].view(shape).clone()}
                if k_aux is not None:
                    ent[k_aux] = self.aux[off:off + k].view(shape).clone()
                sd["state"][i if filtered else self._trained_idx[i]] = ent
        if self.seed_device is not None:
            sd["param_groups"][0][self.SEED_KEY] = ops.get_seed(self.seed_device)
            sd["param_groups"][0][self.SEED_RANK_KEY] = int(self.seed_rank)
        return sd

    def load_state_dict(self, sd: dict):
        k_sq, k_aux = self._STATE_KEYS[self.optimizer]
        state = sd["state"]
        groups = sd.get("param_groups") or [{}]
        n_listed = sum(len(g.get("params", ())) for g in groups)
        if n_listed == len(self._spans) or (n_listed == 0 and len(state) <= len(self._spans)):
            index = list(range(len(self._spans)))
        elif n_listed == self._n_all:
            index = self._trained_idx
        else:
            raise ValueError(f"optimizer state lists {n_listed} parameters; the module has {len(self._spans)} trainable "
                             f"of {self._n_all}")
        known = set(index)
        stray = [k for k in state if int(k) not in known]
        if stray:
            raise ValueError(f"optimizer state has entries for parameters {stray} that are not trained here")
        self.sq.zero_()
        if self.aux is not None:
            self.aux.zero_()
        steps = 0.0
        for (off, k, shape), i in zip(self._spans, index):
            ent = state.get(i, state.get(str(i)))
            if ent is None:
                continue
            if k_sq not in ent:
                raise ValueError(f"state of parameter {i} has no {k_sq!r}: not a torch.optim {self.optimizer} state dict")
            if tuple(ent[k_sq].shape) != shape:
                raise ValueError(f"state of parameter {i} has shape {tuple(ent[k_sq].shape)}, expected {shape}")
            self.sq[off:off + k].copy_(ent[k_sq].reshape(-1))
            if k_aux is not None:
                self.aux[off:off + k].copy_(ent[k_aux].reshape(-1))
            steps = max(steps, float(ent.get("step", 0.0)))
        self.step_count.fill_(steps)
        self._host_steps = int(steps)
        self.lr = groups[0].get("lr", self.lr)
        if self.seed_device is not None and self.SEED_KEY in groups[0]:
            ops.set_seed(ops.rerank_seed(int(groups[0][self.SEED_KEY]), int(groups[0].get(self.SEED_RANK_KEY, 0)), self.seed_rank),
                         self.seed_device)
        return self.lr

    def versions(self) -> int:
        return sum(p._version for p in self.params)


def _set_requires_grad(flat: "FlatParams", flag: bool):
    for p in flat.params:
        p.requires_grad_(flag)


def _forward_writes_no_state(module: nn.Module) -> bool:
    from .mpgan.model import LinearNet, SpectralNorm
    for m in module.modules():
        if isinstance(m, (SpectralNorm, nn.modules.batchnorm._BatchNorm)) or (isinstance(m, LinearNet) and not m.plain):
            return False
    return True


LOSSES = ("ls", "og", "w", "hinge")


@dataclass
class Augment:
    aug_r90: bool = False
    aug_f: bool = False
    aug_t: bool = False
    aug_s: bool = False
    translate_ratio: float = 0.125
    scale_sd: float = 0.125
    aug_prob: float = 1.0


AUG_SITES = {"D_fake": 0, "G_fake": 1, "D_real": 2}


def d_loss(loss: str, out: torch.Tensor, B: int, real: Optional[torch.Tensor] = None) -> torch.Tensor:
    out = out.reshape(-1)
    if real is None:
        real = (torch.arange(2 * B, device=out.device) < B).to(out.dtype)
    if loss == "ls":
        return ((out - real) ** 2).sum() / B
    if loss == "og":
        return torch.nn.functional.binary_cross_entropy(out, real, reduction="sum") / B
    sign = 1.0 - 2.0 * real
    if loss == "w":
        return (sign * out).sum() / B
    if loss == "hinge":
        return torch.relu(1.0 + sign * out).sum() / B
    raise ValueError(f"loss must be one of {LOSSES}, got {loss!r}")


def g_loss(loss: str, out: torch.Tensor) -> torch.Tensor:
    out = out.reshape(-1)
    if loss == "ls":
        return ((out - 1.0) ** 2).mean()
    if loss == "og":
        return torch.nn.functional.binary_cross_entropy(out, torch.ones_like(out))
    if loss in ("w", "hinge"):
        return -out.mean()
    raise ValueError(f"loss must be one of {LOSSES}, got {loss!r}")


class _GenAhead:

    def __init__(self, dev):
        self.dev = dev
        self.stream = None
        self.jets = None
        self.open = False
        self.joined = None

    def fork(self, generate):
        if self.stream is None:
            self.stream = torch.cuda.Stream(device=self.dev)
        main = torch.cuda.current_stream(self.dev)
        self.stream.wait_stream(main)
        self.open = True
        with torch.cuda.stream(self.stream):
            self.jets = generate()
        for t in (self.jets if isinstance(self.jets, tuple) else (self.jets,)):
            if t is not None:
                t.record_stream(main)

    def join(self, place: str):
        if self.open:
            torch.cuda.current_stream(self.dev).wait_stream(self.stream)
            self.open, self.joined = False, place

    def take(self):
        jets, self.jets = self.jets, None
        return jets


class TrainStep:

    def __init__(self, G: nn.Module, D: nn.Module, batch_size: int, num_particles: int, latent: int = 32,
                 lr_disc: float = 3e-5, lr_gen: float = 1e-5, noise_std: float = 0.2, use_graphs: bool = True,
                 process_group=None, world_size: int = 1, batch_real_fake: bool = True, loss: str = "ls",
                 optimizer: str = "rmsprop", betas=(0.9, 0.999), gp_lambda: float = 0.0,
                 graph_collectives: Optional[bool] = None, augment=None, loader=None):
        if loss not in LOSSES:
            raise ValueError(f"loss must be one of {LOSSES}, got {loss!r}")
        self.dev = dev = next(G.parameters()).device
        gpu = dev.type == "cuda"

        def _switch(name: str, default: str = "1") -> str:
            return os.environ.get(name, default)
        on = {k: _switch(k) != "0" for k in ("MPG_PARTS", "MPG_GEN_AHEAD", "MPG_GEN_AHEAD_LATE", "MPG_WGRAD_SIDE", "MPG_BRIDGE", "MPG_NOISE_MASK")}
        if graph_collectives is None:
            graph_collectives = _switch("MPG_GRAPH_COLLECTIVES", "") == "1"
        self.split_graphs = bool(_switch("MPG_SPLIT_GRAPHS", ""))
        self.gp_lambda = float(gp_lambda)
        self.GP = torch.zeros((), device=dev)
        self.fixed_alpha = None
        self.G, self.D = G, D
        self.loss = loss
        self.batch_real_fake = batch_real_fake and not any(isinstance(m, nn.modules.batchnorm._BatchNorm) for m in D.modules())
        self.B, self.N, self.latent = batch_size, num_particles, latent
        self.lr_disc, self.lr_gen, self.noise_std = lr_disc, lr_gen, noise_std
        self.pg, self.world = process_group, world_size
        self.graph_collectives = bool(graph_collectives) and process_group is not None
        self.state = ops.dev_state(dev)
        self.fG = FlatParams(G, optimizer, betas)
        self.fD = FlatParams(D, optimizer, betas)
        if gpu:
            rank = 0
            if torch.distributed.is_available() and torch.distributed.is_initialized():
                rank = torch.distributed.get_rank(process_group)
            key = (torch.initial_seed(), rank)
            if self.state.seed_is_default and self.state.auto_seed_key != key:
                ops.set_seed(ops.derived_seed(*key), dev, _auto=True)
                self.state.auto_seed_key = key
            self.fG.seed_device = dev
            self.fG.seed_rank = rank
            ops.reserve_tickets(dev, 2 * batch_size * ((num_particles + 31) // 32))
        self.data = torch.zeros(batch_size, num_particles, 4, device=dev)
        self.labels = torch.zeros(batch_size, 1, device=dev)
        self._real = torch.cat([torch.ones(batch_size, device=dev), torch.zeros(batch_size, device=dev)])
        self._dcat = torch.zeros(2 * batch_size, num_particles, 4, device=dev)
        self._labels2 = torch.zeros(2 * batch_size, 1, device=dev)
        self._x3 = torch.zeros(2 * batch_size, num_particles, 3, device=dev)
        self._mask2 = torch.zeros(2 * batch_size, num_particles, 1, device=dev)
        self._ign2 = torch.zeros(2 * batch_size, num_particles, device=dev)
        self.parts = (gpu and hasattr(G, "generate_parts") and hasattr(D, "features_parts") and D.parts_ok()
                      and getattr(G, "use_mask", True) and not getattr(G, "lfc", False)
                      and getattr(G, "mask_args", {}).get("mask_c", True) and on["MPG_PARTS"])
        self.D_loss = torch.zeros((), device=dev)
        self.G_loss = torch.zeros((), device=dev)
        self.use_graphs = use_graphs and gpu
        self._graphs = None
        self.gen_ahead = gpu and isinstance(G, MPGenerator) and _forward_writes_no_state(G) and on["MPG_GEN_AHEAD"]
        self._ahead = _GenAhead(dev)
        self.wgrad_side = gpu and on["MPG_WGRAD_SIDE"]
        self._wside = None
        self.gen_ahead_late = self.gen_ahead and self.wgrad_side and on["MPG_GEN_AHEAD_LATE"]
        self.bridge = gpu and on["MPG_BRIDGE"]
        self.aug = self.aug_p = None
        if augment is not None:
            flags = ops.augment_flags(augment.aug_r90, augment.aug_f, augment.aug_t, augment.aug_s)
            self.aug_p = torch.full((1,), float(augment.aug_prob), device=dev)
            if flags:
                self.aug = SimpleNamespace(flags=flags, translate_ratio=float(augment.translate_ratio), scale_sd=float(augment.scale_sd))
                self.aug_params = [torch.zeros(batch_size, 6, device=dev) for _ in AUG_SITES]
        self.noise_mask = gpu and on["MPG_NOISE_MASK"]
        self.fixed_noise = None
        self._seen_versions = (self.fD.versions(), self.fG.versions())
        self._clean = {"D": True, "G": True}
        self.loader = None
        if loader is not None:
            self.attach_loader(loader)

    @property
    def gen_join(self):
        return self._ahead.joined

    def attach_loader(self, loader):
        if self._graphs is not None:
            raise RuntimeError("attach_loader: the iteration has been captured already (the feed launch is part of the graph); "
                               "attach the loader before the first step")
        if loader.batch_size != self.B or loader.num_particles != self.N:
            raise ValueError(f"loader serves batches of {loader.batch_size} jets of {loader.num_particles} particles; the step "
                             f"was built for {self.B} x {self.N}")
        if loader.device != self.data.device:
            raise ValueError(f"loader lives on {loader.device}, the step on {self.data.device}")
        self.loader = loader

    def _noise(self, which: int = 0):
        if self.fixed_noise is not None:
            return self.fixed_noise[which]
        if self.dev.type == "cuda":
            return ops.normal_noise((self.B, self.N, self.latent), self.noise_std, site=which, device=self.dev)
        return torch.empty(self.B, self.N, self.latent, device=self.dev).normal_(0.0, self.noise_std)

    def _noise_masked(self, which: int, mask_out=None, ign_out=None):
        if (self.fixed_noise is None and self.noise_mask and self.dev.type == "cuda"
                and getattr(self.G, "noise_mask_ok", lambda: False)() and (self.N * self.latent) % 2 == 0):
            z, m, ig = ops.normal_noise_masked((self.B, self.N, self.latent), self.noise_std, self.labels, site=which, device=self.dev,
                                               mask_out=None if mask_out is None else mask_out.view(self.B, -1),
                                               ignore_out=None if ign_out is None else ign_out.view(self.B, -1))
            return z, (m, ig)
        return self._noise(which), None

    def _fused_ends(self) -> bool:
        return (self.dev.type == "cuda" and hasattr(self.G, "generate_into") and hasattr(self.D, "features")
                and getattr(self.D, "fused_head", lambda: None)() is not None and self.batch_real_fake
                and not self.gp_lambda)

    def set_aug_prob(self, p: float):
        if self.aug_p is None:
            raise RuntimeError("TrainStep was built without augmentation")
        self.aug_p.fill_(float(p))

    def _augment(self, x: torch.Tensor, site: int, in_place: bool = False) -> torch.Tensor:
        a = self.aug
        if self.dev.type != "cuda":
            args = SimpleNamespace(device=self.dev, aug_r90=a.flags & ops.AUG_R90, aug_f=a.flags & ops.AUG_FLIP,
                                   aug_t=a.flags & ops.AUG_TRANSLATE, aug_s=a.flags & ops.AUG_SCALE,
                                   translate_ratio=a.translate_ratio, scale_sd=a.scale_sd)
            return maugment.augment(args, x, float(self.aug_p))
        if torch.is_grad_enabled() and x.requires_grad:
            return ops.AugmentFn.apply(x, self.aug_p, a.flags, a.translate_ratio, a.scale_sd, site, self.aug_params[site])
        return ops.augment(x, self.aug_p, a.flags, a.translate_ratio, a.scale_sd, site, out=x if in_place else None,
                           params=self.aug_params[site])[0]

    def _bridge(self) -> bool:
        if self.aug is not None or not self.bridge or not hasattr(self.G, "bridge_head") or not hasattr(self.D, "bridge_tail"):
            return False
        h, t = self.G.bridge_head(), self.D.bridge_tail()
        return h is not None and t is not None and ops.bridge_fusable(h[0].shape[1], h[0].shape[0], t[0].shape[0]) \
            and t[0].shape[1] == h[0].shape[0] and h[0].data_ptr() % 16 == 0

    def _route(self, rows_ok: bool = True) -> str:
        if not self._fused_ends():
            return "module"
        if not self.parts:
            return "into"
        return "rows" if rows_ok and self._bridge() else "parts"

    def _generate_for_D(self, route: str):
        own = slice(self.B, None)
        with torch.no_grad():
            if route in ("rows", "parts"):
                rows = {"mask_out": self._mask2[own], "ign_out": self._ign2[own]}
                z, pm = self._noise_masked(0, **rows)
                if route == "rows":
                    fake, jets = None, (self.G.generate_rows(z, self.labels, premask=pm, **rows)[0], self._mask2, self._ign2)
                else:
                    fake, jets = self._x3[own], (self._x3, self._mask2, self._ign2)
                    self.G.generate_parts(z, self.labels, feat_out=fake, premask=pm, **rows)
            elif route == "into":
                fake, jets = self._dcat[own], self._dcat
                self.G.generate_into(self._noise(0), self.labels, fake)
            else:
                fake, jets = self.G(self._noise(0), self.labels), None
            if self.aug is not None:
                fake = self._augment(fake, AUG_SITES["D_fake"], in_place=True)
        return fake, jets

    def _generate(self, route: str):
        if route in ("rows", "parts"):
            z, pm = self._noise_masked(1)
            return (self.G.generate_rows if route == "rows" else self.G.generate_parts)(z, self.labels, premask=pm)
        return self.G(self._noise(1), self.labels)

    def _features(self, route: str, jets, labels, gen_step: bool):
        if route == "into":
            return self.D.features(jets, labels)
        x, mask, ign = jets
        if route == "parts":
            return self.D.features_parts(x, mask, labels, ignore=ign)
        head, real = self.G.bridge_head(), None
        if not gen_step:
            head, real = (head[0].detach(), None if head[1] is None else head[1].detach(), head[2]), self._x3
        return self.D.features_rows(x, head, real, mask, labels, ignore=ign)

    def _head_loss_backward(self, y, mask, gen_step: bool, then=None):
        w, b, mean, sigmoid, p = self.D.fused_head()
        _, dy = ops.disc_head_loss(y, mask, w, b, mean=mean, sigmoid=sigmoid, p_drop=p, training=self.D.training, loss=self.loss,
                                   n_real=self.B, gen_step=gen_step, count=self.B, loss_out=self.G_loss if gen_step else self.D_loss,
                                   want_dy=True, wgrad=None if gen_step else (w.grad, None if b is None else b.grad))
        self._backward(y, dy, then)

    def _seg_D(self, join: bool = True):
        if self.loader is not None:
            self.loader.feed(self)
        self.state.grad_into_param = True
        self.state.order_cache = None
        self.D.train()
        if self.gen_ahead and not self.gen_ahead_late:
            self._fork_generator()
        self.G.eval()
        if not self._clean["D"]:
            self.fD.zero_grad()
        self._clean["D"] = False
        _set_requires_grad(self.fD, True)
        try:
            self._seg_D_body(self._fork_generator if self.gen_ahead_late else None)
        finally:
            if join:
                self._ahead.join("seg_D")

    def _fork_generator(self):
        self.G.train()
        for m in self.G.modules():
            if hasattr(m, "_packed") and getattr(m, "fused", False):
                m._packed().ensure()
        self._ahead.fork(lambda: self._generate(self._route(rows_ok=False)))

    def _seg_D_body(self, late_fork=None):
        route = self._route()
        fake, jets = self._generate_for_D(route)
        if route != "module":
            return self._head_loss_backward(*self._features(route, jets, self._labels2, False), False, late_fork)
        if self.batch_real_fake:
            out = self.D(torch.cat([self.data, fake], 0), torch.cat([self.labels, self.labels], 0))
        else:
            out = torch.cat([self.D(self.data.clone(), self.labels).reshape(-1), self.D(fake, self.labels).reshape(-1)])
        loss = d_loss(self.loss, out, self.B, self._real)
        self.D_loss.copy_(loss.detach())
        if self.gp_lambda:
            real = self.data
            if self.aug is not None:
                with torch.no_grad():
                    real = self._augment(self.data, AUG_SITES["D_real"])
            gp = self.gradient_penalty(real, fake)
            self.GP.copy_(gp.detach())
            loss = loss + gp
        self._backward(loss, then=late_fork)

    def gradient_penalty(self, real: torch.Tensor, fake: torch.Tensor) -> torch.Tensor:
        B = real.shape[0]
        alpha = self.fixed_alpha if self.fixed_alpha is not None else torch.rand(B, 1, 1, device=real.device)
        x = (alpha * real + (1 - alpha) * fake.detach()).requires_grad_(True)
        with ops.double_backward_route(self.dev):
            prob = self.D(x)
            grads = torch.autograd.grad(prob, x, torch.ones_like(prob), create_graph=True, retain_graph=True)[0]
        norm = torch.sqrt((grads.reshape(B, -1) ** 2).sum(1) + 1e-12)
        return self.gp_lambda * ((norm - 1) ** 2).mean()

    def _backward(self, root, grad=None, then=None):
        self.state.deferred_wgrad = ops.WgradBatch()
        if self.wgrad_side:
            if self._wside is None:
                self._wside = torch.cuda.Stream(device=self.dev)
            self.state.wgrad_stream = self._wside
        try:
            torch.autograd.backward([root], None if grad is None else [grad])
            self.state.deferred_wgrad.flush()
            if then is not None:
                then()
        finally:
            self.state.deferred_wgrad = None
            if self.wgrad_side:
                self.state.wgrad_stream = None
                torch.cuda.current_stream(self.dev).wait_stream(self._wside)
                self.state.wgrad_keep.clear()

    @staticmethod
    def _refresh_packed(module: nn.Module):
        packs = []
        for m in module.modules():
            if hasattr(m, "packed_sets"):
                packs += m.packed_sets()
            elif hasattr(m, "refresh_packed"):
                m.refresh_packed()
        if packs:
            ops.refresh_many(packs)

    def _seg_G(self):
        self.fD.step(self.lr_disc, gscale=1.0 / self.world, zero_grad=True)
        self._clean["D"] = True
        self._refresh_packed(self.D)
        self.G.train()
        if not self._clean["G"]:
            self.fG.zero_grad()
        self._clean["G"] = False
        _set_requires_grad(self.fD, False)
        self._ahead.join("seg_G")
        ahead = self._ahead.take()
        route = self._route(rows_ok=ahead is None)
        fake = self._generate(route) if ahead is None else ahead
        if self.aug is not None:
            if isinstance(fake, tuple):
                fake = (self._augment(fake[0], AUG_SITES["G_fake"]),) + tuple(fake[1:])
            else:
                fake = self._augment(fake, AUG_SITES["G_fake"])
        if route != "module":
            self._head_loss_backward(*self._features(route, fake, self.labels, True), True)
        else:
            loss = g_loss(self.loss, self.D(fake, self.labels))
            self._backward(loss)
            self.G_loss.copy_(loss.detach())
        _set_requires_grad(self.fD, True)

    def _seg_end(self):
        self.fG.step(self.lr_gen, gscale=1.0 / self.world, zero_grad=True, advance_seed=ops.seed_tensor(self.dev))
        self._clean["G"] = True
        self._refresh_packed(self.G)
        self.state.grad_into_param = False

    def mark_grads_dirty(self):
        self.fD.zero_grad()
        self.fG.zero_grad()
        self._clean = {"D": True, "G": True}

    def _allreduce(self, flat: FlatParams):
        mdist.allreduce_sum_(flat.grad, self.pg, self.world)

    def _eager(self):
        self._seg_D(join=False); self._allreduce(self.fD)
        self._seg_G(); self._allreduce(self.fG)
        self._seg_end()

    def _training_state(self):
        ts = [self.D_loss, self.G_loss, self.GP, ops.seed_tensor(self.dev)]
        for f in (self.fD, self.fG):
            ts += [f.flat, f.sq, f.step_count] + ([f.aux] if f.aux is not None else [])
            ts += list(f.module.buffers()) + [p for p in f.module.parameters() if not p.requires_grad]
        if self.loader is not None:
            ts.append(self.loader.cursor)
        return ts

    def capture(self, warmup: int = 3):
        s = torch.cuda.Stream(device=self.dev)
        s.wait_stream(torch.cuda.current_stream(self.dev))
        with torch.cuda.stream(s):
            if warmup:
                saved = [t.clone() for t in self._training_state()]
                host = (self.fD._host_steps, self.fG._host_steps)
                rng = torch.cuda.get_rng_state(self.dev) if self.dev.type == "cuda" else None
            for _ in range(warmup):
                self._eager()
            if warmup:
                for t, v in zip(self._training_state(), saved):
                    t.copy_(v)
                self.fD._host_steps, self.fG._host_steps = host
                if rng is not None:
                    torch.cuda.synchronize(self.dev)
                    torch.cuda.set_rng_state(rng, self.dev)
                self._refresh_packed(self.D)
                self._refresh_packed(self.G)
        torch.cuda.current_stream(self.dev).wait_stream(s)
        torch.cuda.synchronize(self.dev)
        graphs = []
        pool = None
        split = (self.world > 1 or self.pg is not None or self.split_graphs) and not self.graph_collectives
        seg_D_open = lambda: self._seg_D(join=False)
        if self.graph_collectives:
            if torch.distributed.get_backend(self.pg) != "nccl":
                raise RuntimeError("graph_collectives needs an nccl (RCCL) process group: only its collectives are stream operations")
            rD, rG = (lambda: self._allreduce(self.fD)), (lambda: self._allreduce(self.fG))
            groups = [(seg_D_open, rD, self._seg_G, rG, self._seg_end)]
        elif split:
            groups = [(self._seg_D,), (self._seg_G,), (self._seg_end,)]
        else:
            groups = [(seg_D_open, self._seg_G, self._seg_end)]
        for segs in groups:
            g = torch.cuda.CUDAGraph()
            with torch.cuda.graph(g, pool=pool):
                for seg in segs:
                    seg()
            pool = g.pool()
            graphs.append(g)
        self._graphs = graphs
        if self.loader is not None:
            self.loader._captured = True

    def set_batch(self, data: torch.Tensor, labels: torch.Tensor):
        if self.loader is not None:
            raise RuntimeError("set_batch: this step takes its batches from the attached DeviceJetLoader, whose feed launch "
                               "overwrites these buffers at the top of every iteration; build the step without a loader to "
                               "set batches by hand")
        self.data.copy_(data, non_blocking=True)
        self.labels.copy_(labels, non_blocking=True)
        self._dcat[:self.B].copy_(self.data)
        self._x3[:self.B].copy_(self.data[..., :3])
        self._mask2[:self.B].copy_(self.data[..., 3:] + 0.5)
        self._ign2[:self.B].copy_(0.5 - self.data[..., 3])
        self._labels2[:self.B].copy_(self.labels)
        self._labels2[self.B:].copy_(self.labels)

    def sync_external_writes(self):
        seen = (self.fD.versions(), self.fG.versions())
        if seen != self._seen_versions:
            if self.dev.type == "cuda":
                self._refresh_packed(self.D)
                self._refresh_packed(self.G)
            self._seen_versions = seen

    def check_range(self):
        import math
        st = ops.range_status(self.dev)
        losses = (float(self.D_loss), float(self.G_loss))
        if st or not all(math.isfinite(v) for v in losses):
            raise FloatingPointError(
                f"mpgan_amd: outside the fused path's numeric range (guard word {st}: 1 = |weight x operand scale| > 65504 in an "
                f"fp16 image, 2 = non-finite weight; losses D {losses[0]}, G {losses[1]})")

    def step(self):
        self.sync_external_writes()
        if self.use_graphs and self._graphs is None:
            self.capture()
        if not self.use_graphs:
            self._eager()
            return
        if len(self._graphs) == 1:
            self._graphs[0].replay()
        else:
            gD, gG, gE = self._graphs
            gD.replay(); self._allreduce(self.fD)
            gG.replay(); self._allreduce(self.fG)
            gE.replay()
        self.fD.note_step(); self.fG.note_step()

    def optimizer_state_dicts(self):
        return self.fD.state_dict(self.lr_disc), self.fG.state_dict(self.lr_gen)

    def load_optimizer_state_dicts(self, sd_D: dict, sd_G: dict):
        self.fD.load_state_dict(sd_D)
        self.fG.load_state_dict(sd_G)
```

Baseline: 131,800 jets/s.

## Fuse jet-order sort into noise kernel and head loss into one launch

Result: slower. 129,200 jets/s (-1.9%).

```diff
diff --git a/include/mpgan_amd.h b/include/mpgan_amd.h
--- a/include/mpgan_amd.h
+++ b/include/mpgan_amd.h
@@ -196,6 +196,7 @@
     float* terms; float* loss_out;
     float* dy; int ld_dy;
     float* dw; float* db; int accumulate;
+    unsigned int* arrive;
 } MpgDiscHead;
 int mpg_disc_head_fwd(const MpgDiscHead* p, void* stream);
 int mpg_disc_head_bwd(const MpgDiscHead* p, void* stream);
@@ -293,6 +294,9 @@
 int mpg_normal(float* out, uint64_t n, const uint64_t* seed, uint32_t tag, float mean, float std, void* stream);
 int mpg_normal_rank_mask(float* out, int B, int N, int L, const uint64_t* seed, uint32_t tag, float mean, float std,
                          const float* labels, int ld_lab, float* mask, float* ignore, void* stream);
+int mpg_normal_rank_mask_order(float* out, int B, int N, int L, const uint64_t* seed, uint32_t tag, float mean, float std,
+                               const float* labels, int ld_lab, float* mask, float* ignore, const float* order_mask,
+                               int order_B, int* order, unsigned int* arrive, void* stream);
 
 #define MPG_AUG_R90 1
 #define MPG_AUG_FLIP 2
diff --git a/mpgan_amd/_lib.py b/mpgan_amd/_lib.py
--- a/mpgan_amd/_lib.py
+++ b/mpgan_amd/_lib.py
@@ -138,6 +138,7 @@
         ("loss", C.c_int), ("gen_step", C.c_int), ("n_real", C.c_int), ("inv_count", C.c_float),
         ("gout", _fp), ("terms", _fp), ("loss_out", _fp),
         ("dy", _fp), ("ld_dy", C.c_int), ("dw", _fp), ("db", _fp), ("accumulate", C.c_int),
+        ("arrive", _fp),
     ]
 
 
@@ -238,6 +239,8 @@
     "mpg_normal": (C.c_int, [_fp, C.c_uint64, _fp, C.c_uint32, C.c_float, C.c_float, C.c_void_p]),
     "mpg_normal_rank_mask": (C.c_int, [_fp, C.c_int, C.c_int, C.c_int, _fp, C.c_uint32, C.c_float, C.c_float, _fp, C.c_int, _fp, _fp,
                                        C.c_void_p]),
+    "mpg_normal_rank_mask_order": (C.c_int, [_fp, C.c_int, C.c_int, C.c_int, _fp, C.c_uint32, C.c_float, C.c_float, _fp, C.c_int, _fp, _fp,
+                                       _fp, C.c_int, _fp, _fp, C.c_void_p]),
     "mpg_jet_obs": (C.c_int, [_fp, C.c_int, C.c_int, C.c_int, C.c_int, C.c_int, _fp, _fp, C.c_void_p]),
     "mpg_jet_efps_d4": (C.c_int, [_fp, C.c_int, C.c_int, C.c_int, C.c_int, C.c_int, _fp, C.c_void_p]),
     "mpg_jet_emd": (C.c_int, [_fp, C.c_int, _fp, C.c_int, C.c_int, C.c_int, C.c_int, C.c_int, C.c_float, _fp, _fp, C.c_void_p]),
diff --git a/mpgan_amd/csrc/head.hip b/mpgan_amd/csrc/head.hip
--- a/mpgan_amd/csrc/head.hip
+++ b/mpgan_amd/csrc/head.hip
@@ -1,4 +1,5 @@
 #include "common.h"
+#include "jet_order.h"
 #include "../../include/mpgan_amd.h"
 
 namespace {
@@ -25,41 +26,7 @@
 
 __global__ __launch_bounds__(1024) void jet_order_kernel(const float* __restrict__ mask, int B, int N, int* __restrict__ order) {
     extern __shared__ int jo[];
-    int* keys = jo;
-    int* hist = jo + B;
-    int* wcnt = jo + B + N + 2;
-    const int nw = (B + 63) / 64, lane = threadIdx.x & 63;
-    for (int t = threadIdx.x; t < N + 2; t += blockDim.x) hist[t] = 0;
-    for (int t = threadIdx.x; t < nw * (N + 1); t += blockDim.x) wcnt[t] = 0;
-    __syncthreads();
-    for (int b = threadIdx.x; b < B; b += blockDim.x) {
-        const float* mb = mask + (size_t)b * N;
-        int c = 0;
-#pragma unroll 8
-        for (int i = 0; i < N; ++i) c += mb[i] != 0.f;
-        const int k = N - c;
-        keys[b] = k;
-        atomicAdd(&hist[k + 1], 1);
-        atomicAdd(&wcnt[(b >> 6) * (N + 1) + k], 1);
-    }
-    __syncthreads();
-    if (threadIdx.x == 0)
-        for (int k = 1; k < N + 2; ++k) hist[k] += hist[k - 1];
-    for (int k = threadIdx.x; k <= N; k += blockDim.x) {
-        int run = 0;
-        for (int w = 0; w < nw; ++w) { const int c = wcnt[w * (N + 1) + k]; wcnt[w * (N + 1) + k] = run; run += c; }
-    }
-    __syncthreads();
-    for (int b0 = (threadIdx.x >> 6) * 64; b0 < B; b0 += blockDim.x) {
-        const int b = b0 + lane;
-        const int k = b < B ? keys[b] : -1;
-        int below = 0;
-        for (int l = 0; l < 64; ++l) {
-            const int kl = __shfl(k, l, 64);
-            below += (l < lane && kl == k);
-        }
-        if (b < B) order[hist[k] + wcnt[(b >> 6) * (N + 1) + k] + below] = b;
-    }
+    jet_order_sort(mask, B, N, order, jo);
 }
 
 __global__ __launch_bounds__(256) void gen_tail_fwd_kernel(const float* __restrict__ y, int ldy, const float* __restrict__ mask,
@@ -92,9 +59,7 @@
 MPG_DEV void disc_head_bwd_jet(const MpgDiscHead& p, const int b, const int lane, const float out, const float aux0);
 
 template <bool FUSED>
-__global__ __launch_bounds__(256) void disc_head_fwd_kernel(const MpgDiscHead p) {
-    const int lane = threadIdx.x & 63, b = blockIdx.x * 4 + (threadIdx.x >> 6);
-    if (b >= p.B) return;
+MPG_DEV void disc_head_fwd_jet(const MpgDiscHead& p, const int b, const int lane) {
     const float* yb = p.y + (size_t)b * p.N * p.ldy;
     float z = 0.f, msum = 0.f;
     for (int f0 = 0; f0 < p.F; f0 += 32) {
@@ -131,6 +96,13 @@
     if (FUSED) disc_head_bwd_jet(p, b, lane, out, keep * pool_scale);
 }
 
+template <bool FUSED>
+__global__ __launch_bounds__(256) void disc_head_fwd_kernel(const MpgDiscHead p) {
+    const int lane = threadIdx.x & 63, b = blockIdx.x * 4 + (threadIdx.x >> 6);
+    if (b >= p.B) return;
+    disc_head_fwd_jet<FUSED>(p, b, lane);
+}
+
 MPG_DEV float loss_grad(int loss, float out, float t, float& term) {
     switch (loss) {
     case 0: term = (out - t) * (out - t); return 2.f * (out - t);
@@ -177,42 +149,83 @@
     disc_head_bwd_jet(p, b, lane, p.out[b], p.aux[2 * b]);
 }
 
+MPG_DEV void head_loss_sum(const MpgDiscHead& p, float* red, const int tid) {
+    float s = 0.f;
+    for (int b = tid; b < p.B; b += 256) s += p.terms[b];
+    red[tid] = s;
+    __syncthreads();
+    for (int o = 128; o > 0; o >>= 1) { if (tid < o) red[tid] += red[tid + o]; __syncthreads(); }
+    if (tid == 0) *p.loss_out = red[0];
+}
+
+template <int NF>
+MPG_DEV void head_wgrad_wave(const MpgDiscHead& p, const int f0, const int fstep, const int lane) {
+    const float ds = p.thr ? p.dscale : 1.f;
+    float s0[NF], s1[NF], s2[NF], s3[NF];
+#pragma unroll
+    for (int j = 0; j < NF; ++j) s0[j] = s1[j] = s2[j] = s3[j] = 0.f;
+    auto add = [&](float* s, int b) {
+        if (b >= p.B) {
+#pragma unroll
+            for (int j = 0; j < NF; ++j) s[j] += 0.f;
+            return;
+        }
+        const float gzp = p.aux[2 * b + 1], a0 = p.aux[2 * b];
+        const float ps = a0 != 0.f ? a0 / ds : 0.f;
+#pragma unroll
+        for (int j = 0; j < NF; ++j) {
+            const int f = f0 + j * fstep;
+            if (f > p.F) continue;
+            s[j] += f >= p.F ? gzp : gzp * ps * p.pooled[(size_t)b * p.F + f];
+        }
+    };
+    for (int b = lane; b < p.B; b += 256) { add(s0, b); add(s1, b + 64); add(s2, b + 128); add(s3, b + 192); }
+#pragma unroll
+    for (int j = 0; j < NF; ++j) {
+        const int f = f0 + j * fstep;
+        if (f > p.F) continue;
+        float s = (s0[j] + s1[j]) + (s2[j] + s3[j]);
+        s += __shfl_xor(s, 1, 64); s += __shfl_xor(s, 2, 64); s += __shfl_xor(s, 4, 64); s += __shfl_xor(s, 8, 64); s += __shfl_xor(s, 16, 64);
+        s += __shfl_xor(s, 32, 64);
+        if (lane == 0) {
+            if (f < p.F) p.dw[f] = s + (p.accumulate ? p.dw[f] : 0.f);
+            else if (p.db != nullptr) p.db[0] = s + (p.accumulate ? p.db[0] : 0.f);
+        }
+    }
+}
+
 __global__ __launch_bounds__(256) void disc_head_reduce_kernel(const MpgDiscHead p) {
     __shared__ float red[256];
     const int tid = threadIdx.x;
     if (blockIdx.x == 0) {
-        if (p.loss >= 0 && p.loss_out != nullptr) {
-            float s = 0.f;
-            for (int b = tid; b < p.B; b += 256) s += p.terms[b];
-            red[tid] = s;
-            __syncthreads();
-            for (int o = 128; o > 0; o >>= 1) { if (tid < o) red[tid] += red[tid + o]; __syncthreads(); }
-            if (tid == 0) *p.loss_out = red[0];
-        }
+        if (p.loss >= 0 && p.loss_out != nullptr) head_loss_sum(p, red, tid);
         return;
     }
     if (p.dw == nullptr) return;
-    const int f = (blockIdx.x - 1) * 4 + (tid >> 6), lane = tid & 63;
+    const int f = (blockIdx.x - 1) * 4 + (tid >> 6);
     if (f > p.F) return;
-    const float ds = p.thr ? p.dscale : 1.f;
-    auto term = [&](int b) {
-        if (b >= p.B) return 0.f;
-        const float gzp = p.aux[2 * b + 1];
-        if (f >= p.F) return gzp;
-        const float a0 = p.aux[2 * b];
-        return gzp * (a0 != 0.f ? a0 / ds : 0.f) * p.pooled[(size_t)b * p.F + f];
-    };
-    float s0 = 0.f, s1 = 0.f, s2 = 0.f, s3 = 0.f;
-    for (int b = lane; b < p.B; b += 256) {
-        s0 += term(b); s1 += term(b + 64); s2 += term(b + 128); s3 += term(b + 192);
-    }
-    float s = (s0 + s1) + (s2 + s3);
-    s += __shfl_xor(s, 1, 64); s += __shfl_xor(s, 2, 64); s += __shfl_xor(s, 4, 64); s += __shfl_xor(s, 8, 64); s += __shfl_xor(s, 16, 64);
-    s += __shfl_xor(s, 32, 64);
-    if (lane == 0) {
-        if (f < p.F) p.dw[f] = s + (p.accumulate ? p.dw[f] : 0.f);
-        else if (p.db != nullptr) p.db[0] = s + (p.accumulate ? p.db[0] : 0.f);
-    }
+    head_wgrad_wave<1>(p, f, 0, tid & 63);
+}
+
+constexpr int HEAD_NF = 9;
+__global__ __launch_bounds__(256) void disc_head_loss_kernel(const MpgDiscHead p) {
+    __shared__ float red[256];
+    __shared__ unsigned int last;
+    const int tid = threadIdx.x, lane = tid & 63, b = blockIdx.x * 4 + (tid >> 6);
+    if (b < p.B) disc_head_fwd_jet<true>(p, b, lane);
+    __threadfence();
+    __syncthreads();
+    if (tid == 0) {
+        const unsigned int old = __hip_atomic_fetch_add(p.arrive, 1u, __ATOMIC_ACQ_REL, __HIP_MEMORY_SCOPE_AGENT);
+        last = old == gridDim.x - 1;
+        if (old == gridDim.x - 1) __hip_atomic_store(p.arrive, 0u, __ATOMIC_RELAXED, __HIP_MEMORY_SCOPE_AGENT);
+    }
+    __syncthreads();
+    if (!last) return;
+    __threadfence();
+    if (p.loss >= 0 && p.loss_out != nullptr) head_loss_sum(p, red, tid);
+    if (p.dw == nullptr) return;
+    for (int f0 = tid >> 6; f0 <= p.F; f0 += 4 * HEAD_NF) head_wgrad_wave<HEAD_NF>(p, f0, 4, lane);
 }
 
 __global__ __launch_bounds__(256) void knn_sets_kernel(const float* __restrict__ x, int ldx, const float* __restrict__ mask, int N, int F,
@@ -385,6 +398,10 @@
     if (p->loss < 0 || p->terms == nullptr) return -2;
     if (p->dw != nullptr && p->pooled == nullptr) return -2;
     hipStream_t st = (hipStream_t)stream;
+    if (p->arrive != nullptr && (p->loss_out != nullptr || p->dw != nullptr)) {
+        hipLaunchKernelGGL(disc_head_loss_kernel, dim3((p->B + 3) / 4), dim3(256), 0, st, *p);
+        return (int)hipGetLastError();
+    }
     hipLaunchKernelGGL(disc_head_fwd_kernel<true>, dim3((p->B + 3) / 4), dim3(256), 0, st, *p);
     if (p->loss_out != nullptr || p->dw != nullptr)
         hipLaunchKernelGGL(disc_head_reduce_kernel, dim3(1 + (p->dw != nullptr ? (p->F + 1 + 3) / 4 : 0)), dim3(256), 0, st, *p);
diff --git a/mpgan_amd/csrc/jet_order.h b/mpgan_amd/csrc/jet_order.h
--- /dev/null
+++ b/mpgan_amd/csrc/jet_order.h
@@ -0,0 +1,40 @@
+#pragma once
+#include "common.h"
+
+MPG_DEV void jet_order_sort(const float* mask, int B, int N, int* __restrict__ order, int* jo) {
+    int* keys = jo;
+    int* hist = jo + B;
+    int* wcnt = jo + B + N + 2;
+    const int nw = (B + 63) / 64, lane = threadIdx.x & 63;
+    for (int t = threadIdx.x; t < N + 2; t += blockDim.x) hist[t] = 0;
+    for (int t = threadIdx.x; t < nw * (N + 1); t += blockDim.x) wcnt[t] = 0;
+    __syncthreads();
+    for (int b = threadIdx.x; b < B; b += blockDim.x) {
+        const float* mb = mask + (size_t)b * N;
+        int c = 0;
+#pragma unroll 8
+        for (int i = 0; i < N; ++i) c += mb[i] != 0.f;
+        const int k = N - c;
+        keys[b] = k;
+        atomicAdd(&hist[k + 1], 1);
+        atomicAdd(&wcnt[(b >> 6) * (N + 1) + k], 1);
+    }
+    __syncthreads();
+    if (threadIdx.x == 0)
+        for (int k = 1; k < N + 2; ++k) hist[k] += hist[k - 1];
+    for (int k = threadIdx.x; k <= N; k += blockDim.x) {
+        int run = 0;
+        for (int w = 0; w < nw; ++w) { const int c = wcnt[w * (N + 1) + k]; wcnt[w * (N + 1) + k] = run; run += c; }
+    }
+    __syncthreads();
+    for (int b0 = (threadIdx.x >> 6) * 64; b0 < B; b0 += blockDim.x) {
+        const int b = b0 + lane;
+        const int k = b < B ? keys[b] : -1;
+        int below = 0;
+        for (int l = 0; l < 64; ++l) {
+            const int kl = __shfl(k, l, 64);
+            below += (l < lane && kl == k);
+        }
+        if (b < B) order[hist[k] + wcnt[(b >> 6) * (N + 1) + k] + below] = b;
+    }
+}
diff --git a/mpgan_amd/csrc/optim.hip b/mpgan_amd/csrc/optim.hip
--- a/mpgan_amd/csrc/optim.hip
+++ b/mpgan_amd/csrc/optim.hip
@@ -1,4 +1,5 @@
 #include "common.h"
+#include "jet_order.h"
 #include "../../include/mpgan_amd.h"
 
 namespace {
@@ -72,10 +73,9 @@
     }
 }
 
-__global__ __launch_bounds__(256) void normal_rank_mask_kernel(float* __restrict__ out, int N, int L, const uint64_t* __restrict__ seed,
-                                                               uint32_t tag, float mean, float std, const float* __restrict__ labels,
-                                                               int ld_lab, float* __restrict__ mask, float* __restrict__ ignore) {
-    extern __shared__ float first[];
+MPG_DEV void normal_rank_mask_jet(float* __restrict__ out, int N, int L, const uint64_t* __restrict__ seed, uint32_t tag, float mean,
+                                  float std, const float* __restrict__ labels, int ld_lab, float* mask, float* __restrict__ ignore,
+                                  float* first) {
     const uint64_t sd = *seed;
     const uint32_t lo = (uint32_t)sd, hi = (uint32_t)(sd >> 32);
     const int b = blockIdx.x;
@@ -108,6 +108,34 @@
         mask[(size_t)b * N + i] = rank <= n_minus_1 ? 1.f : 0.f;
         if (ignore != nullptr) ignore[(size_t)b * N + i] = rank <= n_minus_1 ? 0.f : 1.f;
     }
+}
+
+__global__ __launch_bounds__(256) void normal_rank_mask_kernel(float* __restrict__ out, int N, int L, const uint64_t* __restrict__ seed,
+                                                               uint32_t tag, float mean, float std, const float* __restrict__ labels,
+                                                               int ld_lab, float* __restrict__ mask, float* __restrict__ ignore) {
+    extern __shared__ float first[];
+    normal_rank_mask_jet(out, N, L, seed, tag, mean, std, labels, ld_lab, mask, ignore, first);
+}
+
+__global__ __launch_bounds__(256) void normal_rank_mask_order_kernel(float* __restrict__ out, int N, int L, const uint64_t* __restrict__ seed,
+                                                                     uint32_t tag, float mean, float std, const float* __restrict__ labels,
+                                                                     int ld_lab, float* mask, float* __restrict__ ignore,
+                                                                     const float* omask, int OB, int* __restrict__ order,
+                                                                     unsigned int* arrive) {
+    extern __shared__ float first[];
+    __shared__ unsigned int last;
+    normal_rank_mask_jet(out, N, L, seed, tag, mean, std, labels, ld_lab, mask, ignore, first);
+    __threadfence();
+    __syncthreads();
+    if (threadIdx.x == 0) {
+        const unsigned int old = __hip_atomic_fetch_add(arrive, 1u, __ATOMIC_ACQ_REL, __HIP_MEMORY_SCOPE_AGENT);
+        last = old == gridDim.x - 1;
+        if (old == gridDim.x - 1) __hip_atomic_store(arrive, 0u, __ATOMIC_RELAXED, __HIP_MEMORY_SCOPE_AGENT);
+    }
+    __syncthreads();
+    if (!last) return;
+    __threadfence();
+    jet_order_sort(omask, OB, N, order, reinterpret_cast<int*>(first));
 }
 
 inline int nblocks(uint64_t n) { return (int)((n + 255) / 256 < 2048 ? (n + 255) / 256 : 2048); }
@@ -155,3 +183,17 @@
                        std, labels, ld_lab, mask, ignore);
     return (int)hipGetLastError();
 }
+
+extern "C" int mpg_normal_rank_mask_order(float* out, int B, int N, int L, const uint64_t* seed, uint32_t tag, float mean, float std,
+                                          const float* labels, int ld_lab, float* mask, float* ignore, const float* order_mask,
+                                          int order_B, int* order, unsigned int* arrive, void* stream) {
+    if (B <= 0 || N <= 0 || L <= 0 || N > 8192 || ((size_t)N * L) % 2) return -1;
+    if (seed == nullptr || labels == nullptr || mask == nullptr || !(std >= 0.f)) return -1;
+    if (order_mask == nullptr || order_B <= 0 || order == nullptr || arrive == nullptr) return -1;
+    const size_t words = (size_t)order_B + N + 2 + (size_t)((order_B + 63) / 64) * (N + 1);
+    if (words > 16000) return -2;
+    const size_t lds = (words > (size_t)N ? words : (size_t)N) * sizeof(int);
+    hipLaunchKernelGGL(normal_rank_mask_order_kernel, dim3(B), dim3(256), lds, (hipStream_t)stream, out, N, L, seed, tag, mean, std,
+                       labels, ld_lab, mask, ignore, order_mask, order_B, order, arrive);
+    return (int)hipGetLastError();
+}
diff --git a/mpgan_amd/ops.py b/mpgan_amd/ops.py
--- a/mpgan_amd/ops.py
+++ b/mpgan_amd/ops.py
@@ -327,7 +327,8 @@
 
 
 def normal_noise_masked(shape, std: float, labels: torch.Tensor, site: int = 0, device="cuda", mean: float = 0.0,
-                        mask_out: Optional[torch.Tensor] = None, ignore_out: Optional[torch.Tensor] = None):
+                        mask_out: Optional[torch.Tensor] = None, ignore_out: Optional[torch.Tensor] = None,
+                        order_of: Optional[torch.Tensor] = None):
     B, N, L = shape
     out = torch.empty(shape, device=device, dtype=torch.float32)
     lab = labels[:, -1]
@@ -336,6 +337,17 @@
     mask = mask_out if mask_out is not None else torch.empty((B, N), device=device, dtype=torch.float32)
     ign = ignore_out if ignore_out is not None else torch.empty((B, N), device=device, dtype=torch.float32)
     assert mask.is_contiguous() and ign.is_contiguous() and mask.numel() == B * N and ign.numel() == B * N
+    if order_of is not None and jet_order_fits(*order_of.shape):
+        B2 = order_of.shape[0]
+        assert mask_out is not None and order_of.is_contiguous() and order_of.shape[1] == N
+        assert order_of.data_ptr() <= mask.data_ptr() and mask.data_ptr() + 4 * B * N <= order_of.data_ptr() + 4 * B2 * N
+        order = torch.empty((B2,), device=out.device, dtype=torch.int32)
+        check(_lib.lib().mpg_normal_rank_mask_order(_p(out), B, N, L, _p(seed_tensor(out.device)), NOISE_TAG + int(site), mean, std,
+                                                    _p(lab), lab.stride(0), _p(mask), _p(ign), _p(order_of), B2,
+                                                    C.c_void_p(order.data_ptr()), C.c_void_p(_tickets(out.device, 1).data_ptr()),
+                                                    _stream()), "mpg_normal_rank_mask_order")
+        dev_state(out.device).order_cache = (_order_key(order_of), order)
+        return out, mask.view(B, N), ign.view(B, N)
     check(_lib.lib().mpg_normal_rank_mask(_p(out), B, N, L, _p(seed_tensor(out.device)), NOISE_TAG + int(site), mean, std,
                                           _p(lab), lab.stride(0), _p(mask), _p(ign), _stream()), "mpg_normal_rank_mask")
     return out, mask.view(B, N), ign.view(B, N)
@@ -563,9 +575,21 @@
 MAX_CHUNK_SENDERS = 160
 
 
+def _order_key(mask2d: torch.Tensor):
+    return (mask2d.data_ptr(), tuple(mask2d.shape), mask2d._version)
+
+
+def jet_order_fits(B: int, N: int) -> bool:
+    return B + N + 2 + (B + 63) // 64 * (N + 1) <= 16000
+
+
+def jet_order_wanted(B: int, N: int) -> bool:
+    return bool(OPTIONS["lpt_order"]) and B * ((N + 31) // 32) * _sender_chunks(B, N) > NUM_CUS and jet_order_fits(B, N)
+
+
 def jet_order(mask2d: torch.Tensor) -> torch.Tensor:
     st = dev_state(mask2d.device)
-    key = (mask2d.data_ptr(), tuple(mask2d.shape), mask2d._version)
+    key = _order_key(mask2d)
     hit = getattr(st, "order_cache", None)
     if hit is not None and hit[0] == key:
         return hit[1]
@@ -708,7 +732,7 @@
             e.es, e.wq = _p(es), _p(wq)
         RB = (N + 31) // 32
         order = None
-        if m1 is not None and OPTIONS["lpt_order"] and B * RB * SC > NUM_CUS and B + N + 2 + (B + 63) // 64 * (N + 1) <= 16384:
+        if m1 is not None and OPTIONS["lpt_order"] and B * RB * SC > NUM_CUS and jet_order_fits(B, N):
             order = jet_order(m1.view(B, N))
             e.order = C.c_void_p(order.data_ptr())
         need_grad = any(ctx.needs_input_grad) and not no_grad
@@ -1636,7 +1660,7 @@
 
 
 def disc_head_loss(y, mask, w, b, *, mean, sigmoid, p_drop, training, loss, n_real, gen_step, count, loss_out,
-                   want_dy=True, wgrad=None):
+                   want_dy=True, wgrad=None, one_launch=False):
     y, m = _head_inputs(y, mask)
     B, N, F = y.shape
     dev = y.device
@@ -1652,6 +1676,8 @@
     h.dy, h.ld_dy = _p(dy), F
     if wgrad is not None:
         h.dw, h.db, h.accumulate = _p(wgrad[0]), _p(wgrad[1]), 1
+    if one_launch is not False:
+        h.arrive = C.c_void_p((_tickets(dev, 1) if one_launch is True else one_launch).data_ptr())
     check(_lib.lib().mpg_disc_head_loss(C.byref(h), _stream()), "mpg_disc_head_loss")
     return out, dy
 
diff --git a/mpgan_amd/train.py b/mpgan_amd/train.py
--- a/mpgan_amd/train.py
+++ b/mpgan_amd/train.py
@@ -309,7 +309,8 @@
 
         def _switch(name: str, default: str = "1") -> str:
             return os.environ.get(name, default)
-        on = {k: _switch(k) != "0" for k in ("MPG_PARTS", "MPG_GEN_AHEAD", "MPG_GEN_AHEAD_LATE", "MPG_WGRAD_SIDE", "MPG_BRIDGE", "MPG_NOISE_MASK")}
+        on = {k: _switch(k) != "0" for k in ("MPG_PARTS", "MPG_GEN_AHEAD", "MPG_GEN_AHEAD_LATE", "MPG_WGRAD_SIDE", "MPG_BRIDGE", "MPG_NOISE_MASK",
+                                            "MPG_FUSE_GLUE")}
         if graph_collectives is None:
             graph_collectives = _switch("MPG_GRAPH_COLLECTIVES", "") == "1"
         self.split_graphs = bool(_switch("MPG_SPLIT_GRAPHS", ""))
@@ -367,6 +368,7 @@
                 self.aug_params = [torch.zeros(batch_size, 6, device=dev) for _ in AUG_SITES]
         self.noise_mask = gpu and on["MPG_NOISE_MASK"]
         self.fixed_noise = None
+        self.fuse_glue = gpu and on["MPG_FUSE_GLUE"]
         self._seen_versions = (self.fD.versions(), self.fG.versions())
         self._clean = {"D": True, "G": True}
         self.loader = None
@@ -395,12 +397,13 @@
             return ops.normal_noise((self.B, self.N, self.latent), self.noise_std, site=which, device=self.dev)
         return torch.empty(self.B, self.N, self.latent, device=self.dev).normal_(0.0, self.noise_std)
 
-    def _noise_masked(self, which: int, mask_out=None, ign_out=None):
+    def _noise_masked(self, which: int, mask_out=None, ign_out=None, order_of=None):
         if (self.fixed_noise is None and self.noise_mask and self.dev.type == "cuda"
                 and getattr(self.G, "noise_mask_ok", lambda: False)() and (self.N * self.latent) % 2 == 0):
             z, m, ig = ops.normal_noise_masked((self.B, self.N, self.latent), self.noise_std, self.labels, site=which, device=self.dev,
                                                mask_out=None if mask_out is None else mask_out.view(self.B, -1),
-                                               ignore_out=None if ign_out is None else ign_out.view(self.B, -1))
+                                               ignore_out=None if ign_out is None else ign_out.view(self.B, -1),
+                                               order_of=None if order_of is None else order_of.view(order_of.shape[0], -1))
             return z, (m, ig)
         return self._noise(which), None
 
@@ -445,7 +448,8 @@
         with torch.no_grad():
             if route in ("rows", "parts"):
                 rows = {"mask_out": self._mask2[own], "ign_out": self._ign2[own]}
-                z, pm = self._noise_masked(0, **rows)
+                early = self.fuse_glue and isinstance(self.D, MPDiscriminator) and ops.jet_order_wanted(2 * self.B, self.N)
+                z, pm = self._noise_masked(0, order_of=self._mask2 if early else None, **rows)
                 if route == "rows":
                     fake, jets = None, (self.G.generate_rows(z, self.labels, premask=pm, **rows)[0], self._mask2, self._ign2)
                 else:
@@ -481,7 +485,8 @@
         w, b, mean, sigmoid, p = self.D.fused_head()
         _, dy = ops.disc_head_loss(y, mask, w, b, mean=mean, sigmoid=sigmoid, p_drop=p, training=self.D.training, loss=self.loss,
                                    n_real=self.B, gen_step=gen_step, count=self.B, loss_out=self.G_loss if gen_step else self.D_loss,
-                                   want_dy=True, wgrad=None if gen_step else (w.grad, None if b is None else b.grad))
+                                   want_dy=True, wgrad=None if gen_step else (w.grad, None if b is None else b.grad),
+                                   one_launch=self.fuse_glue)
         self._backward(y, dy, then)
 
     def _seg_D(self, join: bool = True):
```
